# divelab/DIG

Hardware: NVIDIA H100
Metric: molecules/sec SphereNet QM9-shape (higher is better)
Workload: dtype f32

## Files before the change

### dig_b200/_lib.py

```python
import ctypes
import os
from ctypes import POINTER, Structure, c_char_p, c_double, c_int32, c_int64, c_void_p

_HERE = os.path.dirname(os.path.abspath(__file__))
LIB_PATH = os.path.join(_HERE, "libdig3d.so")

P = c_void_p


class InitEWeights(Structure):
    _fields_ = [(n, P) for n in ("emb", "w_rbf0", "b_rbf0", "w_lin", "b_lin", "w_rbf1")]


class UpdateEWeights(Structure):
    _fields_ = ([(n, P) for n in ("w_rbf1", "w_rbf2", "w_sbf2", "w_t2", "w_rbf",
                                  "w_kj", "b_kj", "w_ji", "b_ji", "w_down", "w_up")]
                + [("w_res", P * 6), ("b_res", P * 6), ("w_lin", P), ("b_lin", P)])


class SchnetBlockWeights(Structure):
    _fields_ = [(n, P) for n in ("w_lin", "w_mlp0", "b_mlp0", "w_mlp2", "b_mlp2", "w_v1", "b_v1", "w_v2", "b_v2")]


class ComenetBlockWeights(Structure):
    _fields_ = ([(n, P) for n in ("w_lin", "b_lin", "w_f1a", "w_f1b", "w_f2a", "w_f2b", "w_rel1", "b_rel1",
                                  "w_root1", "w_rel2", "b_rel2", "w_root2", "w_lin1", "b_lin1", "w_lin2",
                                  "b_lin2", "w_cat", "b_cat")]
                + [("w_lins", P * 8), ("b_lins", P * 8)]
                + [(n, P) for n in ("norm_w", "norm_b", "norm_ms", "w_final", "b_final")]
                + [("n_lins", c_int32)])


class ComenetHeadWeights(Structure):
    _fields_ = [("w_lins", P * 8), ("b_lins", P * 8), ("w_out", P), ("b_out", P), ("n_lins", c_int32)]


class TcUpdateE(Structure):
    _fields_ = ([(n, P) for n in ("p_ji", "b_ji", "p_kj", "b_kj", "p_down", "p_up")]
                + [("p_res", P * 6), ("b_res", P * 6)]
                + [(n, P) for n in ("p_lin", "b_lin", "w_rbf1", "w_rbf2", "w_rbf", "w_sbf2", "w_t2")])


class UpdateVWeights(Structure):
    _fields_ = [("w_up", P), ("b_up", P), ("w_lins", P * 8), ("b_lins", P * 8), ("w_out", P),
                ("n_lins", c_int32)]


SIGNATURES = {
    "dig3d_last_error": [],
    "dig3d_abi_version": [],
    "dig3d_graph_ptr": [P, c_int64, c_int64, P, P],
    "dig3d_radius_neighbors": [P, P, P, c_int64, c_int64, c_double, c_int32, P, P, P],
    "dig3d_validate_nodes": [P, P, c_int64, c_int64, c_int32, P, P],
    "dig3d_knn2": [P, P, P, c_int64, c_int64, P, P, P],
    "dig3d_triplet_geometry_knn": [P, P, P, P, P, c_int64, P, P, P, P, P, P, P],
    "dig3d_triplet_count": [P, P, c_int64, c_int32, P, P],
    "dig3d_triplet_count_out": [P, P, c_int64, c_int32, P, P, P],
    "dig3d_scan_counts3": [P, P, P, c_int64, P, P, P, P, P],
    "dig3d_edge_fill_out": [P, P, P, P, P, c_int64, c_int32, c_int64, P, P, P, P, P, P, P, P, P, P, P, P],
    "dig3d_scan_counts": [P, P, c_int64, P, P, P, P],
    "dig3d_edge_fill": [P, P, P, P, P, c_int64, c_int32, c_int64, P, P, P, P, P, P, P],
    "dig3d_edges_to_csr": [P, P, c_int64, c_int64, P, P, P, P, P, P, P, P],
    "dig3d_triplet_geometry": [P, P, P, P, P, c_int64, c_int32, P, P, P, P, P, P, P],
    "dig3d_edge_basis": [P, c_int64, c_double, c_int32, P, c_int32, c_int32, P, P, P],
    "dig3d_edge_basis_set_split": [c_int32],
    "dig3d_triplet_basis_project_set_mode": [c_int32],
    "dig3d_triplet_basis": [P, P, P, P, c_int64, c_int32, P, P, P],
    "dig3d_triplet_basis_project": [P, P, P, P, P, P, P, P, P, c_int64, c_int64, c_int32, c_int32,
                                    c_int32, P, P, P, P, P],
    "dig3d_triplet_basis_project_lists": [P, P, P, P, P, P, P, P, P, c_int64, c_int64, c_int32, c_int32,
                                    c_int32, P, P, P, P, P, P, P, P],
    "dig3d_triplet_basis_project_node": [P, P, P, P, P, P, P, P, c_int64, c_int64, c_int32, c_int32, c_int32, c_int32,
                                         P, P, P, P, P],
    "dig3d_segment_sum": [P, P, c_int64, c_int64, P, P],
    "dig3d_sphere_init_e": [P, P, P, P, c_int64, POINTER(InitEWeights), P, P, P],
    "dig3d_sphere_update_e_a": [P, P, c_int64, POINTER(UpdateEWeights), P, P, P],
    "dig3d_sphere_update_e_b": [P, P, P, P, P, P, c_int32, P, P, P, P, c_int64,
                                POINTER(UpdateEWeights), P, P, P],
    "dig3d_sphere_update_v": [P, c_int64, c_int32, POINTER(UpdateVWeights), P, P],
    "dig3d_sphere_update_v_batched": [P, c_int64, c_int32, c_int32, P, P, P],
    "dig3d_graph_readout": [P, P, c_int64, c_int64, c_int32, c_int32, P, P],
    "dig3d_tc_packed_floats": [c_int32, c_int32],
    "dig3d_tc_pack": [P, P, P, P, c_int32, P],
    "dig3d_tc_timeouts": [],
    "dig3d_sphere_init_e_tc": [P, P, P, P, c_int64, POINTER(InitEWeights), P, P, P, P],
    "dig3d_sphere_update_e_a_tc": [P, P, c_int64, POINTER(TcUpdateE), P, P, P],
    "dig3d_sphere_triplet_gather": [P, P, P, c_int32, P, P, P, P, c_int64, P, P, P, P],
    "dig3d_sphere_triplet_gather_node": [P, P, P, c_int32, P, P, P, P, P, c_int64, c_int32, P, P, P, P],
    "dig3d_sphere_triplet_gather_warp": [P, P, P, c_int32, P, P, P, P, P, c_int64, c_int32, c_int32, P, P, P, P, P,
                                         P, P],
    "dig3d_sphere_triplet_gather_tc": [P, P, P, c_int32, P, P, P, P, P, c_int64, c_int32, P, P, P, P],
    "dig3d_sphere_update_e_b_tc": [P, P, P, P, P, c_int64, POINTER(TcUpdateE), P, P, P],
    "dig3d_tc_set_fast_swish": [c_int32],
    "dig3d_h16_packed_bytes": [c_int32, c_int32],
    "dig3d_h16_pack": [P, P, P, P, c_int32, P],
    "dig3d_sphere_init_e_h16": [P, P, P, P, c_int64, POINTER(InitEWeights), P, P, P, P],
    "dig3d_sphere_init_e_h16_tab": [P, P, P, P, c_int64, POINTER(InitEWeights), P, P, P, P, P, P],
    "dig3d_sphere_update_e_a_h16": [P, P, c_int64, POINTER(TcUpdateE), P, P, P],
    "dig3d_sphere_update_e_b_h16": [P, P, P, P, P, c_int64, POINTER(TcUpdateE), P, P, P],
    "dig3d_sphere_update_e_ba_h16": [P, P, P, P, P, c_int64, POINTER(TcUpdateE), POINTER(TcUpdateE), P, P, P, P, P],
    "dig3d_sphere_update_v_h16_supported": [c_int32, c_int32, c_int32, c_int32],
    "dig3d_sphere_update_v_h16": [P, c_int64, c_int32, c_int32, c_int32, P, P, P, P],
    "dig3d_h16_pack_t": [P, P, P, P, P, c_int32, P],
    "dig3d_linear_h16_supported": [c_int32, c_int32],
    "dig3d_linear_h16": [P, c_int64, c_int32, c_int32, P, P, P, P, P, P],
    "dig3d_h16_overflow": [c_int32],
    "dig3d_h16_timeouts": [],
    "dig3d_h16_trace": [c_int32, P],
    "dig3d_h16_set_fast_swish": [c_int32],
    "dig3d_h16_set_wide_epilogue": [c_int32],
    "dig3d_tc_trace": [c_int32, P],
    "dig3d_schnet_block": [P, c_int64, P, P, P, c_int64, P, c_int32, c_double, c_double, c_int32, c_int32,
                           POINTER(SchnetBlockWeights), P, P, P, P],
    "dig3d_schnet_readout": [P, c_int64, c_int32, P, P, P, P, c_int32, P, P],
    "dig3d_comenet_geometry": [P, P, P, P, P, P, P, c_int64, c_int64, c_double, P, P, P, P, P],
    "dig3d_comenet_embed": [P, P, c_int64, P, P],
    "dig3d_pbc_edge_vectors": [P, P, P, P, P, c_int64, P, P, P],
    "dig3d_comenet_geometry_edges": [P, P, P, P, P, c_int64, c_int64, c_double, P, P, P, P, P, P],
    "dig3d_radius_graph_pbc_count": [P, P, P, c_int64, c_int64, c_double, c_int32, P, P, P, P, P, P, P],
    "dig3d_radius_graph_pbc_fill": [P, P, c_int64, c_int64, c_double, P, P, P, P, c_int64, P, P, P, P],
    "dig3d_comenet_block": [P, P, P, P, P, P, P, c_int64, c_int64, c_int64, POINTER(ComenetBlockWeights),
                            POINTER(ComenetHeadWeights), c_int32, P, P, P, P, P, P, P, P],
    "dig3d_edge_weighted_sum": [P, P, P, P, c_int64, c_int32, P, P],
    "dig3d_comenet_filter_sum": [P, c_int32, P, P, P, P, c_int64, c_int32, P, P],
    "dig3d_linear": [P, c_int64, c_int32, c_int32, P, P, P, P, c_int32, P],
    "dig3d_wgrad": [P, P, c_int64, c_int32, c_int32, P, P, c_int32, P],
    "dig3d_wgrad_tc": [P, P, c_int64, c_int32, c_int32, P, P, c_int32, P],
    "dig3d_wgrad_tc_supported": [c_int64, c_int32, c_int32],
    "dig3d_wgrad_set_mode": [c_int32],
    "dig3d_wgrad_tc_timeouts": [],
    "dig3d_act": [P, c_int64, c_int32, P, P],
    "dig3d_act_bwd": [P, P, c_int64, c_int32, P, P],
    "dig3d_adam_step": [P, P, P, P, c_int64, c_double, c_double, c_double, c_double, c_double, c_int64, P],
    "dig3d_ewise": [P, P, c_int64, c_int32, P, P],
    "dig3d_rowscale": [P, P, c_int64, c_int32, P, P],
    "dig3d_gather_rows": [P, P, c_int32, c_int64, c_int32, P, P],
    "dig3d_scatter_add_rows": [P, P, c_int32, c_int64, c_int32, P, P],
    "dig3d_rbf_freq_grad": [P, c_int64, c_double, c_int32, P, c_int32, P, P, P],
    "dig3d_triplet_basis_project_bwd": [P, P, P, P, P, P, P, P, P, c_int64, c_int64, c_int32, P, P, P, P, P],
    "dig3d_sphere_triplet_gather_bwd": [P, P, P, P, P, P, P, P, c_int64, P, P, P, P, P, P, P, P],
    "dig3d_graphnorm": [P, P, c_int64, c_int32, P, P, P, c_double, P, P, P, P],
    "dig3d_graphnorm_bwd": [P, P, P, c_int64, c_int32, P, P, P, P, P, P, P, P, P],
    "dig3d_edge_dist_bwd": [P, P, P, P, P, c_int64, P, P],
    "dig3d_triplet_angle_bwd": [P, P, P, P, P, P, c_int64, P, P],
    "dig3d_edge_basis_bwd": [P, c_int64, c_double, c_int32, P, c_int32, c_int32, P, P, P, P],
    "dig3d_triplet_basis_project_bwd_geom": [P, P, P, P, P, P, P, P, P, P, c_int64, c_int64, c_int32, P, P, P, P,
                                             c_double, P, P, P, P],
    "dig3d_triplet_torsion_bwd": [P, P, P, P, P, P, c_int64, P, P],
    "dig3d_schnet_edge_features_bwd": [P, c_int64, P, c_int32, c_double, c_double, P, P, P, P],
    "dig3d_rowdot": [P, P, c_int64, c_int32, P, P],
    "dig3d_tc_pack_t": [P, P, P, P, P, c_int32, P],
    "dig3d_linear_tc_supported": [c_int32, c_int32],
    "dig3d_linear_tc": [P, c_int64, c_int32, c_int32, P, P, P, P, P],
    "dig3d_act_bwd2": [P, P, P, c_int64, c_int32, P, P],
    "dig3d_geometry_jvp": [P, P, P, P, P, P, P, c_int64, P, P, P, P],
    "dig3d_edge_basis_tangent": [P, P, c_int64, c_double, c_int32, P, c_int32, c_int32, P, P, P],
    "dig3d_rbf_freq_grad_tangent": [P, P, c_int64, c_double, c_int32, P, c_int32, P, P, P],
    "dig3d_triplet_basis_tangent": [P, P, P, P, P, P, P, c_int64, c_int32, P, P, P],
    "dig3d_edge_dist_bwd2": [P, P, P, P, P, P, c_int64, P, P, P],
    "dig3d_schnet_edge_features_bwd2": [P, c_int64, P, c_int32, c_double, c_double, P, P, P, P, P, P, P],
    "dig3d_pronet_edge_features": [P, P, P, P, P, c_int64, c_int64, c_int32, c_double, c_int32, P, P, P, P, P, P],
    "dig3d_linear_set_config": [c_int32],
    "dig3d_transpose": [P, c_int32, c_int32, P, P],
    "dig3d_schnet_edge_features": [P, c_int64, P, c_int32, c_double, c_double, P, P, P],
}
_RESTYPES = {"dig3d_last_error": c_char_p, "dig3d_h16_packed_bytes": c_int64}

_lib = None


class Dig3dError(RuntimeError):
    rc = None


def load():
    global _lib
    if _lib is not None:
        return _lib
    if not os.path.exists(LIB_PATH):
        raise Dig3dError(
            f"{LIB_PATH} not found: build it with `python -m dig_b200.build` "
            "(nvcc -gencode arch=compute_90a,code=sm_90a). There is no CPU/PyTorch fallback.")
    lib = ctypes.CDLL(LIB_PATH)
    for name, argtypes in SIGNATURES.items():
        try:
            fn = getattr(lib, name)
        except AttributeError as exc:
            raise Dig3dError(f"libdig3d.so does not export {name}") from exc
        fn.argtypes = argtypes
        fn.restype = _RESTYPES.get(name, ctypes.c_int)
    _lib = lib
    return lib


launch_count = 0
_timing = None


def start_timing():
    global _timing
    _timing = {}


def stop_timing():
    global _timing
    import torch
    torch.cuda.synchronize()
    out = {k: [a.elapsed_time(b) for a, b in v] for k, v in (_timing or {}).items()}
    _timing = None
    return out


def call(name, *args):
    global launch_count
    lib = load()
    if _timing is not None:
        import torch
        a, b = torch.cuda.Event(enable_timing=True), torch.cuda.Event(enable_timing=True)
        a.record()
        rc = getattr(lib, name)(*args)
        b.record()
        _timing.setdefault(name, []).append((a, b))
    else:
        rc = getattr(lib, name)(*args)
    launch_count += 1
    if rc != 0:
        msg = lib.dig3d_last_error()
        err = Dig3dError(f"{name} failed (rc={rc}): {msg.decode() if msg else ''}")
        err.rc = rc
        raise err
```

### dig_b200/csrc/spherenet_h16.cu

```cuda
#include <cuda_fp16.h>
#include "common.cuh"
#define TC90_TM_COLS 512
#include "wgmma.cuh"

namespace dig3d {
using namespace tc90;

constexpr int H_M = 128;
constexpr int H_AKU = H_M + 1;
constexpr int H_PLANE = 16 * H_AKU * 16;
constexpr int H_STAGES = 5;
constexpr int H_SLAB_K = 32;
constexpr int H_STAGE_BYTES = 2 * 4 * 128 * 16;
constexpr int H_TILE_WARPS = 8;
constexpr int H_TILE_THREADS = H_TILE_WARPS * 32;
constexpr int H_CTRL_THREADS = 128;
constexpr int H_THREADS = H_CTRL_THREADS + 2 * H_TILE_THREADS;
constexpr int H_CTRL_WARPS = H_CTRL_THREADS / 32;
__device__ __forceinline__ void h_regs_ctrl() { asm volatile("setmaxnreg.dec.sync.aligned.u32 64;"); }
__device__ __forceinline__ void h_regs_epi() { asm volatile("setmaxnreg.inc.sync.aligned.u32 104;"); }
constexpr float H_SA = 8.0f, H_SW = 64.0f;
constexpr float H_INV = 1.0f / (H_SA * H_SW);
constexpr int H_LDS = 129;

struct HSmem {
  unsigned char a[2][2][H_PLANE];
  unsigned char w[H_STAGES][H_STAGE_BYTES];
  float bias[8][128];
  float wr[128 * 8];
  int dst[2][H_M];
  int aux[2][2][H_M];
  uint64_t full[H_STAGES], empty[H_STAGES], a_ready[2], d_ready[2][2], d_free[2][2];
  uint64_t l_done;
  uint32_t tmem_base;
};
static_assert(sizeof(HSmem) <= 227 * 1024, "HSmem exceeds the shared memory of an SM");
static_assert(sizeof(HSmem) > TM_ONE_CTA_PER_SM_SMEM, "one CTA per SM sizes the accumulator-store slot pool");
static_assert(2 * H_PLANE == H_M * H_LDS * 4, "the fp32 staging overlay must cover exactly one tile's planes");

struct HGemm {
  const unsigned char* w;
  const float* bias;
  int K, N;
  int tile_stride;
};

static __device__ unsigned int g_h16_overflow = 0;
static int h16_fast_swish = 1;
static __device__ long long g_h16_trace[128];
static __device__ int g_h16_trace_on = 0;

__device__ __forceinline__ float ex2_ftz(float x) {
  float y;
  asm("ex2.approx.ftz.f32 %0, %1;" : "=f"(y) : "f"(x));
  return y;
}
__device__ __forceinline__ float rcp_ftz(float x) {
  float y;
  asm("rcp.approx.ftz.f32 %0, %1;" : "=f"(y) : "f"(x));
  return y;
}
template <bool FAST>
__device__ __forceinline__ float hswish(float x) {
  return FAST ? x * rcp_ftz(1.0f + ex2_ftz(x * -1.4426950408889634f)) : __fdiv_rn(x, 1.0f + expf(-x));
}
template <bool FAST>
__device__ __forceinline__ float hswish8(float t8) {
  return FAST ? t8 * rcp_ftz(1.0f + ex2_ftz(t8 * (-1.4426950408889634f / H_SA)))
              : __fdiv_rn(t8, 1.0f + expf(-t8 * (1.0f / H_SA)));
}

struct HRing {
  int q, t, c;
};
__device__ __forceinline__ void h_produce(HSmem& s, const HGemm* g, int ng, int ntile, HRing& r, int& it) {
  if (r.q >= ng) return;
  const uint32_t bytes = 2u * 4u * (uint32_t)g[r.q].N * 16u;
  if (threadIdx.x == 0) {
    const int st = it % H_STAGES;
    mbar_arrive_expect_tx(&s.full[st], bytes);
    bulk_g2s(s.w[st], g[r.q].w + (size_t)r.t * g[r.q].tile_stride + (size_t)r.c * bytes, bytes, &s.full[st]);
  }
  ++it;
  if (++r.c == g[r.q].K / H_SLAB_K) { r.c = 0; if (++r.t == ntile) { r.t = 0; ++r.q; } }
}
template <bool SHARED_A>
__device__ __forceinline__ void h_mma_n(HSmem& s, const HGemm* g, int ng, int ntile, uint32_t tmem) {
  const int wt = threadIdx.x;
  HRing ring = {0, 0, 0};
  int pit = 0;
  for (int i = 0; i < H_STAGES; ++i) h_produce(s, g, ng, ntile, ring, pit);
  int it = 0, ch = 0;
  int uses00 = 0, uses01 = 0, uses10 = 0, uses11 = 0;
  int last0 = -1, last1 = -1;
  for (int q = 0; q < ng; ++q) {
    const int nslab = g[q].K / H_SLAB_K, n = g[q].N;
    for (int t = 0; t < ntile; ++t) {
      if (!SHARED_A || t == 0) {
        mbar_wait(&s.a_ready[SHARED_A ? 0 : t], q & 1);
        tc_fence_after();
      }
      const uint32_t a_hi = smem_u32(SHARED_A ? s.a[0][0] : s.a[t][0]), a_lo = smem_u32(SHARED_A ? s.a[1][0] : s.a[t][1]);
      for (int c = 0; c < nslab; c += 2, it += 2) {
        const int ab = ch & 1;
        const int lt = ab ? last1 : last0;
        if (lt >= 0) {
          const int u = lt ? (ab ? uses11 : uses10) : (ab ? uses01 : uses00);
          mbar_wait(&s.d_free[lt][ab], (u - 1) & 1);
        }
        mbar_wait(&s.full[it % H_STAGES], (it / H_STAGES) & 1);
        mbar_wait(&s.full[(it + 1) % H_STAGES], ((it + 1) / H_STAGES) & 1);
        tc_fence_after();
        for (int mh = 0; mh < 2; ++mh)
          for (int nh = 0; nh < n / 64; ++nh) {
            float d[32];
            wg_fence();
#pragma unroll
            for (int sl = 0; sl < 2; ++sl) {
              const uint32_t w_hi = smem_u32(s.w[(it + sl) % H_STAGES]) + (uint32_t)(nh * 64 * 16), w_lo = w_hi + 4u * n * 16u;
              const uint32_t a_m = (uint32_t)(mh * 64 * 16);
#pragma unroll
              for (int ks = 0; ks < 2; ++ks) {
                const uint32_t a_off = a_m + (uint32_t)(((c + sl) * 4 + ks * 2) * H_AKU * 16), b_off = (uint32_t)(ks * 2 * n * 16);
                mma_f16(d, smem_desc(a_lo + a_off, H_AKU * 16, 128), smem_desc(w_hi + b_off, n * 16, 128), (sl | ks) != 0);
                mma_f16(d, smem_desc(a_hi + a_off, H_AKU * 16, 128), smem_desc(w_lo + b_off, n * 16, 128), 1);
              }
#pragma unroll
              for (int ks = 0; ks < 2; ++ks) {
                const uint32_t a_off = a_m + (uint32_t)(((c + sl) * 4 + ks * 2) * H_AKU * 16), b_off = (uint32_t)(ks * 2 * n * 16);
                mma_f16(d, smem_desc(a_hi + a_off, H_AKU * 16, 128), smem_desc(w_hi + b_off, n * 16, 128), 1);
              }
            }
            wg_commit();
            wg_wait0();
            tm_store_frag(d, wt, tmem + ((uint32_t)(64 * mh) << 16) + 128u * ab + 64u * nh);
          }
        tc_fence_before();
        wg_bar();
        h_produce(s, g, ng, ntile, ring, pit);
        h_produce(s, g, ng, ntile, ring, pit);
        if (wt == 0) mbar_arrive(&s.d_ready[t][ab]);
        if (t) { if (ab) ++uses11; else ++uses10; } else { if (ab) ++uses01; else ++uses00; }
        if (ab) last1 = t; else last0 = t;
        ++ch;
      }
      if (SHARED_A && t == ntile - 1 && wt == 0) mbar_arrive(&s.l_done);
    }
  }
}

struct HCtx {
  int t, et, row, half;
  uint32_t tl;
  int ntile, ch;
  int use0, use1;
  bool bad;
  unsigned char *ahi, *alo;
};
__device__ __forceinline__ HCtx h_ctx(HSmem& s, int ntile) {
  const int warp = threadIdx.x >> 5, lane = threadIdx.x & 31;
  const int t = (warp - H_CTRL_WARPS) / H_TILE_WARPS, we = (warp - H_CTRL_WARPS) % H_TILE_WARPS;
  const int quarter = warp & 3;
  return {t, (int)threadIdx.x - H_CTRL_THREADS - t * H_TILE_THREADS, 32 * quarter + lane, we >> 2,
          s.tmem_base + ((uint32_t)(32 * quarter) << 16), ntile, 0, 0, 0, false, s.a[t][0], s.a[t][1]};
}
__device__ __forceinline__ void h_tile_bar(int t) {
  asm volatile("bar.sync %0, %1;" ::"r"(1 + t), "n"(H_TILE_THREADS) : "memory");
}
__device__ __forceinline__ void h_epi_done(HSmem& s, int t) {
  fence_async_smem();
  tc_fence_before();
  __syncwarp();
  if ((threadIdx.x & 31) == 0) mbar_arrive(&s.a_ready[t]);
}
__device__ __forceinline__ void h_store_ku(HSmem& s, const HCtx& c, int row, int ku, const float (&x)[8]) {
  uint32_t h[4], l[4];
#pragma unroll
  for (int i = 0; i < 4; ++i) {
    const __half2 hh = __floats2half2_rn(x[2 * i], x[2 * i + 1]);
    const float2 hf = __half22float2(hh);
    const __half2 ll = __floats2half2_rn(x[2 * i] - hf.x, x[2 * i + 1] - hf.y);
    h[i] = *reinterpret_cast<const uint32_t*>(&hh);
    l[i] = *reinterpret_cast<const uint32_t*>(&ll);
  }
  const int o = (ku * H_AKU + row) * 16;
  *reinterpret_cast<uint4*>(c.ahi + o) = make_uint4(h[0], h[1], h[2], h[3]);
  *reinterpret_cast<uint4*>(c.alo + o) = make_uint4(l[0], l[1], l[2], l[3]);
}
__device__ __forceinline__ void h_store_a16(HSmem& s, const HCtx& c, int col, const float (&v8)[16]) {
  float x[8];
#pragma unroll
  for (int u = 0; u < 2; ++u) {
#pragma unroll
    for (int i = 0; i < 8; ++i) x[i] = v8[8 * u + i];
    h_store_ku(s, c, c.row, (col >> 3) + u, x);
  }
}
__device__ __forceinline__ bool h_finite(float x) { return fabsf(x) <= 3.402823466e38f; }
template <int KU>
__device__ __forceinline__ void h_load_tile(HSmem& s, HCtx& c, const float* __restrict__ g, size_t ld, int rows) {
#pragma unroll
  for (int k = 0; k < H_M * KU / H_TILE_THREADS; ++k) {
    const int f = c.et + k * H_TILE_THREADS, row = f / KU, ku = f % KU;
    float x[8];
    if (row < rows) {
      const float4 p0 = __ldg(reinterpret_cast<const float4*>(g + (size_t)row * ld + ku * 8));
      const float4 p1 = __ldg(reinterpret_cast<const float4*>(g + (size_t)row * ld + ku * 8 + 4));
      x[0] = p0.x * H_SA; x[1] = p0.y * H_SA; x[2] = p0.z * H_SA; x[3] = p0.w * H_SA;
      x[4] = p1.x * H_SA; x[5] = p1.y * H_SA; x[6] = p1.z * H_SA; x[7] = p1.w * H_SA;
    } else {
#pragma unroll
      for (int i = 0; i < 8; ++i) x[i] = 0.f;
    }
    h_store_ku(s, c, row, ku, x);
  }
}
template <int KU>
struct HTileRegs { float4 v[H_M * KU / H_TILE_THREADS][2]; };
template <int KU>
__device__ __forceinline__ void h_tile_fetch(HTileRegs<KU>& r, int et, const float* __restrict__ g, size_t ld, int rows) {
#pragma unroll
  for (int k = 0; k < H_M * KU / H_TILE_THREADS; ++k) {
    const int f = et + k * H_TILE_THREADS, row = f / KU, ku = f % KU;
    if (row < rows) {
      r.v[k][0] = __ldg(reinterpret_cast<const float4*>(g + (size_t)row * ld + ku * 8));
      r.v[k][1] = __ldg(reinterpret_cast<const float4*>(g + (size_t)row * ld + ku * 8 + 4));
    } else {
      r.v[k][0] = r.v[k][1] = make_float4(0.f, 0.f, 0.f, 0.f);
    }
  }
}
template <int KU>
__device__ __forceinline__ void h_tile_commit(HSmem& s, const HCtx& c, const HTileRegs<KU>& r) {
#pragma unroll
  for (int k = 0; k < H_M * KU / H_TILE_THREADS; ++k) {
    const int f = c.et + k * H_TILE_THREADS, row = f / KU, ku = f % KU;
    const float4 p0 = r.v[k][0], p1 = r.v[k][1];
    const float x[8] = {p0.x * H_SA, p0.y * H_SA, p0.z * H_SA, p0.w * H_SA, p1.x * H_SA, p1.y * H_SA, p1.z * H_SA, p1.w * H_SA};
    h_store_ku(s, c, row, ku, x);
  }
}
template <int NP, bool FIRST>
__device__ __forceinline__ void h_drain(HSmem& s, HCtx& c, int col0, int chunks, float (&acc)[NP * 16]) {
  if (c.t == 1) c.ch += chunks;
  for (int k = 0; k < chunks; ++k, ++c.ch) {
    const int ab = c.ch & 1;
    const int use = ab ? c.use1 : c.use0;
    mbar_wait(&s.d_ready[c.t][ab], use & 1);
    if (ab) ++c.use1; else ++c.use0;
    tc_fence_after();
    const uint32_t ta = c.tl + 128u * ab + col0;
    if (FIRST && k == 0) {
#pragma unroll
      for (int p = 0; p < NP; ++p) tmem_ld16f(ta + 16 * p, &acc[p * 16]);
      tmem_ld_wait();
    } else {
#pragma unroll
      for (int p = 0; p < NP; p += 2) {
        uint32_t r[2][16];
        tmem_ld16(ta + 16 * p, r[0]);
        if (p + 1 < NP) tmem_ld16(ta + 16 * p + 16, r[1]);
        tmem_ld_wait();
#pragma unroll
        for (int i = 0; i < 16; ++i) {
          acc[p * 16 + i] = __fadd_rn(acc[p * 16 + i], __uint_as_float(r[0][i]));
          if (p + 1 < NP) acc[p * 16 + 16 + i] = __fadd_rn(acc[p * 16 + 16 + i], __uint_as_float(r[1][i]));
        }
      }
    }
    tc_fence_before();
    __syncwarp();
    if ((threadIdx.x & 31) == 0) mbar_arrive(&s.d_free[c.t][ab]);
  }
  if (c.t == 0 && c.ntile == 2) c.ch += chunks;
}
__device__ __forceinline__ void h_setup(HSmem& s, int a_ready_warps = H_TILE_WARPS, int d_free_warps = H_TILE_WARPS) {
  if (threadIdx.x == 0) {
    for (int i = 0; i < H_STAGES; ++i) { mbar_init(&s.full[i], 1); mbar_init(&s.empty[i], 1); }
    for (int i = 0; i < 2; ++i) {
      mbar_init(&s.a_ready[i], a_ready_warps);
      for (int j = 0; j < 2; ++j) { mbar_init(&s.d_ready[i][j], 1); mbar_init(&s.d_free[i][j], d_free_warps); }
    }
    mbar_init(&s.l_done, 1);
    mbar_fence_init();
  }
  if ((threadIdx.x >> 5) == 0) tmem_alloc(&s.tmem_base, 512);
}
__device__ __forceinline__ void h_finish(HSmem& s, const HCtx* c) {
  if (c && c->bad) atomicOr(&g_h16_overflow, 1u);
  tc_fence_before();
  __syncthreads();
  if ((threadIdx.x >> 5) == 0) tmem_dealloc(s.tmem_base, 512);
}
template <int W>
__device__ __forceinline__ void h_store_tile_coalesced(HSmem& s, const HCtx& c, int col0, const float (&v)[W / 2],
                                                       float* __restrict__ out, int rows) {
  constexpr int LD = W + 1, RPW = 128 / W;
  float* st = reinterpret_cast<float*>(s.a[c.t][0]);
#pragma unroll
  for (int i = 0; i < W / 2; ++i) st[c.row * LD + col0 + i] = v[i];
  h_tile_bar(c.t);
  const int w = c.et >> 5, lane = c.et & 31;
  for (int r0 = w * RPW; r0 < rows; r0 += H_TILE_WARPS * RPW) {
    const int r = r0 + (RPW == 2 ? (lane >> 4) : 0), c4 = 4 * (RPW == 2 ? (lane & 15) : lane);
    if (r < rows) {
      const float* src = st + r * LD + c4;
      *reinterpret_cast<float4*>(out + (size_t)r * W + c4) = make_float4(src[0], src[1], src[2], src[3]);
    }
  }
}

template <int W>
__device__ __forceinline__ void h_store_tile_strided(HSmem& s, const HCtx& c, int col0, const float (&v)[W / 2],
                                                     float* __restrict__ out, int ld, int rows,
                                                     const float* __restrict__ res = nullptr) {
  constexpr int LD = W + 1, RPW = 128 / W;
  float* st = reinterpret_cast<float*>(s.a[c.t][0]);
#pragma unroll
  for (int i = 0; i < W / 2; ++i) st[c.row * LD + col0 + i] = v[i];
  h_tile_bar(c.t);
  const int w = c.et >> 5, lane = c.et & 31;
  for (int r0 = w * RPW; r0 < rows; r0 += H_TILE_WARPS * RPW) {
    const int r = r0 + (RPW == 2 ? (lane >> 4) : 0), c4 = 4 * (RPW == 2 ? (lane & 15) : lane);
    if (r < rows) {
      const float* src = st + r * LD + c4;
      float4 o = make_float4(src[0], src[1], src[2], src[3]);
      if (res) {
        const float4 q = __ldg(reinterpret_cast<const float4*>(res + (size_t)r * ld + c4));
        o.x += q.x; o.y += q.y; o.z += q.z; o.w += q.w;
      }
      *reinterpret_cast<float4*>(out + (size_t)r * ld + c4) = o;
    }
  }
}

__device__ __forceinline__ void h_segment_sums(const HSmem& s, const HCtx& c, int rows, float* __restrict__ v_in) {
  const int col = c.et & 127, r0 = (c.et >> 7) * 64, r1 = min(rows, r0 + 64);
  if (r0 >= r1) return;
  const float* e2t = reinterpret_cast<const float*>(s.a[c.t][0]);
  const int* dst = s.dst[c.t];
  float run = 0.f;
  int cur = dst[r0];
  bool first = true;
  for (int r = r0; r < r1; ++r) {
    const int d = dst[r];
    if (d != cur) {
      if (first) atomicAdd(v_in + (size_t)cur * 128 + col, run);
      else v_in[(size_t)cur * 128 + col] = run;
      first = false; run = 0.f; cur = d;
    }
    run += e2t[r * H_LDS + col];
  }
  atomicAdd(v_in + (size_t)cur * 128 + col, run);
}

struct HPackJob { const float* w; unsigned char* out; int N, K, trans; };
struct HPackJobs { HPackJob job[16]; };
__global__ void h16_pack_kernel(HPackJobs jobs) {
  const HPackJob jb = jobs.job[blockIdx.y];
  const int total = jb.N * jb.K;
  for (int id = blockIdx.x * blockDim.x + threadIdx.x; id < total; id += gridDim.x * blockDim.x) {
    const int n = id / jb.K, k = id % jb.K;
    const float x = __ldg(jb.w + (jb.trans ? (size_t)k * jb.trans + n : (size_t)id)) * H_SW;
    const __half h = __float2half_rn(x);
    const __half l = __float2half_rn(x - __half2float(h));
    const int c = k >> 5, ku = (k & 31) >> 3, kk = k & 7;
    const size_t slab = (size_t)c * (2 * 4 * jb.N * 16);
    const size_t o = ((size_t)ku * jb.N + n) * 16 + kk * 2;
    *reinterpret_cast<__half*>(jb.out + slab + o) = h;
    *reinterpret_cast<__half*>(jb.out + slab + (size_t)4 * jb.N * 16 + o) = l;
  }
}

constexpr int R_UNIT = 64;
constexpr int R_STAGES = 8;
constexpr int R_LDS = 136;
constexpr int R_WG = 128;
constexpr int R_THREADS = 3 * R_WG;
__device__ __forceinline__ void r_regs_producer() { asm volatile("setmaxnreg.dec.sync.aligned.u32 40;"); }
__device__ __forceinline__ void r_regs_consumer() { asm volatile("setmaxnreg.inc.sync.aligned.u32 232;"); }

struct RSmem {
  unsigned char w[R_STAGES][H_STAGE_BYTES];
  float tile[2][R_UNIT * R_LDS];
  float rbf[2][R_UNIT * 6];
  float bias[8][128];
  float bias_a[2][128];
  float wr[128 * 8];
  float wr1[64];
  float wr2[128 * 8];
  int dst[2][R_UNIT];
  uint64_t full[R_STAGES], empty[R_STAGES];
};
static_assert(sizeof(RSmem) <= 227 * 1024, "RSmem exceeds the shared memory of an SM");

enum { RE_B = 0, RE_BA = 1, RE_A = 2 };
struct REParams {
  HGemm g[11];
  const float* w_rbf;
  const float *w_rbf1, *w_rbf2;
  float *x_ji, *x_down;
};

__device__ __forceinline__ void r_bar(int cw) { asm volatile("bar.sync %0, %1;" ::"r"(1 + cw), "n"(R_WG) : "memory"); }
__device__ __forceinline__ void cp_async4(void* sm, const void* g, bool valid) {
  asm volatile("cp.async.ca.shared.global [%0], [%1], 4, %2;" ::"r"(smem_u32(sm)), "l"(g), "r"(valid ? 4 : 0) : "memory");
}
__device__ __forceinline__ void cp_async8(void* sm, const void* g, bool valid) {
  asm volatile("cp.async.ca.shared.global [%0], [%1], 8, %2;" ::"r"(smem_u32(sm)), "l"(g), "r"(valid ? 8 : 0) : "memory");
}
__device__ __forceinline__ void cp_async_commit() { asm volatile("cp.async.commit_group;" ::: "memory"); }
__device__ __forceinline__ void cp_async_wait_all() { asm volatile("cp.async.wait_group 0;" ::: "memory"); }

__device__ __forceinline__ void r_split(float x0, float x1, uint32_t& hi, uint32_t& lo) {
  const __half2 hh = __floats2half2_rn(x0, x1);
  const float2 hf = __half22float2(hh);
  const __half2 ll = __floats2half2_rn(x0 - hf.x, x1 - hf.y);
  hi = *reinterpret_cast<const uint32_t*>(&hh);
  lo = *reinterpret_cast<const uint32_t*>(&ll);
}
struct RA { uint32_t hi[8][4], lo[8][4]; };
__device__ __forceinline__ void r_acc_to_a(const float (&v)[64], RA& a, float scale = 1.0f) {
#pragma unroll
  for (int s = 0; s < 8; ++s)
#pragma unroll
    for (int r = 0; r < 4; ++r) r_split(v[frag_a_src(s, r)] * scale, v[frag_a_src(s, r) + 1] * scale, a.hi[s][r], a.lo[s][r]);
}
template <int KS>
__device__ __forceinline__ void r_load_a(RA& a, const float* __restrict__ g, int ld, int rows, int wt) {
#pragma unroll
  for (int s = 0; s < KS; ++s)
#pragma unroll
    for (int r = 0; r < 4; ++r) {
      const int row = frag_a_row(wt, r), col = frag_a_col(wt, s, r);
      const float2 x = row < rows ? __ldg(reinterpret_cast<const float2*>(g + (size_t)row * ld + col)) : make_float2(0.f, 0.f);
      r_split(x.x * H_SA, x.y * H_SA, a.hi[s][r], a.lo[s][r]);
    }
}
__device__ __forceinline__ void r_fetch_rows(float* tile, const float* __restrict__ src, int rows, int fr, int fc) {
#pragma unroll
  for (int j = 0; j < 16; ++j)
#pragma unroll
    for (int h = 0; h < 2; ++h) {
      const int row = fr + 8 * h, col = 8 * j + fc;
      cp_async8(tile + row * R_LDS + col, src + (size_t)(row < rows ? row : 0) * 128 + col, row < rows);
    }
  cp_async_commit();
}

__device__ __forceinline__ void r_release(RSmem& s, int it, int n) {
  __syncwarp();
  if ((threadIdx.x & 31) == 0)
    for (int i = 0; i < n; ++i) mbar_arrive(&s.empty[(it + i) % R_STAGES]);
}
template <int CH, int N>
__device__ __forceinline__ void r_chunk(RSmem& s, const RA& a, float (&t)[N / 2], int it) {
#pragma unroll
  for (int sl = 0; sl < 2; ++sl) {
    const uint32_t w_hi = smem_u32(s.w[(it + 2 * CH + sl) % R_STAGES]), w_lo = w_hi + 4u * N * 16u;
#pragma unroll
    for (int ks = 0; ks < 2; ++ks) {
      const int k = 4 * CH + 2 * sl + ks;
      const uint32_t b_off = (uint32_t)(ks * 2 * N * 16);
      mma_f16_rs(t, a.lo[k], smem_desc(w_hi + b_off, N * 16, 128), (sl | ks) != 0);
      mma_f16_rs(t, a.hi[k], smem_desc(w_lo + b_off, N * 16, 128), 1);
    }
#pragma unroll
    for (int ks = 0; ks < 2; ++ks)
      mma_f16_rs(t, a.hi[4 * CH + 2 * sl + ks], smem_desc(w_hi + (uint32_t)(ks * 2 * N * 16), N * 16, 128), 1);
  }
}
template <int NCH, int N>
__device__ __forceinline__ void r_issue(RSmem& s, const RA& a, float (&acc)[N / 2], float (&d)[N / 2], int it) {
#pragma unroll
  for (int i = 0; i < 2 * NCH; ++i) mbar_wait(&s.full[(it + i) % R_STAGES], ((it + i) / R_STAGES) & 1);
  wg_fence();
  r_chunk<0, N>(s, a, acc, it);
  if (NCH == 2) r_chunk<1, N>(s, a, d, it);
  wg_commit();
}
template <int NCH, int N>
__device__ __forceinline__ void r_complete(RSmem& s, float (&acc)[N / 2], const float (&d)[N / 2], int& it) {
  wg_wait0();
  r_release(s, it, 2 * NCH);
  it += 2 * NCH;
  if (NCH == 2) {
#pragma unroll
    for (int i = 0; i < N / 2; ++i) acc[i] = __fadd_rn(acc[i], d[i]);
  }
}
__device__ __forceinline__ void r_skip(RSmem& s, int& it, int n) {
  for (int i = 0; i < n; ++i, ++it) {
    mbar_wait(&s.full[it % R_STAGES], (it / R_STAGES) & 1);
    r_release(s, it, 1);
  }
}

__device__ __forceinline__ void r_segment_sums(const float* tile, const int* dst, int rows, int col,
                                               float* __restrict__ v_in) {
  float run = 0.f;
  int cur = dst[0];
  bool first = true;
  for (int r = 0; r < rows; ++r) {
    const int d = dst[r];
    if (d != cur) {
      if (first) atomicAdd(v_in + (size_t)cur * 128 + col, run);
      else v_in[(size_t)cur * 128 + col] = run;
      first = false; run = 0.f; cur = d;
    }
    run += tile[r * R_LDS + col];
  }
  atomicAdd(v_in + (size_t)cur * 128 + col, run);
}

template <bool FAST, int MODE>
__global__ void __launch_bounds__(R_THREADS, 1)
sphere_update_e_h16_kernel(const float* __restrict__ m, const float* __restrict__ x_ji,
                           const float* __restrict__ e1_in, const float* __restrict__ rbf0,
                           const int32_t* __restrict__ dst, int n_edges, REParams P, float* __restrict__ e1_out,
                           float* __restrict__ v_in) {
  constexpr int NG = MODE == RE_B ? 8 : MODE == RE_BA ? 11 : 3;
  extern __shared__ __align__(1024) unsigned char h_raw[];
  RSmem& s = *reinterpret_cast<RSmem*>(h_raw);
  const int tid = threadIdx.x, wg = tid / R_WG;
  auto n_units = [&]() { return (n_edges + R_UNIT - 1) / R_UNIT; };
  auto rounds = [&]() {
    return (n_units() - (int)blockIdx.x + 2 * (int)gridDim.x - 1) / (2 * (int)gridDim.x);
  };
  const bool trace = g_h16_trace_on && blockIdx.x == 0;
  if (tid == 0 && trace) { g_h16_trace[100] = clock64(); g_h16_trace[101] = (long long)global_ns(); }
  if (tid == 0) {
    for (int i = 0; i < R_STAGES; ++i) { mbar_init(&s.full[i], 1); mbar_init(&s.empty[i], 8); }
    mbar_fence_init();
  }
  if (MODE != RE_A) {
    for (int i = tid; i < 8 * 128; i += R_THREADS) {
      const float* b = P.g[i / 128].bias;
      s.bias[i / 128][i % 128] = b ? H_SA * __ldg(b + i % 128) : 0.f;
    }
    for (int i = tid; i < 128 * 8; i += R_THREADS) s.wr[i] = (i % 8 < 6) ? __ldg(P.w_rbf + (i / 8) * 6 + i % 8) : 0.f;
  }
  if (MODE != RE_B) {
    constexpr int GA = MODE == RE_A ? 0 : 8;
    for (int i = tid; i < 2 * 128; i += R_THREADS)
      s.bias_a[i / 128][i % 128] = (i / 128 ? H_SA : 1.0f) * __ldg(P.g[GA + i / 128].bias + i % 128);
    for (int i = tid; i < 128 * 8; i += R_THREADS) s.wr2[i] = __ldg(P.w_rbf2 + i);
    for (int i = tid; i < 64; i += R_THREADS) s.wr1[i] = (i % 8 < 6) ? __ldg(P.w_rbf1 + (i / 8) * 6 + i % 8) : 0.f;
  }
  __syncthreads();
  if (tid == 0 && trace) g_h16_trace[104] = clock64();

  if (wg == 0) {
    r_regs_producer();
    if (tid == 0) {
      int it = 0;
      const int nr = rounds();
      for (int k = 0; k < nr; ++k)
        for (int q = 0; q < NG; ++q) {
          const uint32_t bytes = 2u * 4u * (uint32_t)P.g[q].N * 16u;
          for (int c = 0; c < P.g[q].K / H_SLAB_K; ++c, ++it) {
            const int st = it % R_STAGES;
            if (it >= R_STAGES) mbar_wait(&s.empty[st], ((it / R_STAGES) + 1) & 1);
            mbar_arrive_expect_tx(&s.full[st], bytes);
            bulk_g2s(s.w[st], P.g[q].w + (size_t)c * bytes, bytes, &s.full[st]);
          }
        }
    }
    return;
  }

  r_regs_consumer();
  const int cw = threadIdx.x / R_WG - 1, wt = threadIdx.x & (R_WG - 1);
  const int nu = n_units(), nr = rounds();
  const int fr = frag_row(wt), fc = frag_col(wt);
  float* tile = s.tile[cw];
  const float* rbf = s.rbf[cw];
  int slabs = 0;
  for (int q = 0; q < NG; ++q) slabs += P.g[q].K / H_SLAB_K;
  const bool probe = g_h16_trace_on && blockIdx.x == 0 && wt == 0;
  int lq = 0;
  auto tp = [&](bool on, int point) { if (on) g_h16_trace[cw * 48 + lq * 4 + point] = clock64(); };
  bool staggered = cw == 1, bad = false;
  auto stagger = [&]() {
    if (!staggered) { asm volatile("bar.arrive 3, %0;" ::"n"(2 * R_WG) : "memory"); staggered = true; }
  };
  if (cw == 1) asm volatile("bar.sync 3, %0;" ::"n"(2 * R_WG) : "memory");
  int it = 0;
#pragma unroll 1
  for (int k = 0; k < nr; ++k) {
    const int unit = blockIdx.x + (2 * k + cw) * gridDim.x;
    if (unit >= nu) { r_skip(s, it, slabs); continue; }
    const int e0 = unit * R_UNIT, rows = min(R_UNIT, n_edges - e0);
    const bool tr = probe && k == 0;
    lq = 0;
    r_bar(cw);
    for (int i = wt; i < R_UNIT * 6; i += R_WG)
      cp_async4(&s.rbf[cw][i], rbf0 + (size_t)e0 * 6 + (i < rows * 6 ? i : 0), i < rows * 6);
    RA a;
    float acc[64], d[64];
    if (MODE != RE_A) {
      if (wt < R_UNIT) cp_async4(&s.dst[cw][wt], dst + e0 + (wt < rows ? wt : 0), wt < rows);
      r_fetch_rows(tile, x_ji + (size_t)e0 * 128, rows, fr, fc);
      r_load_a<4>(a, m + (size_t)e0 * 64, 64, rows, wt);
#pragma unroll 1
      for (int q = 0; q < 7; ++q, ++lq) {
        tp(tr, 0);
        if (q == 0) {
          r_issue<1, 128>(s, a, acc, d, it);
          stagger();
          tp(tr, 1);
          r_complete<1, 128>(s, acc, d, it);
        } else {
          r_issue<2, 128>(s, a, acc, d, it);
          tp(tr, 1);
          r_complete<2, 128>(s, acc, d, it);
        }
        tp(tr, 2);
        const bool add_tile = q == 0 || q == 2 || q == 3 || q == 5;
        const bool to_tile = q == 0 || q == 3 || q == 5;
        const float tile_scale = (q == 0 || q == 3) ? H_SA : 1.0f;
        if (q == 0 || q == 3) cp_async_wait_all();
#pragma unroll
        for (int j = 0; j < 16; ++j)
#pragma unroll
          for (int h = 0; h < 2; ++h) {
            const int row = fr + 8 * h, col = 8 * j + fc, i = 4 * j + 2 * h;
            const float2 b = *reinterpret_cast<const float2*>(&s.bias[q][col]);
            float v0 = hswish8<FAST>(fmaf(acc[i], H_SA * H_INV, b.x));
            float v1 = hswish8<FAST>(fmaf(acc[i + 1], H_SA * H_INV, b.y));
            float2* tp2 = reinterpret_cast<float2*>(tile + row * R_LDS + col);
            if (add_tile) {
              const float2 r = *tp2;
              v0 += r.x * tile_scale;
              v1 += r.y * tile_scale;
            }
            if (to_tile) *tp2 = make_float2(v0, v1);
            acc[i] = v0;
            acc[i + 1] = v1;
          }
        r_acc_to_a(acc, a);
        if (q == 0) r_bar(cw);
        if (q == 2) r_fetch_rows(tile, e1_in + (size_t)e0 * 128, rows, fr, fc);
        tp(tr, 3);
      }
      tp(tr, 0);
      r_issue<2, 128>(s, a, acc, d, it);
      tp(tr, 1);
      r_complete<2, 128>(s, acc, d, it);
      tp(tr, 2);
      {
        float rb[2][6];
#pragma unroll
        for (int h = 0; h < 2; ++h)
#pragma unroll
          for (int n = 0; n < 6; ++n) rb[h][n] = rbf[(fr + 8 * h) * 6 + n];
#pragma unroll
        for (int j = 0; j < 16; ++j)
#pragma unroll
          for (int h = 0; h < 2; ++h) {
            const int row = fr + 8 * h, col = 8 * j + fc, i = 4 * j + 2 * h;
            const float2 b = *reinterpret_cast<const float2*>(&s.bias[7][col]);
            float2* tp2 = reinterpret_cast<float2*>(tile + row * R_LDS + col);
            const float2 r = *tp2;
            float e2[2];
#pragma unroll
            for (int u = 0; u < 2; ++u) {
              const float v = hswish8<FAST>(fmaf(acc[i + u], H_SA * H_INV, u ? b.y : b.x)) + (u ? r.y : r.x);
              const float o = v * (1.0f / H_SA);
              bad |= !h_finite(o);
              const float4 w0 = *reinterpret_cast<const float4*>(s.wr + (col + u) * 8);
              const float2 w1 = *reinterpret_cast<const float2*>(s.wr + (col + u) * 8 + 4);
              const float gsum = fmaf(w1.y, rb[h][5], fmaf(w1.x, rb[h][4], fmaf(w0.w, rb[h][3], fmaf(w0.z, rb[h][2],
                                 fmaf(w0.y, rb[h][1], w0.x * rb[h][0])))));
              e2[u] = gsum * o;
              acc[i + u] = o;
            }
            *tp2 = make_float2(e2[0], e2[1]);
          }
      }
      tp(tr, 3);
      ++lq;
      r_bar(cw);
      r_segment_sums(tile, s.dst[cw], rows, wt, v_in);
#pragma unroll
      for (int j = 0; j < 16; ++j)
#pragma unroll
        for (int h = 0; h < 2; ++h) {
          const int row = fr + 8 * h, i = 4 * j + 2 * h;
          if (row < rows)
            *reinterpret_cast<float2*>(e1_out + (size_t)(e0 + row) * 128 + 8 * j + fc) = make_float2(acc[i], acc[i + 1]);
        }
      if (tr) g_h16_trace[96 + cw] = clock64();
      if (MODE == RE_BA) r_acc_to_a(acc, a, H_SA);
    } else {
      cp_async_commit();
      r_load_a<8>(a, e1_in + (size_t)e0 * 128, 128, rows, wt);
    }
    if (MODE != RE_B) {
      tp(tr, 0);
      r_issue<2, 128>(s, a, acc, d, it);
      stagger();
      tp(tr, 1);
      r_complete<2, 128>(s, acc, d, it);
      tp(tr, 2);
#pragma unroll
      for (int j = 0; j < 16; ++j)
#pragma unroll
        for (int h = 0; h < 2; ++h) {
          const int row = fr + 8 * h, col = 8 * j + fc, i = 4 * j + 2 * h;
          const float2 b = *reinterpret_cast<const float2*>(&s.bias_a[0][col]);
          if (row < rows) {
            const float2 o = make_float2(hswish<FAST>(fmaf(acc[i], H_INV, b.x)), hswish<FAST>(fmaf(acc[i + 1], H_INV, b.y)));
            bad |= !(h_finite(o.x) && h_finite(o.y));
            *reinterpret_cast<float2*>(P.x_ji + (size_t)(e0 + row) * 128 + col) = o;
          }
        }
      if (MODE == RE_A) { cp_async_wait_all(); r_bar(cw); }
      tp(tr, 3);
      ++lq;
      tp(tr, 0);
      r_issue<2, 128>(s, a, acc, d, it);
      tp(tr, 1);
      r_complete<2, 128>(s, acc, d, it);
      tp(tr, 2);
      {
        float r8[2][8];
#pragma unroll
        for (int h = 0; h < 2; ++h)
#pragma unroll
          for (int mm = 0; mm < 8; ++mm) {
            float x = 0.f;
#pragma unroll
            for (int n = 0; n < 6; ++n) x = fmaf(s.wr1[mm * 8 + n], rbf[(fr + 8 * h) * 6 + n], x);
            r8[h][mm] = x;
          }
#pragma unroll
        for (int j = 0; j < 16; ++j)
#pragma unroll
          for (int h = 0; h < 2; ++h)
#pragma unroll
            for (int u = 0; u < 2; ++u) {
              const int col = 8 * j + fc + u, i = 4 * j + 2 * h + u;
              const float4 w0 = *reinterpret_cast<const float4*>(s.wr2 + col * 8);
              const float4 w1 = *reinterpret_cast<const float4*>(s.wr2 + col * 8 + 4);
              const float* g = r8[h];
              const float gate = fmaf(w1.w, g[7], fmaf(w1.z, g[6], fmaf(w1.y, g[5], fmaf(w1.x, g[4],
                                 fmaf(w0.w, g[3], fmaf(w0.z, g[2], fmaf(w0.y, g[1], w0.x * g[0])))))));
              acc[i] = hswish8<FAST>(fmaf(acc[i], H_SA * H_INV, s.bias_a[1][col])) * gate;
            }
      }
      r_acc_to_a(acc, a);
      tp(tr, 3);
      ++lq;
      {
        float a64[32], d64[32];
        tp(tr, 0);
        r_issue<2, 64>(s, a, a64, d64, it);
        tp(tr, 1);
        r_complete<2, 64>(s, a64, d64, it);
        tp(tr, 2);
#pragma unroll
        for (int j = 0; j < 8; ++j)
#pragma unroll
          for (int h = 0; h < 2; ++h) {
            const int row = fr + 8 * h, i = 4 * j + 2 * h;
            if (row < rows) {
              const float2 o = make_float2(hswish<FAST>(a64[i] * H_INV), hswish<FAST>(a64[i + 1] * H_INV));
              bad |= !(h_finite(o.x) && h_finite(o.y));
              *reinterpret_cast<float2*>(P.x_down + (size_t)(e0 + row) * 64 + 8 * j + fc) = o;
            }
          }
        tp(tr, 3);
      }
    }
  }
  stagger();
  if (bad) atomicOr(&g_h16_overflow, 1u);
  if (probe && cw == 0) { g_h16_trace[102] = clock64(); g_h16_trace[103] = (long long)global_ns(); }
}

template <int MODE>
static int launch_update_e_h16(const float* m, const float* x_ji, const float* e1_in, const float* rbf0,
                               const int32_t* dst, int64_t n_edges, const REParams& P, float* e1_out, float* v_in,
                               cudaStream_t st) {
  auto kfn = h16_fast_swish ? sphere_update_e_h16_kernel<true, MODE> : sphere_update_e_h16_kernel<false, MODE>;
  cudaError_t e = cudaFuncSetAttribute(kfn, cudaFuncAttributeMaxDynamicSharedMemorySize, (int)sizeof(RSmem));
  if (e != cudaSuccess) {
    set_error("cudaFuncSetAttribute(%zu): %s", sizeof(RSmem), cudaGetErrorString(e));
    return DIG3D_ECUDA;
  }
  int dev = 0, n_sm = 132;
  cudaGetDevice(&dev);
  cudaDeviceGetAttribute(&n_sm, cudaDevAttrMultiProcessorCount, dev);
  const int units = (int)ceil_div(n_edges, R_UNIT);
  const int grid = min(n_sm, (units + 1) / 2);
  kfn<<<grid, R_THREADS, sizeof(RSmem), st>>>(m, x_ji, e1_in, rbf0, dst, (int)n_edges, P, e1_out, v_in);
  DIG3D_LAUNCH_CHECK();
  return DIG3D_OK;
}

struct HInitParams {
  HGemm g[3];
  const float *emb, *w_rbf0, *b_rbf0, *b_lin, *w_rbf1;
  const float *tab_i, *tab_j;
};

template <bool FAST, bool TABLE>
__global__ void __launch_bounds__(H_THREADS, 1)
sphere_init_e_h16_kernel(const int64_t* __restrict__ z, const int32_t* __restrict__ src,
                         const int32_t* __restrict__ dst, const float* __restrict__ rbf0, int n_edges, HInitParams P,
                         float* __restrict__ e1, float* __restrict__ v_in) {
  extern __shared__ __align__(1024) unsigned char h_raw[];
  HSmem& s = *reinterpret_cast<HSmem*>(h_raw);
  const int tid = threadIdx.x, warp = tid >> 5;
  const int n_tiles = (n_edges + H_M - 1) / H_M, tile0 = blockIdx.x * 2, ntile = min(2, n_tiles - tile0);
  float* w0 = &s.bias[2][0];
  h_setup(s);
  for (int i = tid; i < 128; i += H_THREADS) { s.bias[0][i] = __ldg(P.b_lin + i); s.bias[1][i] = __ldg(P.b_rbf0 + i); }
  for (int i = tid; i < 128 * 6; i += H_THREADS) w0[i] = __ldg(P.w_rbf0 + i);
  for (int i = tid; i < 128 * 8; i += H_THREADS) s.wr[i] = (i % 8 < 6) ? __ldg(P.w_rbf1 + (i / 8) * 6 + i % 8) : 0.f;
  for (int i = tid; i < 2 * H_M; i += H_THREADS) {
    const int t = i / H_M, r = i % H_M, e = (tile0 + t) * H_M + r;
    const int d = (e < n_edges) ? dst[e] : -1, sj = (e < n_edges) ? src[e] : -1;
    s.dst[t][r] = d;
    s.aux[t][0][r] = d >= 0 ? (int)z[d] : 0;
    s.aux[t][1][r] = sj >= 0 ? (int)z[sj] : 0;
  }
  tc_fence_before();
  __syncthreads();
  tc_fence_after();
  HCtx c;
  bool epi = false;
  if (warp < H_CTRL_WARPS) {
    h_regs_ctrl();
    h_mma_n<false>(s, P.g, TABLE ? 1 : 3, ntile, s.tmem_base);
  } else if (h_regs_epi(), (c = h_ctx(s, ntile)).t < ntile) {
    epi = true;
    const int e0 = (tile0 + c.t) * H_M, rows = min(H_M, n_edges - e0);
    const bool valid = c.row < rows;
    const size_t ge = (size_t)(e0 + c.row);
    const int col0 = c.half * 64;
    const uint32_t stash = c.tl + 256u + 128u * c.t + col0;
    float rb[6];
#pragma unroll
    for (int n = 0; n < 6; ++n) rb[n] = valid ? __ldg(rbf0 + ge * 6 + n) : 0.f;
    auto fill_embedding = [&](const int* zrow) {
#pragma unroll
      for (int k = 0; k < H_M * 16 / H_TILE_THREADS; ++k) {
        const int f = c.et + k * H_TILE_THREADS, row = f >> 4, ku = f & 15;
        float x[8];
        if (row < rows) {
          const float* er = P.emb + (size_t)zrow[row] * 128 + ku * 8;
          const float4 p0 = __ldg(reinterpret_cast<const float4*>(er));
          const float4 p1 = __ldg(reinterpret_cast<const float4*>(er + 4));
          x[0] = p0.x * H_SA; x[1] = p0.y * H_SA; x[2] = p0.z * H_SA; x[3] = p0.w * H_SA;
          x[4] = p1.x * H_SA; x[5] = p1.y * H_SA; x[6] = p1.z * H_SA; x[7] = p1.w * H_SA;
        } else {
#pragma unroll
          for (int i = 0; i < 8; ++i) x[i] = 0.f;
        }
        h_store_ku(s, c, row, ku, x);
      }
    };
    float acc[64];
    if (!TABLE) {
      fill_embedding(s.aux[c.t][0]);
      h_epi_done(s, c.t);
      h_drain<4, true>(s, c, col0, 2, acc);
      fill_embedding(s.aux[c.t][1]);
      h_epi_done(s, c.t);
      h_drain<4, false>(s, c, col0, 2, acc);
    }
#pragma unroll
    for (int p = 0; p < 4; ++p) {
      float v[16];
#pragma unroll
      for (int i = 0; i < 16; ++i) {
        const int col = col0 + 16 * p + i;
        float a = 0.f;
#pragma unroll
        for (int n = 0; n < 6; ++n) a = fmaf(w0[col * 6 + n], rb[n], a);
        v[i] = valid ? H_SA * hswish<FAST>(a + s.bias[1][col]) : 0.f;
      }
      h_store_a16(s, c, col0 + 16 * p, v);
    }
    h_epi_done(s, c.t);
    if (TABLE) {
      const float* ti = P.tab_i + (size_t)s.aux[c.t][0][c.row] * 128 + col0;
      const float* tj = P.tab_j + (size_t)s.aux[c.t][1][c.row] * 128 + col0;
#pragma unroll
      for (int p = 0; p < 4; ++p) {
        uint32_t r[16];
#pragma unroll
        for (int i = 0; i < 16; i += 4) {
          const float4 a = __ldg(reinterpret_cast<const float4*>(ti + 16 * p + i));
          const float4 b = __ldg(reinterpret_cast<const float4*>(tj + 16 * p + i));
          r[i] = __float_as_uint(a.x + b.x); r[i + 1] = __float_as_uint(a.y + b.y);
          r[i + 2] = __float_as_uint(a.z + b.z); r[i + 3] = __float_as_uint(a.w + b.w);
        }
        tmem_st16(stash + 16 * p, r);
      }
      tmem_st_wait();
      h_drain<4, true>(s, c, col0, 2, acc);
#pragma unroll
      for (int p = 0; p < 4; ++p) {
        uint32_t r[16];
        tmem_ld16(stash + 16 * p, r);
        tmem_ld_wait();
#pragma unroll
        for (int i = 0; i < 16; ++i) acc[16 * p + i] = fmaf(acc[16 * p + i], H_INV, __uint_as_float(r[i])) * (H_SA * H_SW);
      }
    } else {
      h_drain<4, false>(s, c, col0, 2, acc);
    }
    float* e2t = reinterpret_cast<float*>(s.a[c.t][0]);
#pragma unroll
    for (int i = 0; i < 64; ++i) {
      const int col = col0 + i;
      const float o = hswish<FAST>(fmaf(acc[i], H_INV, s.bias[0][col]));
      c.bad |= !h_finite(o);
      const float4 w0 = *reinterpret_cast<const float4*>(s.wr + col * 8);
      const float2 w1 = *reinterpret_cast<const float2*>(s.wr + col * 8 + 4);
      const float gsum = fmaf(w1.y, rb[5], fmaf(w1.x, rb[4], fmaf(w0.w, rb[3], fmaf(w0.z, rb[2],
                         fmaf(w0.y, rb[1], w0.x * rb[0])))));
      e2t[c.row * H_LDS + col] = gsum * o;
      acc[i] = o;
    }
    h_tile_bar(c.t);
    h_segment_sums(s, c, rows, v_in);
    h_tile_bar(c.t);
    h_store_tile_coalesced<128>(s, c, col0, acc, e1 + (size_t)e0 * 128, rows);
  }
  h_finish(s, epi ? &c : nullptr);
}

struct HVBlock {
  const unsigned char* p[9];
  const float* b[9];
  const float* w_out;
};
struct HVParams { HVBlock blk[8]; int n_lins, out_channels; };

template <bool FAST>
__global__ void __launch_bounds__(H_THREADS, 1)
sphere_update_v_h16_kernel(const float* __restrict__ v_in_all, int n_nodes, HVParams P, float* __restrict__ v_out_all) {
  extern __shared__ __align__(1024) unsigned char h_raw[];
  HSmem& s = *reinterpret_cast<HSmem*>(h_raw);
  const int tid = threadIdx.x, warp = tid >> 5;
  const HVBlock& B = P.blk[blockIdx.y];
  const int r0 = blockIdx.x * H_M, rows = min(H_M, n_nodes - r0);
  const int ng = P.n_lins + 1, C = P.out_channels;
  __shared__ HGemm g[9];
  h_setup(s, 2 * H_TILE_WARPS);
  if (tid < ng) g[tid] = {B.p[tid], nullptr, tid == 0 ? 128 : 256, 128, (tid == 0 ? 128 : 256) * 128 * 4};
  for (int i = tid; i < min(ng, 4) * 256; i += H_THREADS) (&s.bias[0][0])[i] = H_SA * __ldg(B.b[i / 256] + i % 256);
  for (int i = tid; i < C * 256; i += H_THREADS) s.wr[i] = __ldg(B.w_out + i);
  tc_fence_before();
  __syncthreads();
  tc_fence_after();
  if (warp < H_CTRL_WARPS) {
    h_regs_ctrl();
    h_mma_n<true>(s, g, ng, 2, s.tmem_base);
  } else {
    h_regs_epi();
    HCtx c = h_ctx(s, 2);
    c.ahi = s.a[0][0];
    c.alo = s.a[1][0];
    const int et2 = tid - H_CTRL_THREADS;
    const int col0 = c.half * 64;
    const int gcol0 = 128 * c.t + col0;
    const float* vin = v_in_all + ((size_t)blockIdx.y * n_nodes + r0) * 128;
#pragma unroll
    for (int k = 0; k < H_M * 16 / (2 * H_TILE_THREADS); ++k) {
      const int f = et2 + k * 2 * H_TILE_THREADS, row = f >> 4, ku = f & 15;
      float x[8];
      if (row < rows) {
        const float4 p0 = __ldg(reinterpret_cast<const float4*>(vin + (size_t)row * 128 + ku * 8));
        const float4 p1 = __ldg(reinterpret_cast<const float4*>(vin + (size_t)row * 128 + ku * 8 + 4));
        x[0] = p0.x * H_SA; x[1] = p0.y * H_SA; x[2] = p0.z * H_SA; x[3] = p0.w * H_SA;
        x[4] = p1.x * H_SA; x[5] = p1.y * H_SA; x[6] = p1.z * H_SA; x[7] = p1.w * H_SA;
      } else {
#pragma unroll
        for (int i = 0; i < 8; ++i) x[i] = 0.f;
      }
      h_store_ku(s, c, row, ku, x);
    }
    fence_async_smem();
    tc_fence_before();
    __syncwarp();
    if ((tid & 31) == 0) mbar_arrive(&s.a_ready[0]);
    float acc[64];
#pragma unroll 1
    for (int q = 0; q < ng; ++q) {
      h_drain<4, true>(s, c, col0, q == 0 ? 2 : 4, acc);
#pragma unroll
      for (int i = 0; i < 64; i += 4) {
        float4 b;
        if (q < 4) b = *reinterpret_cast<const float4*>(&(&s.bias[0][0])[q * 256 + gcol0 + i]);
        else {
          b = __ldg(reinterpret_cast<const float4*>(B.b[q] + gcol0 + i));
          b.x *= H_SA; b.y *= H_SA; b.z *= H_SA; b.w *= H_SA;
        }
        acc[i] = fmaf(acc[i], H_SA * H_INV, b.x); acc[i + 1] = fmaf(acc[i + 1], H_SA * H_INV, b.y);
        acc[i + 2] = fmaf(acc[i + 2], H_SA * H_INV, b.z); acc[i + 3] = fmaf(acc[i + 3], H_SA * H_INV, b.w);
        if (q > 0) {
          acc[i] = hswish8<FAST>(acc[i]); acc[i + 1] = hswish8<FAST>(acc[i + 1]);
          acc[i + 2] = hswish8<FAST>(acc[i + 2]); acc[i + 3] = hswish8<FAST>(acc[i + 3]);
        }
      }
      mbar_wait(&s.l_done, q & 1);
      tc_fence_after();
      if (q + 1 < ng) {
#pragma unroll
        for (int p = 0; p < 4; ++p) {
          float v16[16];
#pragma unroll
          for (int i = 0; i < 16; ++i) v16[i] = acc[16 * p + i];
          h_store_a16(s, c, gcol0 + 16 * p, v16);
        }
        fence_async_smem();
        tc_fence_before();
        __syncwarp();
        if ((tid & 31) == 0) mbar_arrive(&s.a_ready[0]);
      }
    }
    float* red = reinterpret_cast<float*>(s.a[0][0]);
    const int slot = 2 * c.t + c.half;
    for (int o = 0; o < C; ++o) {
      float part = 0.f;
#pragma unroll
      for (int i = 0; i < 64; ++i) part = fmaf(acc[i], s.wr[o * 256 + gcol0 + i], part);
      red[(c.row * 4 + slot) * C + o] = part * (1.0f / H_SA);
      c.bad |= !h_finite(part);
    }
    asm volatile("bar.sync 3, %0;" ::"n"(2 * H_TILE_THREADS) : "memory");
    if (slot == 0 && c.row < rows) {
      float* out = v_out_all + ((size_t)blockIdx.y * n_nodes + r0 + c.row) * C;
      for (int o = 0; o < C; ++o) {
        const float* rr = red + (c.row * 4) * C + o;
        out[o] = ((rr[0] + rr[C]) + rr[2 * C]) + rr[3 * C];
      }
    }
    h_finish(s, &c);
    return;
  }
  h_finish(s, nullptr);
}

struct HLinParams { HGemm g[3]; };

template <int NPANEL, int KU, int N>
__global__ void __launch_bounds__(H_THREADS, 1)
linear_h16_kernel(const float* __restrict__ x, int n_rows, int ldx, HLinParams P, const float* __restrict__ bias,
                  float* __restrict__ y, float* __restrict__ act_out, const float* __restrict__ residual, int ldy,
                  int tiles_per_cta, int slice_bytes) {
  extern __shared__ __align__(1024) unsigned char h_raw[];
  HSmem& s = *reinterpret_cast<HSmem*>(h_raw);
  constexpr int NC = N / 2;
  const int tid = threadIdx.x, warp = tid >> 5;
  {
    const int slice = blockIdx.y;
#pragma unroll
    for (int p = 0; p < NPANEL; ++p) P.g[p].w += (size_t)slice * slice_bytes;
    if (bias) bias += slice * N;
    if (y) y += slice * N;
    if (act_out) act_out += slice * N;
    if (residual) residual += slice * N;
  }
  const int n_tiles = (n_rows + H_M - 1) / H_M, tile0 = blockIdx.x * tiles_per_cta;
  const int ntile = min(tiles_per_cta, n_tiles - tile0);
  h_setup(s);
  for (int i = tid; i < N; i += H_THREADS) s.bias[0][i] = bias ? __ldg(bias + i) : 0.f;
  tc_fence_before();
  __syncthreads();
  tc_fence_after();
  HCtx c;
  bool epi = false;
  if (warp < H_CTRL_WARPS) {
    h_regs_ctrl();
    h_mma_n<false>(s, P.g, NPANEL, ntile, s.tmem_base);
  } else if (h_regs_epi(), (c = h_ctx(s, ntile)).t < ntile) {
    epi = true;
    const int r0 = (tile0 + c.t) * H_M, rows = min(H_M, n_rows - r0);
    const int col0 = c.half * NC;
    float acc[NC];
#pragma unroll
    for (int p = 0; p < NPANEL; ++p) {
      h_load_tile<KU>(s, c, x + (size_t)r0 * ldx + p * (KU * 8), ldx, rows);
      h_epi_done(s, c.t);
      if (p == 0) h_drain<NC / 16, true>(s, c, col0, KU / 8, acc);
      else h_drain<NC / 16, false>(s, c, col0, KU / 8, acc);
    }
#pragma unroll
    for (int i = 0; i < NC; ++i) {
      acc[i] = fmaf(acc[i], H_INV, s.bias[0][col0 + i]);
      c.bad |= !h_finite(acc[i]);
    }
    const float* res = residual ? residual + (size_t)r0 * ldy : nullptr;
    if (y) h_store_tile_strided<N>(s, c, col0, acc, y + (size_t)r0 * ldy, ldy, rows, act_out ? nullptr : res);
    if (act_out) {
#pragma unroll
      for (int i = 0; i < NC; ++i) acc[i] = hswish<false>(acc[i]);
      if (y) h_tile_bar(c.t);
      h_store_tile_strided<N>(s, c, col0, acc, act_out + (size_t)r0 * ldy, ldy, rows, res);
    }
  }
  h_finish(s, epi ? &c : nullptr);
}

constexpr int GT_ROWS = 128;
constexpr int GT_XLD = 68;
constexpr int GT_YLD = 65;
constexpr int GT_MAXIN = 64, GT_MAXOUT = 256, GT_MAXSEG = 128;
constexpr float GT_SS = 8.0f, GT_SW = 64.0f;

struct GTSmem {
  unsigned char s_hi[2 * GT_ROWS * 16], s_lo[2 * GT_ROWS * 16];
  unsigned char t_hi[2 * GT_ROWS * 16], t_lo[2 * GT_ROWS * 16];
  unsigned char ws_hi[2 * 64 * 16], ws_lo[2 * 64 * 16], wt_hi[2 * 64 * 16], wt_lo[2 * 64 * 16];
  float x[GT_MAXIN * GT_XLD];
  float y[GT_ROWS * GT_YLD];
  int in_src[GT_MAXIN];
  int out_e[GT_MAXOUT], out_pos[GT_MAXOUT];
  int seg_row[GT_MAXSEG + 1], seg_out[GT_MAXSEG];
  int row_seg[GT_ROWS];
  int row_src[GT_ROWS];
  int n_out, n_seg, next_u;
};

template <bool TORSION>
__global__ void __launch_bounds__(GT_ROWS)
sphere_triplet_gather_tc_kernel(const float* __restrict__ x_down, const float* __restrict__ sbf_p,
                                const float* __restrict__ t_p, const int32_t* __restrict__ src,
                                const int32_t* __restrict__ row_ptr, const int32_t* __restrict__ trip_ptr,
                                const int32_t* __restrict__ graph_ptr, const int64_t* __restrict__ batch,
                                int n_nodes, const float* __restrict__ w_sbf2, const float* __restrict__ w_t2,
                                float* __restrict__ m) {
  extern __shared__ __align__(1024) unsigned char gt_raw[];
  GTSmem& s = *reinterpret_cast<GTSmem*>(gt_raw);
  const int tid = threadIdx.x, lane = tid & 31, w = tid >> 5;
  for (int i = tid; i < (int)(4 * 2 * GT_ROWS * 16 / 16); i += GT_ROWS) reinterpret_cast<uint4*>(s.s_hi)[i] = make_uint4(0, 0, 0, 0);
  for (int i = tid; i < 64 * 8; i += GT_ROWS) {
    const int n = i >> 3, k = i & 7;
    {
      const float v = __ldg(w_sbf2 + i) * GT_SW;
      const __half h = __float2half_rn(v);
      reinterpret_cast<__half*>(s.ws_hi)[n * 8 + k] = h;
      reinterpret_cast<__half*>(s.ws_lo)[n * 8 + k] = __float2half_rn(v - __half2float(h));
    }
    if (TORSION) {
      const float v = __ldg(w_t2 + i) * GT_SW;
      const __half h = __float2half_rn(v);
      reinterpret_cast<__half*>(s.wt_hi)[n * 8 + k] = h;
      reinterpret_cast<__half*>(s.wt_lo)[n * 8 + k] = __float2half_rn(v - __half2float(h));
    }
  }
  for (int i = tid; i < 64 * 8; i += GT_ROWS) {
    reinterpret_cast<__half*>(s.ws_hi)[64 * 8 + i] = __float2half_rn(0.f);
    reinterpret_cast<__half*>(s.ws_lo)[64 * 8 + i] = __float2half_rn(0.f);
    reinterpret_cast<__half*>(s.wt_hi)[64 * 8 + i] = __float2half_rn(0.f);
    reinterpret_cast<__half*>(s.wt_lo)[64 * 8 + i] = __float2half_rn(0.f);
  }
  __syncthreads();
  for (int j = blockIdx.x; j < n_nodes; j += gridDim.x) {
    const int base = row_ptr[j], d = row_ptr[j + 1] - base;
    const int g = (int)batch[j], lo = graph_ptr[g], hi = graph_ptr[g + 1];
    __syncthreads();
    for (int k = tid; k < d; k += GT_ROWS) s.in_src[k] = src[base + k];
    for (int i = tid; i < d * 16; i += GT_ROWS) {
      const int r = i >> 4, c4 = i & 15;
      *reinterpret_cast<float4*>(&s.x[r * GT_XLD + 4 * c4]) =
          __ldg(reinterpret_cast<const float4*>(x_down + (size_t)(base + r) * 64) + c4);
    }
    for (int c0 = lo; c0 < hi; c0 += GT_MAXOUT) {
      if (tid == 0) s.n_out = 0;
      __syncthreads();
      for (int i = c0 + tid; i < min(hi, c0 + GT_MAXOUT); i += GT_ROWS) {
        if (i == j) continue;
        const int ib = row_ptr[i], di = row_ptr[i + 1] - ib;
        int a = 0, b = di;
        while (a < b) { const int mid = (a + b) >> 1; if (src[ib + mid] < j) a = mid + 1; else b = mid; }
        if (a < di && src[ib + a] == j) {
          int pa = 0, pb = d;
          while (pa < pb) { const int mid = (pa + pb) >> 1; if (s.in_src[mid] < i) pa = mid + 1; else pb = mid; }
          const int slot = atomicAdd(&s.n_out, 1);
          s.out_e[slot] = ib + a;
          s.out_pos[slot] = (pa < d && s.in_src[pa] == i) ? pa : d;
        }
      }
      __syncthreads();
      const int no = s.n_out;
      int u0 = 0;
      while (u0 < no) {
        if (tid == 0) {
          int rows = 0, u = u0, ns = 0;
          while (u < no && ns < GT_MAXSEG) {
            const int nt = d - (s.out_pos[u] < d ? 1 : 0);
            if (rows + nt > GT_ROWS) break;
            s.seg_row[ns] = rows; s.seg_out[ns] = u;
            rows += nt; ++ns; ++u;
          }
          s.seg_row[ns] = rows;
          s.n_seg = ns;
          s.next_u = u;
        }
        __syncthreads();
        const int ns = s.n_seg, rows = s.seg_row[ns];
        for (int sg = w; sg < ns; sg += GT_ROWS / 32)
          for (int r = s.seg_row[sg] + lane; r < s.seg_row[sg + 1]; r += 32) s.row_seg[r] = sg;
        __syncthreads();
        int srow = 0;
        {
          const int p = tid;
          float sv[8], tv[8];
#pragma unroll
          for (int i = 0; i < 8; ++i) sv[i] = tv[i] = 0.f;
          if (p < rows) {
            const int sg = s.row_seg[p], u = s.seg_out[sg], r = p - s.seg_row[sg];
            const int pos_i = s.out_pos[u];
            srow = r + (r >= pos_i ? 1 : 0);
            const size_t t = (size_t)trip_ptr[s.out_e[u]] + r;
            const float4 a0 = __ldg(reinterpret_cast<const float4*>(sbf_p + t * 8));
            const float4 a1 = __ldg(reinterpret_cast<const float4*>(sbf_p + t * 8) + 1);
            sv[0] = a0.x; sv[1] = a0.y; sv[2] = a0.z; sv[3] = a0.w; sv[4] = a1.x; sv[5] = a1.y; sv[6] = a1.z; sv[7] = a1.w;
            if (TORSION) {
              const float4 b0 = __ldg(reinterpret_cast<const float4*>(t_p + t * 8));
              const float4 b1 = __ldg(reinterpret_cast<const float4*>(t_p + t * 8) + 1);
              tv[0] = b0.x; tv[1] = b0.y; tv[2] = b0.z; tv[3] = b0.w; tv[4] = b1.x; tv[5] = b1.y; tv[6] = b1.z; tv[7] = b1.w;
            }
          }
          uint32_t h[4], l[4];
#pragma unroll
          for (int i = 0; i < 4; ++i) {
// ... 23 lines not shown
        __syncthreads();
        {
          const float scale = TORSION ? 1.0f / (GT_SS * GT_SW * GT_SS * GT_SW) : 1.0f / (GT_SS * GT_SW);
          const uint64_t dwh = smem_desc(smem_u32(s.ws_hi), 64 * 16, 128), dwl = smem_desc(smem_u32(s.ws_lo), 64 * 16, 128);
          const uint64_t dvh = smem_desc(smem_u32(s.wt_hi), 64 * 16, 128), dvl = smem_desc(smem_u32(s.wt_lo), 64 * 16, 128);
#pragma unroll 1
          for (int mh = 0; mh < 2; ++mh) {
            const uint32_t mo = (uint32_t)(mh * 64 * 16);
            float gs[32], gt[32];
            wg_fence();
            const uint64_t dsh = smem_desc(smem_u32(s.s_hi) + mo, GT_ROWS * 16, 128), dsl = smem_desc(smem_u32(s.s_lo) + mo, GT_ROWS * 16, 128);
            mma_f16(gs, dsl, dwh, 0);
            mma_f16(gs, dsh, dwl, 1);
            mma_f16(gs, dsh, dwh, 1);
            if (TORSION) {
              const uint64_t dth = smem_desc(smem_u32(s.t_hi) + mo, GT_ROWS * 16, 128), dtl = smem_desc(smem_u32(s.t_lo) + mo, GT_ROWS * 16, 128);
              mma_f16(gt, dtl, dvh, 0);
              mma_f16(gt, dth, dvl, 1);
              mma_f16(gt, dth, dvh, 1);
            }
            wg_commit();
            wg_wait0();
#pragma unroll
            for (int h = 0; h < 2; ++h) {
              const int r = 64 * mh + frag_row(tid) + 8 * h;
              const float* xr = &s.x[s.row_src[r] * GT_XLD];
#pragma unroll
              for (int j = 0; j < 8; ++j)
#pragma unroll
                for (int e = 0; e < 2; ++e) {
                  const int cc = 8 * j + frag_col(tid) + e, i = 4 * j + 2 * h + e;
                  float y = (xr[cc] * scale) * gs[i];
                  if (TORSION) y *= gt[i];
                  s.y[r * GT_YLD + cc] = y;
                }
            }
          }
        }
        __syncthreads();
        for (int sg = w; sg < ns; sg += GT_ROWS / 32) {
          const int r0 = s.seg_row[sg], r1 = s.seg_row[sg + 1];
          float a0 = 0.f, a1 = 0.f;
          for (int r = r0; r < r1; ++r) { a0 += s.y[r * GT_YLD + lane]; a1 += s.y[r * GT_YLD + lane + 32]; }
          const size_t e = (size_t)s.out_e[s.seg_out[sg]];
          m[e * 64 + lane] = a0;
          m[e * 64 + lane + 32] = a1;
        }
        u0 = s.next_u;
        __syncthreads();
      }
    }
  }
}

static int h_smem_attr(const void* fn);
template <int NPANEL, int KU, int N>
static int launch_linear_h16(const float* x, int64_t rows, int ldx, const unsigned char* packed, const float* bias,
                             float* y, float* act_out, const float* residual, int ldy, int slices, cudaStream_t st) {
  HLinParams P;
  const size_t panel = (size_t)(KU / 4) * 2 * 4 * N * 16;
  for (int p = 0; p < NPANEL; ++p) P.g[p] = {packed + p * panel, nullptr, KU * 8, N};
  auto kfn = linear_h16_kernel<NPANEL, KU, N>;
  int rc = h_smem_attr((const void*)kfn);
  if (rc) return rc;
  int dev = 0, n_sm = 132;
  cudaGetDevice(&dev);
  cudaDeviceGetAttribute(&n_sm, cudaDevAttrMultiProcessorCount, dev);
  const int tiles = ceil_div(rows, H_M);
  const int tpc = (ceil_div(tiles, 2) * slices < n_sm) ? 1 : 2;
  dim3 grid(ceil_div(tiles, tpc), slices);
  kfn<<<grid, H_THREADS, sizeof(HSmem), st>>>(x, (int)rows, ldx, P, bias, y, act_out, residual, ldy, tpc,
                                              4 * N * (NPANEL * KU * 8));
  return DIG3D_OK;
}

static int h_smem_attr(const void* fn) {
  cudaError_t e = cudaFuncSetAttribute(fn, cudaFuncAttributeMaxDynamicSharedMemorySize, (int)sizeof(HSmem));
  if (e != cudaSuccess) {
    set_error("cudaFuncSetAttribute(%zu): %s", sizeof(HSmem), cudaGetErrorString(e));
    return DIG3D_ECUDA;
  }
  return DIG3D_OK;
}

}

using namespace dig3d;

extern "C" {

int64_t dig3d_h16_packed_bytes(int32_t n, int32_t k) { return (int64_t)4 * n * k; }

static int h16_pack_impl(const float* const* weights, const int32_t* n, const int32_t* k, const int32_t* trans,
                         void* const* outs, int32_t count, void* stream) {
  DIG3D_REQUIRE(weights && n && k && outs && count >= 1 && count <= 16, "h16_pack: bad arguments");
  HPackJobs jobs;
  int max_total = 0;
  for (int i = 0; i < count; ++i) {
    DIG3D_REQUIRE(weights[i] && outs[i] && k[i] % 64 == 0 && n[i] % 8 == 0 && n[i] <= 128,
                  "h16_pack: matrix %d has N=%d K=%d (need K %% 64 == 0, N %% 8 == 0, N <= 128)", i, n[i], k[i]);
    jobs.job[i] = {weights[i], (unsigned char*)outs[i], n[i], k[i], trans ? trans[i] : 0};
    max_total = max_total > n[i] * k[i] ? max_total : n[i] * k[i];
  }
  dim3 grid(ceil_div(max_total, 256), count);
  h16_pack_kernel<<<grid, 256, 0, (cudaStream_t)stream>>>(jobs);
  DIG3D_LAUNCH_CHECK();
  return DIG3D_OK;
}

int dig3d_h16_pack(const float* const* weights, const int32_t* n, const int32_t* k, void* const* outs, int32_t count,
                   void* stream) {
  return h16_pack_impl(weights, n, k, nullptr, outs, count, stream);
}

int dig3d_h16_pack_t(const float* const* weights, const int32_t* n, const int32_t* k, const int32_t* trans,
                     void* const* outs, int32_t count, void* stream) {
  DIG3D_REQUIRE(trans, "h16_pack_t: null pointer");
  return h16_pack_impl(weights, n, k, trans, outs, count, stream);
}

int dig3d_h16_set_fast_swish(int32_t on) {
  h16_fast_swish = on ? 1 : 0;
  return DIG3D_OK;
}

int dig3d_h16_set_wide_epilogue(int32_t on) {
  (void)on;
  return DIG3D_OK;
}

int dig3d_h16_overflow(int32_t clear) {
  unsigned int v = 0;
  cudaMemcpyFromSymbol(&v, g_h16_overflow, sizeof(v));
  if (clear && v) {
    unsigned int zero = 0;
    cudaMemcpyToSymbol(g_h16_overflow, &zero, sizeof(zero));
  }
  return (int)v;
}

int dig3d_h16_trace(int32_t on, long long* out128 ) {
  if (out128) cudaMemcpyFromSymbol(out128, g_h16_trace, sizeof(long long) * 128);
  int v = on ? 1 : 0;
  cudaMemcpyToSymbol(g_h16_trace_on, &v, sizeof(v));
  return DIG3D_OK;
}

int dig3d_h16_timeouts(void) {
  unsigned int v = 0;
  cudaMemcpyFromSymbol(&v, tc90::g_mbar_timeout, sizeof(v));
  return (int)v;
}

int dig3d_sphere_init_e_h16(const int64_t* z, const int32_t* src, const int32_t* dst, const float* rbf0,
                            int64_t n_edges, const dig3d_init_e_weights* w, const void* packed_lin, float* e1,
                            float* v_in, void* stream) {
  DIG3D_REQUIRE(z && src && dst && rbf0 && w && packed_lin && e1 && v_in, "sphere_init_e_h16: null pointer");
  DIG3D_REQUIRE(w->emb && w->w_rbf0 && w->b_rbf0 && w->b_lin && w->w_rbf1, "sphere_init_e_h16: null weight");
  if (n_edges == 0) return DIG3D_OK;
  HInitParams P;
  const size_t panel = (size_t)4 * 2 * 4 * 128 * 16;
  for (int p = 0; p < 3; ++p) P.g[p] = {(const unsigned char*)packed_lin + p * panel, nullptr, 128, 128};
  P.emb = w->emb; P.w_rbf0 = w->w_rbf0; P.b_rbf0 = w->b_rbf0; P.b_lin = w->b_lin; P.w_rbf1 = w->w_rbf1;
  P.tab_i = P.tab_j = nullptr;
  auto kfn = h16_fast_swish ? sphere_init_e_h16_kernel<true, false> : sphere_init_e_h16_kernel<false, false>;
  int rc = h_smem_attr((const void*)kfn);
  if (rc) return rc;
  const int pairs = ceil_div(ceil_div(n_edges, H_M), 2);
  kfn<<<pairs, H_THREADS, sizeof(HSmem), (cudaStream_t)stream>>>(z, src, dst, rbf0, (int)n_edges, P, e1, v_in);
  DIG3D_LAUNCH_CHECK();
  return DIG3D_OK;
}

int dig3d_sphere_init_e_h16_tab(const int64_t* z, const int32_t* src, const int32_t* dst, const float* rbf0,
                                int64_t n_edges, const dig3d_init_e_weights* w, const void* packed_rbf_panel,
                                const float* tab_i, const float* tab_j, float* e1, float* v_in, void* stream) {
  DIG3D_REQUIRE(z && src && dst && rbf0 && w && packed_rbf_panel && tab_i && tab_j && e1 && v_in,
                "sphere_init_e_h16_tab: null pointer");
  DIG3D_REQUIRE(w->w_rbf0 && w->b_rbf0 && w->b_lin && w->w_rbf1, "sphere_init_e_h16_tab: null weight");
  DIG3D_REQUIRE((((uintptr_t)tab_i | (uintptr_t)tab_j) & 15) == 0, "sphere_init_e_h16_tab: tables must be 16-byte aligned");
  if (n_edges == 0) return DIG3D_OK;
  HInitParams P;
  P.g[0] = {(const unsigned char*)packed_rbf_panel, nullptr, 128, 128};
  P.g[1] = P.g[2] = P.g[0];
  P.emb = w->emb; P.w_rbf0 = w->w_rbf0; P.b_rbf0 = w->b_rbf0; P.b_lin = w->b_lin; P.w_rbf1 = w->w_rbf1;
  P.tab_i = tab_i; P.tab_j = tab_j;
  auto kfn = h16_fast_swish ? sphere_init_e_h16_kernel<true, true> : sphere_init_e_h16_kernel<false, true>;
  int rc = h_smem_attr((const void*)kfn);
  if (rc) return rc;
  const int pairs = ceil_div(ceil_div(n_edges, H_M), 2);
  kfn<<<pairs, H_THREADS, sizeof(HSmem), (cudaStream_t)stream>>>(z, src, dst, rbf0, (int)n_edges, P, e1, v_in);
  DIG3D_LAUNCH_CHECK();
  return DIG3D_OK;
}

int dig3d_sphere_update_e_a_h16(const float* e1, const float* rbf0, int64_t n_edges, const dig3d_tc_update_e* w,
                                float* x_ji, float* x_down, void* stream) {
  DIG3D_REQUIRE(e1 && rbf0 && w && x_ji && x_down, "sphere_update_e_a_h16: null pointer");
  if (n_edges == 0) return DIG3D_OK;
  REParams P = {};
  P.g[0] = {(const unsigned char*)w->p_ji, w->b_ji, 128, 128};
  P.g[1] = {(const unsigned char*)w->p_kj, w->b_kj, 128, 128};
  P.g[2] = {(const unsigned char*)w->p_down, nullptr, 128, 64};
  P.w_rbf1 = w->w_rbf1; P.w_rbf2 = w->w_rbf2;
  P.x_ji = x_ji; P.x_down = x_down;
  return launch_update_e_h16<RE_A>(nullptr, nullptr, e1, rbf0, nullptr, n_edges, P, nullptr, nullptr,
                                   (cudaStream_t)stream);
}

static void update_e_b_params(REParams& P, const dig3d_tc_update_e* w) {
  P.g[0] = {(const unsigned char*)w->p_up, nullptr, 64, 128};
  for (int i = 0; i < 2; ++i) P.g[1 + i] = {(const unsigned char*)w->p_res[i], w->b_res[i], 128, 128};
  P.g[3] = {(const unsigned char*)w->p_lin, w->b_lin, 128, 128};
  for (int i = 2; i < 6; ++i) P.g[2 + i] = {(const unsigned char*)w->p_res[i], w->b_res[i], 128, 128};
  P.w_rbf = w->w_rbf;
}

int dig3d_sphere_update_e_b_h16(const float* m, const float* e1_in, const float* x_ji, const float* rbf0,
                                const int32_t* dst, int64_t n_edges, const dig3d_tc_update_e* w, float* e1_out,
                                float* v_in, void* stream) {
  DIG3D_REQUIRE(m && e1_in && x_ji && rbf0 && dst && w && e1_out && v_in, "sphere_update_e_b_h16: null pointer");
  if (n_edges == 0) return DIG3D_OK;
  REParams P = {};
  update_e_b_params(P, w);
  return launch_update_e_h16<RE_B>(m, x_ji, e1_in, rbf0, dst, n_edges, P, e1_out, v_in, (cudaStream_t)stream);
}

int dig3d_sphere_update_e_ba_h16(const float* m, const float* e1_in, const float* x_ji, const float* rbf0,
                                 const int32_t* dst, int64_t n_edges, const dig3d_tc_update_e* w,
                                 const dig3d_tc_update_e* w_next, float* e1_out, float* v_in, float* x_ji_next,
                                 float* x_down_next, void* stream) {
  DIG3D_REQUIRE(m && e1_in && x_ji && rbf0 && dst && w && w_next && e1_out && v_in && x_ji_next && x_down_next,
                "sphere_update_e_ba_h16: null pointer");
  DIG3D_REQUIRE(x_ji_next != x_ji, "sphere_update_e_ba_h16: x_ji_next must not alias x_ji (other units still read it)");
  if (n_edges == 0) return DIG3D_OK;
  REParams P = {};
  update_e_b_params(P, w);
  P.g[8] = {(const unsigned char*)w_next->p_ji, w_next->b_ji, 128, 128};
  P.g[9] = {(const unsigned char*)w_next->p_kj, w_next->b_kj, 128, 128};
  P.g[10] = {(const unsigned char*)w_next->p_down, nullptr, 128, 64};
  P.w_rbf1 = w_next->w_rbf1; P.w_rbf2 = w_next->w_rbf2;
  P.x_ji = x_ji_next; P.x_down = x_down_next;
  return launch_update_e_h16<RE_BA>(m, x_ji, e1_in, rbf0, dst, n_edges, P, e1_out, v_in, (cudaStream_t)stream);
}

int dig3d_sphere_triplet_gather_tc(const float* x_down, const float* sbf_p, const float* t_p, int32_t ld_p,
                                   const int32_t* src, const int32_t* row_ptr, const int32_t* trip_ptr,
                                   const int32_t* graph_ptr, const int64_t* batch, int64_t n_nodes, int32_t cap,
                                   const float* w_sbf2, const float* w_t2, float* m, void* stream) {
  DIG3D_REQUIRE(x_down && sbf_p && src && row_ptr && trip_ptr && graph_ptr && batch && w_sbf2 && m,
                "sphere_triplet_gather_tc: null pointer");
  DIG3D_REQUIRE((t_p != nullptr) == (w_t2 != nullptr), "sphere_triplet_gather_tc: t_p and w_t2 must agree");
  DIG3D_REQUIRE(ld_p == 8, "sphere_triplet_gather_tc: expects the layer-major [T, 8] slices (ld_p == 8), got %d", ld_p);
  DIG3D_REQUIRE(cap >= 1 && cap <= GT_MAXIN, "sphere_triplet_gather_tc: cap=%d outside [1,%d]", cap, GT_MAXIN);
  DIG3D_REQUIRE((((uintptr_t)x_down | (uintptr_t)sbf_p | (uintptr_t)t_p) & 15) == 0, "sphere_triplet_gather_tc: 16-byte alignment");
  if (n_nodes == 0) return DIG3D_OK;
  cudaStream_t st = (cudaStream_t)stream;
  int dev = 0, n_sm = 132;
  cudaGetDevice(&dev);
  cudaDeviceGetAttribute(&n_sm, cudaDevAttrMultiProcessorCount, dev);
  const int grid = (int)(n_nodes < 2 * n_sm ? n_nodes : 2 * n_sm);
  cudaError_t e;
  if (t_p) {
    e = cudaFuncSetAttribute(sphere_triplet_gather_tc_kernel<true>, cudaFuncAttributeMaxDynamicSharedMemorySize, (int)sizeof(GTSmem));
    if (e == cudaSuccess)
      sphere_triplet_gather_tc_kernel<true><<<grid, GT_ROWS, sizeof(GTSmem), st>>>(
          x_down, sbf_p, t_p, src, row_ptr, trip_ptr, graph_ptr, batch, (int)n_nodes, w_sbf2, w_t2, m);
  } else {
    e = cudaFuncSetAttribute(sphere_triplet_gather_tc_kernel<false>, cudaFuncAttributeMaxDynamicSharedMemorySize, (int)sizeof(GTSmem));
    if (e == cudaSuccess)
      sphere_triplet_gather_tc_kernel<false><<<grid, GT_ROWS, sizeof(GTSmem), st>>>(
          x_down, sbf_p, t_p, src, row_ptr, trip_ptr, graph_ptr, batch, (int)n_nodes, w_sbf2, w_t2, m);
  }
  if (e != cudaSuccess) { set_error("sphere_triplet_gather_tc: %s", cudaGetErrorString(e)); return DIG3D_ECUDA; }
  DIG3D_LAUNCH_CHECK();
  return DIG3D_OK;
}

int dig3d_linear_h16_supported(int32_t k, int32_t nout) {
  return ((k == 64 || k == 128 || k == 256 || k == 384) && nout >= 64 && nout % 64 == 0 && nout <= 512) ? 1 : 0;
}

int dig3d_linear_h16(const float* x, int64_t rows, int32_t k, int32_t nout, const void* packed, const float* bias,
                     float* y, float* act_out, const float* residual, void* stream) {
  DIG3D_REQUIRE(x && packed && (y || act_out), "linear_h16: null pointer");
  DIG3D_REQUIRE(dig3d_linear_h16_supported(k, nout), "linear_h16: shape %d -> %d is not compiled", k, nout);
  DIG3D_REQUIRE((((uintptr_t)x | (uintptr_t)y | (uintptr_t)act_out | (uintptr_t)residual) & 15) == 0,
                "linear_h16: 16-byte alignment");
  if (rows == 0) return DIG3D_OK;
  cudaStream_t st = (cudaStream_t)stream;
  const unsigned char* pw = (const unsigned char*)packed;
  for (int c0 = 0; c0 < nout;) {
    const int n = nout - c0 >= 128 ? 128 : 64;
    const int slices = n == 128 ? (nout - c0) / 128 : 1;
    const float* b = bias ? bias + c0 : nullptr;
    float* yo = y ? y + c0 : nullptr;
    float* ao = act_out ? act_out + c0 : nullptr;
    const float* ro = residual ? residual + c0 : nullptr;
    int rc;
#define DIG3D_LIN(NP, KU)                                                                                             \
    (n == 128 ? launch_linear_h16<NP, KU, 128>(x, rows, k, pw, b, yo, ao, ro, nout, slices, st)                        \
              : launch_linear_h16<NP, KU, 64>(x, rows, k, pw, b, yo, ao, ro, nout, slices, st))
    if (k == 64) rc = DIG3D_LIN(1, 8);
    else if (k == 128) rc = DIG3D_LIN(1, 16);
    else if (k == 256) rc = DIG3D_LIN(2, 16);
    else rc = DIG3D_LIN(3, 16);
#undef DIG3D_LIN
    if (rc) return rc;
    pw += (size_t)4 * n * k * slices;
    c0 += n * slices;
  }
  DIG3D_LAUNCH_CHECK();
  return DIG3D_OK;
}

int dig3d_sphere_update_v_h16_supported(int32_t hidden, int32_t out_emb, int32_t out_channels, int32_t n_lins) {
  return (hidden == 128 && out_emb == 256 && out_channels >= 1 && out_channels <= 4 && n_lins >= 0 && n_lins <= 8) ? 1 : 0;
}

int dig3d_sphere_update_v_h16(const float* v_in_all, int64_t n_nodes, int32_t n_blocks, int32_t out_channels,
                              int32_t n_lins, const void* const* packed ,
                              const dig3d_update_v_weights* w, float* v_out_all, void* stream) {
  DIG3D_REQUIRE(v_in_all && packed && w && v_out_all, "sphere_update_v_h16: null pointer");
  DIG3D_REQUIRE(n_blocks >= 1 && n_blocks <= 8, "sphere_update_v_h16: n_blocks=%d outside [1,8]", n_blocks);
  DIG3D_REQUIRE(dig3d_sphere_update_v_h16_supported(128, 256, out_channels, n_lins),
                "sphere_update_v_h16: out_channels=%d / n_lins=%d not compiled", out_channels, n_lins);
  if (n_nodes == 0) return DIG3D_OK;
  HVParams P;
  P.n_lins = n_lins; P.out_channels = out_channels;
  for (int b = 0; b < n_blocks; ++b) {
    DIG3D_REQUIRE(w[b].n_lins == n_lins && w[b].w_out && w[b].b_up, "sphere_update_v_h16: block %d weights", b);
    for (int l = 0; l <= n_lins; ++l) {
      P.blk[b].p[l] = (const unsigned char*)packed[b * (n_lins + 1) + l];
      P.blk[b].b[l] = l == 0 ? w[b].b_up : w[b].b_lins[l - 1];
      DIG3D_REQUIRE(P.blk[b].p[l] && P.blk[b].b[l], "sphere_update_v_h16: block %d layer %d null", b, l);
    }
    P.blk[b].w_out = w[b].w_out;
  }
  auto kfn = h16_fast_swish ? sphere_update_v_h16_kernel<true> : sphere_update_v_h16_kernel<false>;
  int rc = h_smem_attr((const void*)kfn);
  if (rc) return rc;
  dim3 grid(ceil_div(n_nodes, H_M), n_blocks);
  kfn<<<grid, H_THREADS, sizeof(HSmem), (cudaStream_t)stream>>>(v_in_all, (int)n_nodes, P, v_out_all);
  DIG3D_LAUNCH_CHECK();
  return DIG3D_OK;
}

}
```

### dig_b200/csrc/wgmma.cuh

```cuda
#pragma once
#include <cuda_runtime.h>
#include <stdint.h>

namespace tc90 {

__device__ __forceinline__ uint32_t smem_u32(const void* p) { return (uint32_t)__cvta_generic_to_shared(p); }

__device__ __forceinline__ void mbar_init(uint64_t* bar, uint32_t count) {
  asm volatile("mbarrier.init.shared::cta.b64 [%0], %1;" ::"r"(smem_u32(bar)), "r"(count));
}
__device__ __forceinline__ void mbar_fence_init() { asm volatile("fence.mbarrier_init.release.cluster;" ::: "memory"); }
__device__ __forceinline__ void mbar_arrive(uint64_t* bar) {
  asm volatile("mbarrier.arrive.shared::cta.b64 _, [%0];" ::"r"(smem_u32(bar)) : "memory");
}
__device__ __forceinline__ void mbar_arrive_expect_tx(uint64_t* bar, uint32_t bytes) {
  asm volatile("mbarrier.arrive.expect_tx.shared::cta.b64 _, [%0], %1;" ::"r"(smem_u32(bar)), "r"(bytes) : "memory");
}
static __device__ unsigned int g_mbar_timeout = 0;
__device__ __forceinline__ uint64_t global_ns() {
  uint64_t t;
  asm volatile("mov.u64 %0, %%globaltimer;" : "=l"(t));
  return t;
}
__device__ __forceinline__ bool mbar_try(uint32_t addr, uint32_t parity) {
  uint32_t ok;
  asm volatile(
      "{\n\t.reg .pred p;\n\t"
      "mbarrier.try_wait.parity.shared::cta.b64 p, [%1], %2;\n\t"
      "selp.u32 %0, 1, 0, p;\n\t}"
      : "=r"(ok)
      : "r"(addr), "r"(parity)
      : "memory");
  return ok != 0;
}
static __device__ __noinline__ void mbar_timeout_trap() {
  atomicAdd(&g_mbar_timeout, 1u);
  __threadfence_system();
  __trap();
}
__device__ __forceinline__ bool mbar_wait(uint64_t* bar, uint32_t parity) {
  const uint32_t addr = smem_u32(bar);
  if (mbar_try(addr, parity)) return true;
  const uint64_t t0 = global_ns();
  for (;;) {
#pragma unroll 1
    for (int spin = 0; spin < 4096; ++spin)
      if (mbar_try(addr, parity)) return true;
    if (global_ns() - t0 > 2000000000ull) break;
  }
  mbar_timeout_trap();
  return false;
}

__device__ __forceinline__ void fence_async_smem() { asm volatile("fence.proxy.async.shared::cta;" ::: "memory"); }
__device__ __forceinline__ void tc_fence_before() { asm volatile("fence.acq_rel.cta;" ::: "memory"); }
__device__ __forceinline__ void tc_fence_after() { asm volatile("fence.acq_rel.cta;" ::: "memory"); }

__device__ __forceinline__ void bulk_g2s(void* smem_dst, const void* gmem_src, uint32_t bytes, uint64_t* bar) {
  asm volatile("cp.async.bulk.shared::cluster.global.mbarrier::complete_tx::bytes [%0], [%1], %2, [%3];" ::"r"(
                   smem_u32(smem_dst)),
               "l"(gmem_src), "r"(bytes), "r"(smem_u32(bar))
               : "memory");
}

__device__ __forceinline__ void wg_bar(int id = 15) { asm volatile("bar.sync %0, 128;" ::"r"(id) : "memory"); }

__device__ __forceinline__ uint64_t smem_desc(uint32_t saddr, uint32_t lbo_bytes, uint32_t sbo_bytes) {
  uint64_t d = 0;
  d |= (uint64_t)((saddr & 0x3FFFF) >> 4);
  d |= (uint64_t)((lbo_bytes >> 4) & 0x3FFF) << 16;
  d |= (uint64_t)((sbo_bytes >> 4) & 0x3FFF) << 32;
  return d;
}
__device__ __forceinline__ void wg_fence() { asm volatile("wgmma.fence.sync.aligned;" ::: "memory"); }
__device__ __forceinline__ void wg_commit() { asm volatile("wgmma.commit_group.sync.aligned;" ::: "memory"); }
__device__ __forceinline__ void wg_wait0() { asm volatile("wgmma.wait_group.sync.aligned 0;" ::: "memory"); }

#define TC90_D32 "{%0,%1,%2,%3,%4,%5,%6,%7,%8,%9,%10,%11,%12,%13,%14,%15," \
                 "%16,%17,%18,%19,%20,%21,%22,%23,%24,%25,%26,%27,%28,%29,%30,%31}"
#define TC90_D32_OPS(d)                                                                                          \
  "+f"(d[0]), "+f"(d[1]), "+f"(d[2]), "+f"(d[3]), "+f"(d[4]), "+f"(d[5]), "+f"(d[6]), "+f"(d[7]), "+f"(d[8]),   \
      "+f"(d[9]), "+f"(d[10]), "+f"(d[11]), "+f"(d[12]), "+f"(d[13]), "+f"(d[14]), "+f"(d[15]), "+f"(d[16]),    \
      "+f"(d[17]), "+f"(d[18]), "+f"(d[19]), "+f"(d[20]), "+f"(d[21]), "+f"(d[22]), "+f"(d[23]), "+f"(d[24]),   \
      "+f"(d[25]), "+f"(d[26]), "+f"(d[27]), "+f"(d[28]), "+f"(d[29]), "+f"(d[30]), "+f"(d[31])

__device__ __forceinline__ void mma_f16(float (&d)[32], uint64_t a_desc, uint64_t b_desc, uint32_t accumulate) {
  asm volatile(
      "{\n\t.reg .pred p;\n\t"
      "setp.ne.b32 p, %34, 0;\n\t"
      "wgmma.mma_async.sync.aligned.m64n64k16.f32.f16.f16 " TC90_D32 ", %32, %33, p, 1, 1, 0, 0;\n\t}"
      : TC90_D32_OPS(d)
      : "l"(a_desc), "l"(b_desc), "r"(accumulate)
      : "memory");
}
__device__ __forceinline__ void mma_tf32(float (&d)[32], uint64_t a_desc, uint64_t b_desc, uint32_t accumulate) {
  asm volatile(
      "{\n\t.reg .pred p;\n\t"
      "setp.ne.b32 p, %34, 0;\n\t"
      "wgmma.mma_async.sync.aligned.m64n64k8.f32.tf32.tf32 " TC90_D32 ", %32, %33, p, 1, 1;\n\t}"
      : TC90_D32_OPS(d)
      : "l"(a_desc), "l"(b_desc), "r"(accumulate)
      : "memory");
}
__device__ __forceinline__ int frag_row(int wt) { return 16 * (wt >> 5) + ((wt & 31) >> 2); }
__device__ __forceinline__ int frag_col(int wt) { return 2 * (wt & 3); }

__device__ __forceinline__ constexpr int frag_a_src(int s, int r) { return 8 * s + 2 * r; }
__device__ __forceinline__ int frag_a_row(int wt, int r) { return frag_row(wt) + 8 * (r & 1); }
__device__ __forceinline__ int frag_a_col(int wt, int s, int r) { return 16 * s + 8 * (r >> 1) + frag_col(wt); }

#define TC90_D64 "{%0,%1,%2,%3,%4,%5,%6,%7,%8,%9,%10,%11,%12,%13,%14,%15,"                                          \
                 "%16,%17,%18,%19,%20,%21,%22,%23,%24,%25,%26,%27,%28,%29,%30,%31,"                                  \
                 "%32,%33,%34,%35,%36,%37,%38,%39,%40,%41,%42,%43,%44,%45,%46,%47,"                                  \
                 "%48,%49,%50,%51,%52,%53,%54,%55,%56,%57,%58,%59,%60,%61,%62,%63}"
#define TC90_D64_OPS(d)                                                                                          \
  TC90_D32_OPS(d), "+f"(d[32]), "+f"(d[33]), "+f"(d[34]), "+f"(d[35]), "+f"(d[36]), "+f"(d[37]), "+f"(d[38]),    \
      "+f"(d[39]), "+f"(d[40]), "+f"(d[41]), "+f"(d[42]), "+f"(d[43]), "+f"(d[44]), "+f"(d[45]), "+f"(d[46]),    \
      "+f"(d[47]), "+f"(d[48]), "+f"(d[49]), "+f"(d[50]), "+f"(d[51]), "+f"(d[52]), "+f"(d[53]), "+f"(d[54]),    \
      "+f"(d[55]), "+f"(d[56]), "+f"(d[57]), "+f"(d[58]), "+f"(d[59]), "+f"(d[60]), "+f"(d[61]), "+f"(d[62]),    \
      "+f"(d[63])

__device__ __forceinline__ void mma_f16_rs(float (&d)[32], const uint32_t (&a)[4], uint64_t b_desc, uint32_t accumulate) {
  asm volatile(
      "{\n\t.reg .pred p;\n\t"
      "setp.ne.b32 p, %37, 0;\n\t"
      "wgmma.mma_async.sync.aligned.m64n64k16.f32.f16.f16 " TC90_D32 ", {%32,%33,%34,%35}, %36, p, 1, 1, 0;\n\t}"
      : TC90_D32_OPS(d)
      : "r"(a[0]), "r"(a[1]), "r"(a[2]), "r"(a[3]), "l"(b_desc), "r"(accumulate)
      : "memory");
}
__device__ __forceinline__ void mma_f16_rs(float (&d)[64], const uint32_t (&a)[4], uint64_t b_desc, uint32_t accumulate) {
  asm volatile(
      "{\n\t.reg .pred p;\n\t"
      "setp.ne.b32 p, %69, 0;\n\t"
      "wgmma.mma_async.sync.aligned.m64n128k16.f32.f16.f16 " TC90_D64 ", {%64,%65,%66,%67}, %68, p, 1, 1, 0;\n\t}"
      : TC90_D64_OPS(d)
      : "r"(a[0]), "r"(a[1]), "r"(a[2]), "r"(a[3]), "l"(b_desc), "r"(accumulate)
      : "memory");
}

#ifdef TC90_TM_COLS
constexpr int TM_COLS = TC90_TM_COLS;
constexpr int TM_SLOTS = 144;
constexpr int TM_SLOT_SHIFT = 23;
static __device__ float g_tm_store[(size_t)TM_SLOTS * 128 * TM_COLS];
static __device__ unsigned int g_tm_owner[TM_SLOTS];
constexpr size_t TM_ONE_CTA_PER_SM_SMEM = 114 * 1024;

__device__ __forceinline__ float* tm_ptr(uint32_t taddr, int lane_add) {
  const uint32_t slot = taddr >> TM_SLOT_SHIFT, row = ((taddr >> 16) & 127u) + (uint32_t)lane_add;
  return g_tm_store + ((size_t)slot * 128 + row) * TM_COLS + (taddr & 0xFFFFu);
}
__device__ __forceinline__ void tmem_alloc(uint32_t* smem_holder, uint32_t) {
  if ((threadIdx.x & 31) == 0) {
    uint32_t sm;
    asm volatile("mov.u32 %0, %%smid;" : "=r"(sm));
    const uint64_t t0 = global_ns();
    for (uint32_t i = sm;; ++i) {
      const uint32_t slot = i % TM_SLOTS;
      if (atomicCAS(&g_tm_owner[slot], 0u, 1u) == 0u) {
        __threadfence();
        *smem_holder = slot << TM_SLOT_SHIFT;
        break;
      }
      if ((i & 1023) == 1023 && global_ns() - t0 > 2000000000ull) mbar_timeout_trap();
    }
  }
  __syncwarp();
}
__device__ __forceinline__ void tmem_dealloc(uint32_t taddr, uint32_t) {
  if ((threadIdx.x & 31) == 0) {
    __threadfence();
    atomicExch(&g_tm_owner[taddr >> TM_SLOT_SHIFT], 0u);
  }
  __syncwarp();
}
__device__ __forceinline__ void tmem_ld16(uint32_t taddr, uint32_t (&r)[16]) {
  const float4* p = reinterpret_cast<const float4*>(tm_ptr(taddr, threadIdx.x & 31));
#pragma unroll
  for (int i = 0; i < 4; ++i) {
    const float4 v = __ldcg(p + i);
    r[4 * i] = __float_as_uint(v.x); r[4 * i + 1] = __float_as_uint(v.y);
    r[4 * i + 2] = __float_as_uint(v.z); r[4 * i + 3] = __float_as_uint(v.w);
  }
}
__device__ __forceinline__ void tmem_ld16f(uint32_t taddr, float* r) {
  const float4* p = reinterpret_cast<const float4*>(tm_ptr(taddr, threadIdx.x & 31));
#pragma unroll
  for (int i = 0; i < 4; ++i) {
    const float4 v = __ldcg(p + i);
    r[4 * i] = v.x; r[4 * i + 1] = v.y; r[4 * i + 2] = v.z; r[4 * i + 3] = v.w;
  }
}
__device__ __forceinline__ void tmem_ld_wait() {}
__device__ __forceinline__ void tmem_st16(uint32_t taddr, const uint32_t (&r)[16]) {
  float4* p = reinterpret_cast<float4*>(tm_ptr(taddr, threadIdx.x & 31));
#pragma unroll
  for (int i = 0; i < 4; ++i)
    __stcg(p + i, make_float4(__uint_as_float(r[4 * i]), __uint_as_float(r[4 * i + 1]), __uint_as_float(r[4 * i + 2]),
                              __uint_as_float(r[4 * i + 3])));
}
__device__ __forceinline__ void tmem_st_wait() {}

__device__ __forceinline__ void tm_store_frag(const float (&d)[32], int wt, uint32_t taddr) {
  float* base = tm_ptr(taddr, frag_row(wt)) + frag_col(wt);
#pragma unroll
  for (int j = 0; j < 8; ++j) {
    __stcg(reinterpret_cast<float2*>(base + 8 * j), make_float2(d[4 * j], d[4 * j + 1]));
    __stcg(reinterpret_cast<float2*>(base + 8 * TM_COLS + 8 * j), make_float2(d[4 * j + 2], d[4 * j + 3]));
  }
}
#endif

__device__ __forceinline__ float tf32_rna(float x) {
  uint32_t u;
  asm("cvt.rna.tf32.f32 %0, %1;" : "=r"(u) : "f"(x));
  return __uint_as_float(u);
}
__device__ __forceinline__ void split_tf32(float x, float& hi, float& lo) {
  hi = tf32_rna(x);
  lo = tf32_rna(x - hi);
}

}
```

### dig_b200/threedgraph/method/dimenet_family.py

```python
import os
from math import sqrt

import torch
from torch import nn

from ... import autograd as ag
from ... import autograd_jvp as jv
from ... import ops
from ...basis import envelope_coefficients
from ._common import ResidualLayer, glorot_orthogonal, require_cuda, swish, wants_grad

_SUPPORTED = dict(hidden_channels=128, int_emb_size=64, out_emb_channels=256, num_radial=6,
                  num_before_skip=1, num_after_skip=2)


class dist_emb(nn.Module):

    def __init__(self, num_radial, cutoff=5.0, envelope_exponent=5):
        super().__init__()
        self.cutoff = cutoff
        self.envelope_exponent = envelope_exponent
        self.freq = nn.Parameter(torch.Tensor(num_radial))
        self.reset_parameters()

# ... 182 lines not shown
        out = super().load_state_dict(*args, **kw)
        self.invalidate_packed()
        return out

    def train(self, mode=True):
        self.invalidate_packed()
        return super().train(mode)

    def _projection_rows(self, first, count):
        def rows(name):
            ws = [getattr(self.update_es[l], name).weight.detach() for l in range(first, first + count)]
            w = torch.cat(ws, 0)
            if w.size(0) < 32:
                w = torch.cat([w, w.new_zeros(32 - w.size(0), w.size(1))], 0)
            return w.contiguous()
        return rows("lin_sbf1"), (rows("lin_t1") if self._torsion else None)

    def forward(self, batch_data):
        z, pos, batch = batch_data.z, batch_data.pos, batch_data.batch
        require_cuda(pos, type(self).__name__ + ".forward")
        if self.energy_and_force:
            pos.requires_grad_()
        ns, nr = self.num_spherical, self.num_radial
        with_emb = self.init_e.use_node_features
        g = ops.build_graph(pos, batch, self.cutoff, num_graphs=getattr(batch_data, "num_graphs", None),
                            z=z if with_emb else None, z_rows=self.init_e.emb.num_embeddings if with_emb else 0)
        if wants_grad(self) or self._generic:
            nf = getattr(batch_data, "node_feature", None)
            if (self.training and torch.is_grad_enabled() and pos.requires_grad
                    and any(p.requires_grad for p in self.parameters())):
                return jv.energy_with_force(lambda p: self._exact(self._forward_train, z, p, g, nf),
                                            lambda p, c: self._exact(self._forward_dual, z, p, c, g, nf),
                                            pos, tuple(self.parameters()))
            return self._exact(self._forward_train, z, pos, g, nf, exact=bool(pos.requires_grad))
        ops.h16_wide_from_env()
        if (os.environ.get("DIG3D_DENSE", "h16") == "h16" and g.n_edges and self.num_layers <= 4
                and os.environ.get("DIG3D_LEAN", "1") != "0"):
            plan = self._inference_plan()
            if plan is not None:
                return self._forward_lean(plan, z, pos, g)
        ops.triplet_geometry(g, pos, use_torsion=self._torsion, want_idx=False)
        rbf0, bess = ops.edge_basis(g.dist, self.cutoff, self.envelope_exponent, self.emb.dist_emb.freq,
                                    self._basis_id, envelope_on_bessel=not self._torsion, num_radial=nr,
                                    n_bessel=ns * nr)
        L = self.num_layers
        proj = []
        for first in range(0, L, 4):
            w_s, w_t = self._projection_rows(first, min(4, L - first))
            proj.append(ops.triplet_basis_project(g, bess, self._basis_id, w_s, w_t))

        dev = pos.device
        v_in_all = torch.zeros(L + 1, g.n_nodes, self.hidden_channels, dtype=torch.float32, device=dev)
        v_all = torch.empty(L + 1, g.n_nodes, self.out_channels, dtype=torch.float32, device=dev)
        dense = os.environ.get("DIG3D_DENSE", "h16")
        if dense not in ("h16", "tc", "simt"):
            raise ValueError(f"DIG3D_DENSE={dense!r}: expected h16, tc or simt")
        tc_cache = self.__dict__.setdefault("_tc_cache", {})
        if dense == "h16":
            packed = ops.tc_pack_matrix(self.init_e.lin.weight, tc_cache, "init_e.lin", kind="h16")
            tables = (ops.init_e_tables(self.init_e, tc_cache)
                      if os.environ.get("DIG3D_INIT_TABLES", "1") != "0" and self.hidden_channels == 128 else None)
            e1, _ = ops.sphere_init_e_h16(z, g, rbf0, ops.pack_init_e(self.init_e), packed, self.hidden_channels,
                                          v_in=v_in_all[0], tables=tables)
        elif dense == "tc":
            packed = ops.tc_pack_matrix(self.init_e.lin.weight, tc_cache, "init_e.lin")
            e1, _ = ops.sphere_init_e_tc(z, g, rbf0, ops.pack_init_e(self.init_e), packed, self.hidden_channels,
                                         v_in=v_in_all[0])
        else:
            e1, _ = ops.sphere_init_e(z, g, rbf0, ops.pack_init_e(self.init_e), self.hidden_channels,
                                      v_in=v_in_all[0])
        for l in range(L):
            sbf_p, t_p = proj[l // 4]
            if dense == "h16":
                wt = ops.tc_pack_update_e(self.update_es[l], self._torsion, tc_cache, kind="h16")
                e1, _, _, _ = ops.sphere_update_e_h16(e1, g, rbf0, sbf_p, t_p, 8 * (l % 4), wt,
                                                      self.hidden_channels, self.int_emb_size, v_in=v_in_all[l + 1])
            elif dense == "tc":
                wt = ops.tc_pack_update_e(self.update_es[l], self._torsion, tc_cache)
                e1, _, _, _ = ops.sphere_update_e_tc(e1, g, rbf0, sbf_p, t_p, 8 * (l % 4), wt,
                                                     self.hidden_channels, self.int_emb_size, v_in=v_in_all[l + 1])
            else:
                e1, _ = ops.sphere_update_e(e1, g, rbf0, sbf_p, t_p, 8 * (l % 4),
                                            ops.pack_update_e(self.update_es[l], self._torsion),
                                            self.hidden_channels, self.int_emb_size, v_in=v_in_all[l + 1])
        holders = [self.init_v] + list(self.update_vs)
        if dense == "h16" and ops.update_v_h16_supported(self.init_v, self.out_channels):
            ops.sphere_update_v_h16(v_in_all, holders, self.out_channels, v_all, tc_cache)
        else:
            ops.sphere_update_v_batched(v_in_all, holders, self.out_channels, v_all)
        return ops.graph_readout(v_all, g.graph_ptr, g.n_graphs, g.n_nodes)


    def _inference_plan(self):
        tables = os.environ.get("DIG3D_INIT_TABLES", "1")
        key = ops.plan_key(self, tables)
        plan = self.__dict__.get("_plan")
        if plan is not None and plan["key"] == key:
            return plan
        key = ops.plan_key_refresh(self, tables)
        holders = [self.init_v] + list(self.update_vs)
        if not ops.update_v_h16_supported(self.init_v, self.out_channels):
            return None
        tc_cache = self.__dict__.setdefault("_tc_cache", {})
        L = self.num_layers
        w_s, w_t = self._projection_rows(0, L)
        parr, varr, n_lins = ops.pack_update_v_h16(holders, tc_cache)
        plan = {
            "key": key,
            "init_w": ops.pack_init_e(self.init_e),
            "init_packed": ops.tc_pack_matrix(self.init_e.lin.weight, tc_cache, "init_e.lin", kind="h16"),
            "init_tables": (ops.init_e_tables(self.init_e, tc_cache)
                            if os.environ.get("DIG3D_INIT_TABLES", "1") != "0" and self.hidden_channels == 128 else None),
            "layers": [ops.tc_pack_update_e(self.update_es[l], self._torsion, tc_cache, kind="h16") for l in range(L)],
            "w_s": w_s, "w_t": w_t, "parr": parr, "varr": varr, "n_lins": n_lins,
            "freq": self.emb.dist_emb.freq.detach(),
            "emb_rows": self.init_e.emb.num_embeddings if self.init_e.use_node_features else 0,
        }
        self.__dict__["_plan"] = plan
        return plan

    def _forward_lean(self, plan, z, pos, g):
        import ctypes
        call, byref = ops.call, ctypes.byref
        tors = self._torsion
        E, T, N, L = g.n_edges, g.n_triplets, g.n_nodes, self.num_layers
        H, I, O = self.hidden_channels, self.int_emb_size, self.out_channels
        nb_s = self.num_spherical * self.num_radial
        dev = pos.device
        sizes = (("angle", T), ("torsion", T if tors else 0), ("rbf0", E * self.num_radial), ("bess", E * nb_s),
                 ("sbf_p", 32 * T), ("t_p", 32 * T if tors else 0), ("e1a", E * H), ("e1b", E * H), ("x_ji", E * H),
                 ("x_ji2", E * H), ("x_down", E * I), ("m", E * I), ("v_all", (L + 1) * N * O))
        off, total = {}, 0
        for name, n in sizes:
            off[name] = total
            total += (n + 63) & ~63
        ws = torch.empty(total + 64, dtype=torch.float32, device=dev)
        base = (ws.data_ptr() + 255) & ~255
        a = {name: base + 4 * o for name, o in off.items()}
        v_in_all = torch.zeros(L + 1, N, H, dtype=torch.float32, device=dev)
        v_in = v_in_all.data_ptr()
        st = ops._stream()
        src, dst, row_ptr, trip_ptr = g.src.data_ptr(), g.dst.data_ptr(), g.row_ptr.data_ptr(), g.trip_ptr.data_ptr()
        graph_ptr, batch = g.graph_ptr.data_ptr(), ops._p(g.batch, torch.int64, "batch")
        pos_p = ops._p(pos.detach(), torch.float32, "pos")
        if T:
            call("dig3d_triplet_geometry", pos_p, src, dst, row_ptr, trip_ptr, E, int(tors), a["angle"],
                 a["torsion"] if tors else None, None, None, None, None, st)
        call("dig3d_edge_basis", g.dist.data_ptr(), E, float(self.cutoff), int(self.envelope_exponent),
             ops._p(plan["freq"], torch.float32, "freq"), int(self._basis_id), int(not tors), a["rbf0"], a["bess"], st)
        if T:
            call("dig3d_triplet_basis_project_lists", a["bess"], a["angle"], a["torsion"] if tors else None, src, dst,
                 row_ptr, trip_ptr, graph_ptr, batch, E, T, int(self._basis_id), 4, 8, plan["w_s"].data_ptr(),
                 plan["w_t"].data_ptr() if tors else None, a["sbf_p"], a["t_p"] if tors else None, *ops._out_lists(g), st)
        if plan["init_tables"] is not None:
            tab_i, tab_j, packed_rbf = plan["init_tables"]
            call("dig3d_sphere_init_e_h16_tab", ops._p(z, torch.int64, "z"), src, dst, a["rbf0"], E, byref(plan["init_w"]),
                 packed_rbf.data_ptr(), tab_i.data_ptr(), tab_j.data_ptr(), a["e1a"], v_in, st)
        else:
            call("dig3d_sphere_init_e_h16", ops._p(z, torch.int64, "z"), src, dst, a["rbf0"], E, byref(plan["init_w"]),
                 plan["init_packed"].data_ptr(), a["e1a"], v_in, st)
        fuse = os.environ.get("DIG3D_FUSE_BA", "1") != "0"
        e1, e1_next = a["e1a"], a["e1b"]
        x_ji, x_ji_next = a["x_ji"], a["x_ji2"]
        for l in range(L):
            w = plan["layers"][l]
            if l == 0 or not fuse:
                call("dig3d_sphere_update_e_a_h16", e1, a["rbf0"], E, byref(w), x_ji, a["x_down"], st)
            sp = ctypes.c_void_p(a["sbf_p"] + 4 * 8 * T * l)
            tp = ctypes.c_void_p(a["t_p"] + 4 * 8 * T * l) if tors else None
            ops.triplet_gather(a["x_down"], sp, tp, g, w.w_sbf2, w.w_t2, a["m"], st)
            if fuse and l + 1 < L:
                call("dig3d_sphere_update_e_ba_h16", a["m"], e1, x_ji, a["rbf0"], dst, E, byref(w),
                     byref(plan["layers"][l + 1]), e1_next, v_in + 4 * (l + 1) * N * H, x_ji_next, a["x_down"], st)
                x_ji, x_ji_next = x_ji_next, x_ji
            else:
                call("dig3d_sphere_update_e_b_h16", a["m"], e1, x_ji, a["rbf0"], dst, E, byref(w), e1_next,
                     v_in + 4 * (l + 1) * N * H, st)
            e1, e1_next = e1_next, e1
        call("dig3d_sphere_update_v_h16", v_in, N, L + 1, int(O), plan["n_lins"], plan["parr"], plan["varr"], a["v_all"], st)
        u = torch.empty(g.n_graphs, O, dtype=torch.float32, device=dev)
        if g.n_graphs:
            call("dig3d_graph_readout", a["v_all"], graph_ptr, g.n_graphs, N, L + 1, O, u.data_ptr(), st)
        return u

    @staticmethod
    def _exact(fn, *args, exact=True):
        ag.EXACT_BACKWARD[0] = exact
        try:
            return fn(*args)
        finally:
            ag.EXACT_BACKWARD[0] = False

    def _update_v_train(self, mods, e2_list, g):
        v = torch.stack([ag.segment_sum(e2, g.row_ptr, g.dst) for e2 in e2_list])
        v = ag.grouped_lin([m.lin_up for m in mods], v)
        for j in range(len(mods[0].lins)):
            v = ag.grouped_lin([m.lins[j] for m in mods], v, act=True)
        return ag.grouped_lin([m.lin for m in mods], v)

    def _forward_train(self, z, pos, g, node_feature=None):
        ns, nr = self.num_spherical, self.num_radial
        ops.triplet_geometry(g, pos, use_torsion=self._torsion, want_idx=False)
        tors_angle = None
        if pos.requires_grad:
            if self._torsion:
                dist, angle, tors_angle = ag.geometry(pos, g, 3)
            else:
                dist, angle = ag.geometry(pos, g, 2)
        else:
            dist, angle = g.dist, g.angle
        geo_cfg = (self.cutoff, self.envelope_exponent, not self._torsion, dist)
        rbf0, bess = ag.edge_basis(self.emb.dist_emb.freq, dist, self.cutoff, self.envelope_exponent,
                                   self._basis_id, not self._torsion, nr, ns * nr)
        L = self.num_layers
        sbf_ps, t_ps = [], []
        sbf = tbf = None
        if self._triplet_generic:
            if pos.requires_grad:
                raise NotImplementedError(
                    f"{type(self).__name__}: forces with non-default int_emb_size / basis_emb_size_angle / _torsion are not "
                    "built (the materialised-basis path carries no geometry gradient)")
            ops.triplet_geometry(g, pos, use_torsion=self._torsion, want_idx=True)
            sbf, tbf = ops.triplet_basis(bess, g.angle, g.torsion, g.idx_kj, self._basis_id, ns, nr, self._torsion)
        else:
            for first in range(0, L, 4):
                es = self.update_es[first:first + 4]
                s_l, t_l = ag.basis_project(g, bess, dist, angle, tors_angle, geo_cfg, self._basis_id, ns, nr,
                                            [m.lin_sbf1.weight for m in es],
                                            [m.lin_t1.weight for m in es] if self._torsion else None)
                sbf_ps += s_l
                t_ps += t_l if t_l is not None else [None] * len(s_l)
        swish_, lin = ag.swish, ag.lin
        ie = self.init_e
        if ie.use_node_features:
            x = ag.gather_rows(ie.emb.weight, z)
        else:
            x = ag.gather_rows(ie.node_embedding.view(1, -1), torch.zeros_like(z))
        if self.use_extra_node_feature and node_feature is not None:
            x = torch.cat([x, lin(self.extra_emb, node_feature.to(torch.float32).contiguous())], dim=1)
        r0 = ag.lin_swish(ie.lin_rbf_0, rbf0)
        cat = torch.cat([ag.gather_rows(x, g.dst, g.row_ptr), ag.gather_rows(x, g.src), r0], dim=-1)
        e1 = ag.lin_swish(ie.lin, cat)
        e2 = ag.mul(lin(ie.lin_rbf_1, rbf0), e1)
        e2_list = [e2]
        for l, (ue, uv) in enumerate(zip(self.update_es, self.update_vs)):
            x_ji = ag.lin_swish(ue.lin_ji, e1)
            x_kj = ag.lin_swish(ue.lin_kj, e1)
            x_kj = ag.mul(x_kj, lin(ue.lin_rbf2, lin(ue.lin_rbf1, rbf0)))
            x_kj = ag.lin_swish(ue.lin_down, x_kj)
            if self._triplet_generic:
                prod = ag.mul(ag.gather_rows(x_kj, g.idx_kj), lin(ue.lin_sbf2, lin(ue.lin_sbf1, sbf)))
                if self._torsion:
                    prod = ag.mul(prod, lin(ue.lin_t2, lin(ue.lin_t1, tbf)))
                x_kj = ag.segment_sum(prod, g.trip_ptr, g.idx_ji)
            else:
                x_kj = ag.triplet_gather(x_kj, sbf_ps[l], t_ps[l], ue.lin_sbf2.weight,
                                         ue.lin_t2.weight if self._torsion else None, g)
            x_kj = ag.lin_swish(ue.lin_up, x_kj)
            h = ag.add(x_ji, x_kj)
            for layer in ue.layers_before_skip:
                h = ag.add(h, ag.lin_swish(layer.lin2, ag.lin_swish(layer.lin1, h)))
            h = ag.add(ag.lin_swish(ue.lin, h), e1)
            for layer in ue.layers_after_skip:
                h = ag.add(h, ag.lin_swish(layer.lin2, ag.lin_swish(layer.lin1, h)))
            e1 = h
            e2_list.append(ag.mul(lin(ue.lin_rbf, rbf0), e1))
        v = self._update_v_train([self.init_v] + list(self.update_vs), e2_list, g)
        u = ag.segment_sum(v[0], g.graph_ptr, g.batch)
        for l in range(1, v.size(0)):
            u = ag.add(u, ag.segment_sum(v[l], g.graph_ptr, g.batch))
        return u


    def _forward_dual(self, z, pos, cvec, g, node_feature=None):
        ns, nr = self.num_spherical, self.num_radial
        tors = self._torsion
        pos = pos.detach()
        ops.triplet_geometry(g, pos, use_torsion=tors, want_idx=True)
        d_dot, a_dot, t_dot = ops.geometry_jvp(pos, cvec, g, want_angle=True, want_torsion=tors)
        dist, angle, tors_angle = g.dist.view(-1), g.angle.view(-1), (g.torsion.view(-1) if tors else None)
        freq = self.emb.dist_emb.freq
        cfg = (self.cutoff, self.envelope_exponent, self._basis_id, not tors, nr, ns * nr)
        rbf0, bess = ag.edge_basis(freq, dist, *cfg)
        rbf0_d = jv.edge_basis_tangent(freq, dist, d_dot, *cfg)
        _, bess_d = ops.edge_basis_tangent(dist, d_dot, self.cutoff, self.envelope_exponent, None, self._basis_id,
                                           not tors, nr, ns * nr, want_rbf0=False, want_bess=True)
        sbf_d, tbf_d = ops.triplet_basis_tangent(bess, bess_d, angle, a_dot, tors_angle, t_dot, g.idx_kj,
                                                 self._basis_id, ns, nr, want_tbf=tors)
        geo_cfg = (self.cutoff, self.envelope_exponent, not tors, dist)
        L = self.num_layers
        sbf_ps, t_ps = [], []
        for first in range(0, L, 4):
            es = self.update_es[first:first + 4]
            s_l, t_l = ag.basis_project(g, bess, dist, angle, tors_angle, geo_cfg, self._basis_id, ns, nr,
                                        [m.lin_sbf1.weight for m in es],
                                        [m.lin_t1.weight for m in es] if tors else None)
            sbf_ps += s_l
            t_ps += t_l if t_l is not None else [None] * len(s_l)
        lin, lsd, muld, addd = ag.lin, jv.lin_swish_dual, jv.mul_dual, jv.add_dual
        ie = self.init_e
        if ie.use_node_features:
            x = ag.gather_rows(ie.emb.weight, z)
        else:
            x = ag.gather_rows(ie.node_embedding.view(1, -1), torch.zeros_like(z))
        if self.use_extra_node_feature and node_feature is not None:
            x = torch.cat([x, lin(self.extra_emb, node_feature.to(torch.float32).contiguous())], dim=1)
        r0, r0_d = lsd(ie.lin_rbf_0, rbf0, rbf0_d)
        xi, xj = ag.gather_rows(x, g.dst, g.row_ptr), ag.gather_rows(x, g.src)
        cat = torch.cat([xi, xj, r0], dim=-1)
        cat_d = torch.cat([torch.zeros_like(xi), torch.zeros_like(xj), r0_d], dim=-1)
        e1, e1_d = lsd(ie.lin, cat, cat_d)
        e2, e2_d = muld(*jv.lin_dual(ie.lin_rbf_1, rbf0, rbf0_d), e1, e1_d)
        e2s = [(e2, e2_d)]
        for l, ue in enumerate(self.update_es):
            x_ji, x_ji_d = lsd(ue.lin_ji, e1, e1_d)
            x_kj, x_kj_d = lsd(ue.lin_kj, e1, e1_d)
            rb, rb_d = jv.lin_dual(ue.lin_rbf2, *jv.lin_dual(ue.lin_rbf1, rbf0, rbf0_d))
            x_kj, x_kj_d = muld(x_kj, x_kj_d, rb, rb_d)
            x_kj, x_kj_d = lsd(ue.lin_down, x_kj, x_kj_d)
# ... 54 lines not shown
```

### include/dig3d.h

```cpp
#ifndef DIG3D_H
#define DIG3D_H
#include <stdint.h>
#ifdef __cplusplus
extern "C" {
#endif

#define DIG3D_OK 0
#define DIG3D_EINVAL (-1)
#define DIG3D_ECUDA (-2)
#define DIG3D_EUNSUPPORTED (-3)

const char* dig3d_last_error(void);
int dig3d_abi_version(void);


int dig3d_knn2(const float* pos, const int64_t* batch, const int32_t* graph_ptr, int64_t n_nodes, int64_t n_graphs,
               int32_t* nn1, int32_t* nn2, void* stream);
int dig3d_triplet_geometry_knn(const float* pos, const int32_t* src, const int32_t* dst, const int32_t* row_ptr,
                               const int32_t* trip_ptr, int64_t n_edges, const int32_t* nn1, const int32_t* nn2,
                               float* angle, float* torsion, int64_t* idx_kj64, int64_t* idx_ji64, void* stream);

int dig3d_graph_ptr(const int64_t* batch, int64_t n_nodes, int64_t n_graphs, int32_t* ptr, void* stream);

int dig3d_radius_neighbors(const float* pos, const int64_t* batch, const int32_t* ptr, int64_t n_nodes,
// ... 20 lines not shown
                    int32_t* trip_ptr, void* stream);

int dig3d_edge_fill_out(const float* pos, const int32_t* nbr, const int32_t* deg, const int32_t* row_ptr,
                        const int32_t* node_trip_ptr, int64_t n_nodes, int32_t cap, int64_t n_edges,
                        int64_t* edge_index, int32_t* src, int32_t* dst, float* dist, float* vec,
                        int32_t* trip_ptr, const int32_t* graph_ptr, const int64_t* batch, const int32_t* out_ptr,
                        int32_t* out_list, int32_t* pos_in, void* stream);

int dig3d_edges_to_csr(const float* pos, const int64_t* edge_index, int64_t n_edges, int64_t n_nodes, int32_t* src,
                       int32_t* dst, int32_t* row_ptr, int32_t* cnt_ws, int32_t* trip_ptr, float* dist,
                       int32_t* flags, void* stream);

int dig3d_triplet_geometry(const float* pos, const int32_t* src, const int32_t* dst, const int32_t* row_ptr,
                           const int32_t* trip_ptr, int64_t n_edges, int32_t use_torsion, float* angle,
                           float* torsion, int32_t* idx_kj, int32_t* idx_ji, int64_t* idx_kj64,
                           int64_t* idx_ji64, void* stream);

int dig3d_edge_basis(const float* dist, int64_t n_edges, double cutoff, int32_t envelope_exponent,
                     const float* freq, int32_t basis_id, int32_t envelope_on_bessel, float* rbf0,
                     float* bess, void* stream);
int dig3d_edge_basis_set_split(int32_t on);

int dig3d_triplet_basis(const float* bess, const float* angle, const float* torsion, const int32_t* idx_kj,
                        int64_t n_triplets, int32_t basis_id, float* sbf, float* tbf, void* stream);

int dig3d_triplet_basis_project(const float* bess, const float* angle, const float* torsion,
                                const int32_t* src, const int32_t* dst, const int32_t* row_ptr,
                                const int32_t* trip_ptr, const int32_t* graph_ptr, const int64_t* batch,
                                int64_t n_edges, int64_t n_triplets, int32_t basis_id, int32_t n_layers,
                                int32_t basis_emb, const float* w_sbf1, const float* w_t1, float* sbf_p,
                                float* t_p, void* stream);
int dig3d_triplet_basis_project_lists(const float* bess, const float* angle, const float* torsion,
                                      const int32_t* src, const int32_t* dst, const int32_t* row_ptr,
                                      const int32_t* trip_ptr, const int32_t* graph_ptr, const int64_t* batch,
                                      int64_t n_edges, int64_t n_triplets, int32_t basis_id, int32_t n_layers,
                                      int32_t basis_emb, const float* w_sbf1, const float* w_t1, float* sbf_p,
                                      float* t_p, const int32_t* out_ptr, const int32_t* out_list,
                                      const int32_t* pos_in, void* stream);
int dig3d_triplet_basis_project_set_mode(int32_t mode);
int dig3d_triplet_basis_project_node(const float* bess, const float* angle, const float* torsion, const int32_t* src,
                                     const int32_t* row_ptr, const int32_t* trip_ptr, const int32_t* graph_ptr,
                                     const int64_t* batch, int64_t n_nodes, int64_t n_triplets, int32_t cap,
                                     int32_t basis_id, int32_t n_layers, int32_t basis_emb, const float* w_sbf1,
                                     const float* w_t1, float* sbf_p, float* t_p, void* stream);

int dig3d_segment_sum(const float* x, const int32_t* ptr, int64_t n_segments, int64_t width, float* out,
                      void* stream);

typedef struct {
  const float* emb;
  const float* w_rbf0;
  const float* b_rbf0;
  const float* w_lin;
  const float* b_lin;
  const float* w_rbf1;
} dig3d_init_e_weights;

typedef struct {
  const float *w_rbf1, *w_rbf2;
  const float *w_sbf2, *w_t2;
  const float *w_rbf;
  const float *w_kj, *b_kj, *w_ji, *b_ji;
  const float *w_down, *w_up;
  const float *w_res[6], *b_res[6];
  const float *w_lin, *b_lin;
} dig3d_update_e_weights;

typedef struct {
  const float *w_up, *b_up;
  const float *w_lins[8], *b_lins[8];
  const float *w_out;
  int32_t n_lins;
} dig3d_update_v_weights;

int dig3d_sphere_init_e(const int64_t* z, const int32_t* src, const int32_t* dst, const float* rbf0,
                        int64_t n_edges, const dig3d_init_e_weights* w, float* e1, float* v_in,
                        void* stream);

int dig3d_sphere_update_e_a(const float* e1, const float* rbf0, int64_t n_edges,
                            const dig3d_update_e_weights* w, float* x_ji, float* x_down, void* stream);

int dig3d_sphere_update_e_b(const float* e1_in, const float* x_ji, const float* x_down, const float* rbf0,
                            const float* sbf_p, const float* t_p, int32_t ld_p, const int32_t* src,
                            const int32_t* dst, const int32_t* row_ptr, const int32_t* trip_ptr,
                            int64_t n_edges, const dig3d_update_e_weights* w, float* e1_out, float* v_in,
                            void* stream);

int dig3d_sphere_update_v(const float* v_in, int64_t n_nodes, int32_t out_channels,
                          const dig3d_update_v_weights* w, float* v_out, void* stream);

int dig3d_sphere_update_v_batched(const float* v_in_all, int64_t n_nodes, int32_t n_blocks, int32_t out_channels,
                                  const dig3d_update_v_weights* w, float* v_out_all, void* stream);

int dig3d_graph_readout(const float* v, const int32_t* graph_ptr, int64_t n_graphs, int64_t n_nodes,
                        int32_t n_blocks, int32_t channels, float* u, void* stream);

int dig3d_tc_packed_floats(int32_t n, int32_t k);
int dig3d_tc_pack(const float* const* weights, const int32_t* n, const int32_t* k, float* const* outs,
                  int32_t count, void* stream);
int dig3d_tc_timeouts(void);

typedef struct {
  const float *p_ji, *b_ji, *p_kj, *b_kj;
  const float *p_down, *p_up;
  const float *p_res[6], *b_res[6];
  const float *p_lin, *b_lin;
  const float *w_rbf1, *w_rbf2, *w_rbf;
  const float *w_sbf2, *w_t2;
} dig3d_tc_update_e;

int dig3d_sphere_init_e_tc(const int64_t* z, const int32_t* src, const int32_t* dst, const float* rbf0,
                           int64_t n_edges, const dig3d_init_e_weights* w, const float* packed_lin, float* e1,
                           float* v_in, void* stream);
int dig3d_sphere_update_e_a_tc(const float* e1, const float* rbf0, int64_t n_edges, const dig3d_tc_update_e* w,
                               float* x_ji, float* x_down, void* stream);
int dig3d_sphere_triplet_gather(const float* x_down, const float* sbf_p, const float* t_p, int32_t ld_p,
                                const int32_t* src, const int32_t* dst, const int32_t* row_ptr,
                                const int32_t* trip_ptr, int64_t n_edges, const float* w_sbf2, const float* w_t2,
                                float* m, void* stream);
int dig3d_sphere_triplet_gather_node(const float* x_down, const float* sbf_p, const float* t_p, int32_t ld_p,
                                     const int32_t* src, const int32_t* row_ptr, const int32_t* trip_ptr,
                                     const int32_t* graph_ptr, const int64_t* batch, int64_t n_nodes, int32_t cap,
                                     const float* w_sbf2, const float* w_t2, float* m, void* stream);
int dig3d_sphere_triplet_gather_warp(const float* x_down, const float* sbf_p, const float* t_p, int32_t ld_p,
                                     const int32_t* src, const int32_t* row_ptr, const int32_t* trip_ptr,
                                     const int32_t* graph_ptr, const int64_t* batch, int64_t n_nodes, int32_t cap,
                                     int32_t split, const float* w_sbf2, const float* w_t2, float* m,
                                     const int32_t* out_ptr, const int32_t* out_list, const int32_t* pos_in,
                                     void* stream);
int dig3d_sphere_update_e_b_tc(const float* m, const float* e1_in, const float* x_ji, const float* rbf0,
                               const int32_t* dst, int64_t n_edges, const dig3d_tc_update_e* w, float* e1_out,
                               float* v_in, void* stream);
int dig3d_tc_trace(int32_t on, long long* out64);
int dig3d_tc_set_fast_swish(int32_t on);

int64_t dig3d_h16_packed_bytes(int32_t n, int32_t k);
int dig3d_h16_pack(const float* const* weights, const int32_t* n, const int32_t* k, void* const* outs, int32_t count,
                   void* stream);
int dig3d_sphere_init_e_h16(const int64_t* z, const int32_t* src, const int32_t* dst, const float* rbf0,
                            int64_t n_edges, const dig3d_init_e_weights* w, const void* packed_lin, float* e1,
                            float* v_in, void* stream);
int dig3d_sphere_init_e_h16_tab(const int64_t* z, const int32_t* src, const int32_t* dst, const float* rbf0,
                                int64_t n_edges, const dig3d_init_e_weights* w, const void* packed_rbf_panel,
                                const float* tab_i, const float* tab_j, float* e1, float* v_in, void* stream);
int dig3d_sphere_update_e_a_h16(const float* e1, const float* rbf0, int64_t n_edges, const dig3d_tc_update_e* w,
                                float* x_ji, float* x_down, void* stream);
int dig3d_sphere_update_e_b_h16(const float* m, const float* e1_in, const float* x_ji, const float* rbf0,
                                const int32_t* dst, int64_t n_edges, const dig3d_tc_update_e* w, float* e1_out,
                                float* v_in, void* stream);
int dig3d_sphere_update_e_ba_h16(const float* m, const float* e1_in, const float* x_ji, const float* rbf0,
                                 const int32_t* dst, int64_t n_edges, const dig3d_tc_update_e* w,
                                 const dig3d_tc_update_e* w_next, float* e1_out, float* v_in, float* x_ji_next,
                                 float* x_down_next, void* stream);
int dig3d_sphere_update_v_h16_supported(int32_t hidden, int32_t out_emb, int32_t out_channels, int32_t n_lins);
int dig3d_sphere_update_v_h16(const float* v_in_all, int64_t n_nodes, int32_t n_blocks, int32_t out_channels,
                              int32_t n_lins, const void* const* packed, const dig3d_update_v_weights* w,
                              float* v_out_all, void* stream);
int dig3d_sphere_triplet_gather_tc(const float* x_down, const float* sbf_p, const float* t_p, int32_t ld_p,
                                   const int32_t* src, const int32_t* row_ptr, const int32_t* trip_ptr,
                                   const int32_t* graph_ptr, const int64_t* batch, int64_t n_nodes, int32_t cap,
                                   const float* w_sbf2, const float* w_t2, float* m, void* stream);
int dig3d_h16_pack_t(const float* const* weights, const int32_t* n, const int32_t* k, const int32_t* trans,
                     void* const* outs, int32_t count, void* stream);
int dig3d_linear_h16_supported(int32_t k, int32_t nout);
int dig3d_linear_h16(const float* x, int64_t rows, int32_t k, int32_t nout, const void* packed, const float* bias,
                     float* y, float* act_out, const float* residual, void* stream);
int dig3d_h16_overflow(int32_t clear);
int dig3d_h16_timeouts(void);
int dig3d_h16_trace(int32_t on, long long* out128);
int dig3d_h16_set_fast_swish(int32_t on);
int dig3d_h16_set_wide_epilogue(int32_t on);

typedef struct {
  const float *w_lin;
  const float *w_mlp0, *b_mlp0;
  const float *w_mlp2, *b_mlp2;
  const float *w_v1, *b_v1;
  const float *w_v2, *b_v2;
} dig3d_schnet_block_weights;

int dig3d_schnet_block(const float* v, int64_t n_nodes, const float* dist, const int32_t* src,
                       const int32_t* dst, int64_t n_edges, const float* offset, int32_t n_gauss, double coeff,
                       double cutoff, int32_t hidden, int32_t filters, const dig3d_schnet_block_weights* w,
                       float* vlin, float* agg, float* v_out, void* stream);

int dig3d_schnet_readout(const float* v, int64_t n_nodes, int32_t hidden, const float* w1, const float* b1,
                         const float* w2, const float* b2, int32_t out_channels, float* node_out, void* stream);

int dig3d_comenet_geometry(const float* pos, const float* dist, const int32_t* src, const int32_t* dst,
                           const int32_t* row_ptr, const int32_t* graph_ptr, const int64_t* batch,
                           int64_t n_nodes, int64_t n_edges, double cutoff, int32_t* refs, float* feature1,
                           float* feature2, float* angles, void* stream);

int dig3d_pbc_edge_vectors(const float* pos, const int64_t* edge_index, const float* cell, const float* cell_offsets,
                           const int32_t* edge_graph, int64_t n_edges, float* vec, float* dist, void* stream);
int dig3d_comenet_geometry_edges(const float* vec, const float* dist, const int64_t* edge_index, const int32_t* src,
                                 const int32_t* dst, int64_t n_nodes, int64_t n_edges, double cutoff, int32_t* refs,
                                 unsigned long long* keys, float* feature1, float* feature2, float* angles,
                                 void* stream);

int dig3d_radius_graph_pbc_count(const float* pos, const float* cell, const int64_t* natoms, int64_t n_atoms,
                                 int64_t n_graphs, double radius, int32_t max_num_neighbors, int32_t* graph_ptr,
                                 int32_t* counts, uint32_t* select, int32_t* row_ptr, int64_t* info,
                                 int64_t* n_edges_host, void* stream);
int dig3d_radius_graph_pbc_fill(const float* pos, const float* cell, int64_t n_atoms, int64_t n_graphs, double radius,
                                const int32_t* graph_ptr, const uint32_t* select, const int32_t* row_ptr,
                                const int64_t* info, int64_t n_edges, int64_t* edge_index, float* cell_offsets,
                                int64_t* neighbors, void* stream);

int dig3d_comenet_embed(const int64_t* z, const float* emb, int64_t n_nodes, float* x, void* stream);

typedef struct {
  const float *w_lin, *b_lin;
  const float *w_f1a, *w_f1b;
  const float *w_f2a, *w_f2b;
  const float *w_rel1, *b_rel1, *w_root1;
  const float *w_rel2, *b_rel2, *w_root2;
  const float *w_lin1, *b_lin1, *w_lin2, *b_lin2;
  const float *w_cat, *b_cat;
  const float *w_lins[8], *b_lins[8];
  const float *norm_w, *norm_b, *norm_ms;
  const float *w_final, *b_final;
  int32_t n_lins;
} dig3d_comenet_block_weights;

typedef struct {
  const float *w_lins[8], *b_lins[8];
  const float *w_out, *b_out;
  int32_t n_lins;
} dig3d_comenet_head_weights;

int dig3d_comenet_block(const float* x_in, const float* feature1, const float* feature2, const int32_t* src,
                        const int32_t* dst, const int32_t* graph_ptr, const int64_t* batch, int64_t n_nodes,
                        int64_t n_edges, int64_t n_graphs, const dig3d_comenet_block_weights* w,
                        const dig3d_comenet_head_weights* head, int32_t out_channels, float* xs, float* agg1,
                        float* agg2, float* h, float* stats, float* x_out, float* node_out, void* stream);
int dig3d_edge_weighted_sum(const float* w, const float* x, const int32_t* src, const int32_t* row_ptr, int64_t n_nodes,
                            int32_t width, float* out, void* stream);
int dig3d_comenet_filter_sum(const float* feat, int32_t q, const float* weff_t, const float* x, const int32_t* src,
                             const int32_t* row_ptr, int64_t n_nodes, int32_t width, float* out, void* stream);

int dig3d_linear(const float* x, int64_t rows, int32_t k, int32_t nout, const float* w, const float* bias, float* y,
                 float* act_out , int32_t groups, void* stream);
int dig3d_wgrad(const float* dy, const float* x, int64_t rows, int32_t nout, int32_t k, float* dw, float* db,
                int32_t groups, void* stream);
int dig3d_wgrad_tc(const float* dy, const float* x, int64_t rows, int32_t nout, int32_t k, float* dw, float* db,
                   int32_t groups, void* stream);
int dig3d_wgrad_tc_supported(int64_t rows, int32_t nout, int32_t k);
int dig3d_wgrad_set_mode(int32_t mode);
int dig3d_wgrad_tc_timeouts(void);
int dig3d_linear_set_config(int32_t cfg);
int dig3d_act(const float* x, int64_t n, int32_t mode, float* y, void* stream);
int dig3d_act_bwd(const float* x, const float* dy, int64_t n, int32_t mode, float* dx, void* stream);
int dig3d_adam_step(float* param, const float* grad, float* exp_avg, float* exp_avg_sq, int64_t n, double lr,
                    double beta1, double beta2, double eps, double weight_decay, int64_t step, void* stream);
int dig3d_ewise(const float* a, const float* b, int64_t n, int32_t op, float* y, void* stream);
int dig3d_rowscale(const float* a, const float* s, int64_t rows, int32_t width, float* y, void* stream);
int dig3d_gather_rows(const float* x, const void* idx, int32_t idx_is_64, int64_t rows, int32_t width, float* y,
                      void* stream);
int dig3d_scatter_add_rows(const float* y, const void* idx, int32_t idx_is_64, int64_t rows, int32_t width,
                           float* out, void* stream);
int dig3d_rbf_freq_grad(const float* dist, int64_t n_edges, double cutoff, int32_t envelope_exponent,
                        const float* freq, int32_t num_radial, const float* drbf0, float* dfreq, void* stream);
int dig3d_triplet_basis_project_bwd(const float* bess, const float* angle, const float* torsion, const int32_t* src,
                                    const int32_t* dst, const int32_t* row_ptr, const int32_t* trip_ptr,
                                    const int32_t* graph_ptr, const int64_t* batch, int64_t n_edges, int64_t n_triplets,
                                    int32_t basis_id, const float* const* d_sbf_p, const float* const* d_t_p,
                                    float* dw_sbf1, float* dw_t1, void* stream);
int dig3d_sphere_triplet_gather_bwd(const float* dm, const float* x_down, const float* sbf_p, const float* t_p,
                                    const int32_t* src, const int32_t* dst, const int32_t* row_ptr,
                                    const int32_t* trip_ptr, int64_t n_edges, const float* w_sbf2, const float* w_t2,
                                    float* dx_down, float* d_sbf_p, float* d_t_p, float* dw_sbf2, float* dw_t2,
                                    void* stream);
int dig3d_graphnorm(const float* h, const int32_t* graph_ptr, int64_t n_graphs, int32_t width, const float* weight,
                    const float* bias, const float* mean_scale, double eps, float* y, float* shift, float* stdv,
                    void* stream);
int dig3d_graphnorm_bwd(const float* h, const float* dy, const int32_t* graph_ptr, int64_t n_graphs, int32_t width,
                        const float* weight, const float* mean_scale, const float* shift, const float* stdv, float* dx,
                        float* dweight, float* dbias, float* dmean_scale, void* stream);
int dig3d_edge_dist_bwd(const float* pos, const int32_t* src, const int32_t* dst, const float* dist, const float* ddist,
                        int64_t n_edges, float* dpos, void* stream);
int dig3d_triplet_angle_bwd(const float* pos, const int32_t* src, const int32_t* dst, const int32_t* row_ptr,
                            const int32_t* trip_ptr, const float* dangle, int64_t n_edges, float* dpos, void* stream);
int dig3d_edge_basis_bwd(const float* dist, int64_t n_edges, double cutoff, int32_t envelope_exponent, const float* freq,
                         int32_t basis_id, int32_t envelope_on_bessel, const float* drbf0, float* ddist, float* bess_dx,
                         void* stream);
int dig3d_triplet_basis_project_bwd_geom(const float* bess, const float* bess_dx, const float* angle,
                                         const float* torsion, const int32_t* src, const int32_t* dst,
                                         const int32_t* row_ptr, const int32_t* trip_ptr, const int32_t* graph_ptr,
                                         const int64_t* batch, int64_t n_edges, int64_t n_triplets, int32_t basis_id,
                                         const float* const* d_sbf_p, const float* const* d_t_p, const float* w_sbf1,
                                         const float* w_t1, double cutoff, float* ddist, float* dangle, float* dtorsion,
                                         void* stream);
int dig3d_triplet_torsion_bwd(const float* pos, const int32_t* src, const int32_t* dst, const int32_t* row_ptr,
                              const int32_t* trip_ptr, const float* dtorsion, int64_t n_edges, float* dpos, void* stream);
int dig3d_geometry_jvp(const float* pos, const float* cvec, const int32_t* src, const int32_t* dst,
                       const int32_t* row_ptr, const int32_t* trip_ptr, const float* dist, int64_t n_edges,
                       float* dist_dot, float* angle_dot, float* torsion_dot, void* stream);
int dig3d_edge_basis_tangent(const float* dist, const float* dist_dot, int64_t n_edges, double cutoff,
                             int32_t envelope_exponent, const float* freq, int32_t basis_id, int32_t envelope_on_bessel,
                             float* rbf0_dot, float* bess_dot, void* stream);
int dig3d_rbf_freq_grad_tangent(const float* dist, const float* dist_dot, int64_t n_edges, double cutoff,
                                int32_t envelope_exponent, const float* freq, int32_t nr, const float* g_dot,
                                float* dfreq, void* stream);
int dig3d_triplet_basis_tangent(const float* bess, const float* bess_dot, const float* angle, const float* angle_dot,
                                const float* torsion, const float* torsion_dot, const int32_t* idx_kj,
// ... 29 lines not shown
```

Baseline: 94110.

## Fuse SphereNet init edge embedding with first update-e stage A kernel

Moves the init_e computation into the persistent wgmma update-e kernel as new RE_I/RE_IA modes. With fusion enabled, init and the first layer's stage A (x_ji, x_down) run in one kernel, so e1 no longer needs a separate kernel to read it back. The old tcgen05-style init kernel is dropped, and update_v is relaunched on the persistent R-kernel layout. This saves one launch and one pass over E x 128 floats, at the cost of more code paths and register pressure in the shared kernel.

```diff
diff --git a/dig_b200/_lib.py b/dig_b200/_lib.py
--- a/dig_b200/_lib.py
+++ b/dig_b200/_lib.py
@@ -99,6 +99,8 @@
     "dig3d_sphere_update_e_a_h16": [P, P, c_int64, POINTER(TcUpdateE), P, P, P],
     "dig3d_sphere_update_e_b_h16": [P, P, P, P, P, c_int64, POINTER(TcUpdateE), P, P, P],
     "dig3d_sphere_update_e_ba_h16": [P, P, P, P, P, c_int64, POINTER(TcUpdateE), POINTER(TcUpdateE), P, P, P, P, P],
+    "dig3d_sphere_init_update_e_a_h16": [P, P, P, P, c_int64, POINTER(InitEWeights), P, P, P, POINTER(TcUpdateE), P, P,
+                                         P, P, P],
     "dig3d_sphere_update_v_h16_supported": [c_int32, c_int32, c_int32, c_int32],
     "dig3d_sphere_update_v_h16": [P, c_int64, c_int32, c_int32, c_int32, P, P, P, P],
     "dig3d_h16_pack_t": [P, P, P, P, P, c_int32, P],
diff --git a/dig_b200/csrc/spherenet_h16.cu b/dig_b200/csrc/spherenet_h16.cu
--- a/dig_b200/csrc/spherenet_h16.cu
+++ b/dig_b200/csrc/spherenet_h16.cu
@@ -29,9 +29,7 @@
   float bias[8][128];
   float wr[128 * 8];
   int dst[2][H_M];
-  int aux[2][2][H_M];
   uint64_t full[H_STAGES], empty[H_STAGES], a_ready[2], d_ready[2][2], d_free[2][2];
-  uint64_t l_done;
   uint32_t tmem_base;
 };
 static_assert(sizeof(HSmem) <= 227 * 1024, "HSmem exceeds the shared memory of an SM");
@@ -84,7 +82,6 @@
   ++it;
   if (++r.c == g[r.q].K / H_SLAB_K) { r.c = 0; if (++r.t == ntile) { r.t = 0; ++r.q; } }
 }
-template <bool SHARED_A>
 __device__ __forceinline__ void h_mma_n(HSmem& s, const HGemm* g, int ng, int ntile, uint32_t tmem) {
   const int wt = threadIdx.x;
   HRing ring = {0, 0, 0};
@@ -96,11 +93,9 @@
   for (int q = 0; q < ng; ++q) {
     const int nslab = g[q].K / H_SLAB_K, n = g[q].N;
     for (int t = 0; t < ntile; ++t) {
-      if (!SHARED_A || t == 0) {
-        mbar_wait(&s.a_ready[SHARED_A ? 0 : t], q & 1);
-        tc_fence_after();
-      }
-      const uint32_t a_hi = smem_u32(SHARED_A ? s.a[0][0] : s.a[t][0]), a_lo = smem_u32(SHARED_A ? s.a[1][0] : s.a[t][1]);
+      mbar_wait(&s.a_ready[t], q & 1);
+      tc_fence_after();
+      const uint32_t a_hi = smem_u32(s.a[t][0]), a_lo = smem_u32(s.a[t][1]);
       for (int c = 0; c < nslab; c += 2, it += 2) {
         const int ab = ch & 1;
         const int lt = ab ? last1 : last0;
@@ -144,7 +139,6 @@
         if (ab) last1 = t; else last0 = t;
         ++ch;
       }
-      if (SHARED_A && t == ntile - 1 && wt == 0) mbar_arrive(&s.l_done);
     }
   }
 }
@@ -187,15 +181,6 @@
   *reinterpret_cast<uint4*>(c.ahi + o) = make_uint4(h[0], h[1], h[2], h[3]);
   *reinterpret_cast<uint4*>(c.alo + o) = make_uint4(l[0], l[1], l[2], l[3]);
 }
-__device__ __forceinline__ void h_store_a16(HSmem& s, const HCtx& c, int col, const float (&v8)[16]) {
-  float x[8];
-#pragma unroll
-  for (int u = 0; u < 2; ++u) {
-#pragma unroll
-    for (int i = 0; i < 8; ++i) x[i] = v8[8 * u + i];
-    h_store_ku(s, c, c.row, (col >> 3) + u, x);
-  }
-}
 __device__ __forceinline__ bool h_finite(float x) { return fabsf(x) <= 3.402823466e38f; }
 template <int KU>
 __device__ __forceinline__ void h_load_tile(HSmem& s, HCtx& c, const float* __restrict__ g, size_t ld, int rows) {
@@ -281,7 +266,6 @@
       mbar_init(&s.a_ready[i], a_ready_warps);
       for (int j = 0; j < 2; ++j) { mbar_init(&s.d_ready[i][j], 1); mbar_init(&s.d_free[i][j], d_free_warps); }
     }
-    mbar_init(&s.l_done, 1);
     mbar_fence_init();
   }
   if ((threadIdx.x >> 5) == 0) tmem_alloc(&s.tmem_base, 512);
@@ -292,24 +276,6 @@
   __syncthreads();
   if ((threadIdx.x >> 5) == 0) tmem_dealloc(s.tmem_base, 512);
 }
-template <int W>
-__device__ __forceinline__ void h_store_tile_coalesced(HSmem& s, const HCtx& c, int col0, const float (&v)[W / 2],
-                                                       float* __restrict__ out, int rows) {
-  constexpr int LD = W + 1, RPW = 128 / W;
-  float* st = reinterpret_cast<float*>(s.a[c.t][0]);
-#pragma unroll
-  for (int i = 0; i < W / 2; ++i) st[c.row * LD + col0 + i] = v[i];
-  h_tile_bar(c.t);
-  const int w = c.et >> 5, lane = c.et & 31;
-  for (int r0 = w * RPW; r0 < rows; r0 += H_TILE_WARPS * RPW) {
-    const int r = r0 + (RPW == 2 ? (lane >> 4) : 0), c4 = 4 * (RPW == 2 ? (lane & 15) : lane);
-    if (r < rows) {
-      const float* src = st + r * LD + c4;
-      *reinterpret_cast<float4*>(out + (size_t)r * W + c4) = make_float4(src[0], src[1], src[2], src[3]);
-    }
-  }
-}
-
 template <int W>
 __device__ __forceinline__ void h_store_tile_strided(HSmem& s, const HCtx& c, int col0, const float (&v)[W / 2],
                                                      float* __restrict__ out, int ld, int rows,
@@ -332,26 +298,6 @@
       *reinterpret_cast<float4*>(out + (size_t)r * ld + c4) = o;
     }
   }
-}
-
-__device__ __forceinline__ void h_segment_sums(const HSmem& s, const HCtx& c, int rows, float* __restrict__ v_in) {
-  const int col = c.et & 127, r0 = (c.et >> 7) * 64, r1 = min(rows, r0 + 64);
-  if (r0 >= r1) return;
-  const float* e2t = reinterpret_cast<const float*>(s.a[c.t][0]);
-  const int* dst = s.dst[c.t];
-  float run = 0.f;
-  int cur = dst[r0];
-  bool first = true;
-  for (int r = r0; r < r1; ++r) {
-    const int d = dst[r];
-    if (d != cur) {
-      if (first) atomicAdd(v_in + (size_t)cur * 128 + col, run);
-      else v_in[(size_t)cur * 128 + col] = run;
-      first = false; run = 0.f; cur = d;
-    }
-    run += e2t[r * H_LDS + col];
-  }
-  atomicAdd(v_in + (size_t)cur * 128 + col, run);
 }
 
 struct HPackJob { const float* w; unsigned char* out; int N, K, trans; };
@@ -394,12 +340,16 @@
 };
 static_assert(sizeof(RSmem) <= 227 * 1024, "RSmem exceeds the shared memory of an SM");
 
-enum { RE_B = 0, RE_BA = 1, RE_A = 2 };
+enum { RE_B = 0, RE_BA = 1, RE_A = 2, RE_I = 3, RE_IA = 4 };
 struct REParams {
   HGemm g[11];
   const float* w_rbf;
   const float *w_rbf1, *w_rbf2;
   float *x_ji, *x_down;
+  const int64_t* z;
+  const int32_t* src;
+  const float *emb, *w_rbf0, *b_rbf0, *b_lin;
+  const float *tab_i, *tab_j;
 };
 
 __device__ __forceinline__ void r_bar(int cw) { asm volatile("bar.sync %0, %1;" ::"r"(1 + cw), "n"(R_WG) : "memory"); }
@@ -488,6 +438,28 @@
 #pragma unroll
     for (int i = 0; i < N / 2; ++i) acc[i] = __fadd_rn(acc[i], d[i]);
   }
+}
+__device__ __forceinline__ void r_complete_onto(RSmem& s, float (&acc)[64], const float (&d)[64], const float* tile,
+                                                int fr, int fc, int& it) {
+  wg_wait0();
+  r_release(s, it, 4);
+  it += 4;
+#pragma unroll
+  for (int j = 0; j < 16; ++j)
+#pragma unroll
+    for (int h = 0; h < 2; ++h) {
+      const int i = 4 * j + 2 * h;
+      const float2 t = *reinterpret_cast<const float2*>(tile + (fr + 8 * h) * R_LDS + 8 * j + fc);
+      acc[i] = __fadd_rn(__fadd_rn(t.x, acc[i]), d[i]);
+      acc[i + 1] = __fadd_rn(__fadd_rn(t.y, acc[i + 1]), d[i + 1]);
+    }
+}
+__device__ __forceinline__ void r_park(const float (&acc)[64], float* tile, int fr, int fc) {
+#pragma unroll
+  for (int j = 0; j < 16; ++j)
+#pragma unroll
+    for (int h = 0; h < 2; ++h)
+      *reinterpret_cast<float2*>(tile + (fr + 8 * h) * R_LDS + 8 * j + fc) = make_float2(acc[4 * j + 2 * h], acc[4 * j + 2 * h + 1]);
 }
 __device__ __forceinline__ void r_skip(RSmem& s, int& it, int n) {
   for (int i = 0; i < n; ++i, ++it) {
@@ -513,13 +485,14 @@
   atomicAdd(v_in + (size_t)cur * 128 + col, run);
 }
 
-template <bool FAST, int MODE>
+template <bool FAST, int MODE, bool TABLE = false>
 __global__ void __launch_bounds__(R_THREADS, 1)
 sphere_update_e_h16_kernel(const float* __restrict__ m, const float* __restrict__ x_ji,
                            const float* __restrict__ e1_in, const float* __restrict__ rbf0,
                            const int32_t* __restrict__ dst, int n_edges, REParams P, float* __restrict__ e1_out,
                            float* __restrict__ v_in) {
-  constexpr int NG = MODE == RE_B ? 8 : MODE == RE_BA ? 11 : 3;
+  constexpr bool INIT = MODE == RE_I || MODE == RE_IA;
+  constexpr int NG = MODE == RE_B ? 8 : MODE == RE_BA ? 11 : MODE == RE_I ? 1 : MODE == RE_IA ? 4 : 3;
   extern __shared__ __align__(1024) unsigned char h_raw[];
   RSmem& s = *reinterpret_cast<RSmem*>(h_raw);
   const int tid = threadIdx.x, wg = tid / R_WG;
@@ -533,15 +506,19 @@
     for (int i = 0; i < R_STAGES; ++i) { mbar_init(&s.full[i], 1); mbar_init(&s.empty[i], 8); }
     mbar_fence_init();
   }
-  if (MODE != RE_A) {
+  if (INIT) {
+    for (int i = tid; i < 128; i += R_THREADS) { s.bias[0][i] = __ldg(P.b_lin + i); s.bias[1][i] = __ldg(P.b_rbf0 + i); }
+    for (int i = tid; i < 128 * 6; i += R_THREADS) (&s.bias[2][0])[i] = __ldg(P.w_rbf0 + i);
+  } else if (MODE != RE_A) {
     for (int i = tid; i < 8 * 128; i += R_THREADS) {
       const float* b = P.g[i / 128].bias;
       s.bias[i / 128][i % 128] = b ? H_SA * __ldg(b + i % 128) : 0.f;
     }
+  }
+  if (MODE != RE_A)
     for (int i = tid; i < 128 * 8; i += R_THREADS) s.wr[i] = (i % 8 < 6) ? __ldg(P.w_rbf + (i / 8) * 6 + i % 8) : 0.f;
-  }
-  if (MODE != RE_B) {
-    constexpr int GA = MODE == RE_A ? 0 : 8;
+  if (MODE != RE_B && MODE != RE_I) {
+    constexpr int GA = MODE == RE_A ? 0 : MODE == RE_IA ? 1 : 8;
     for (int i = tid; i < 2 * 128; i += R_THREADS)
       s.bias_a[i / 128][i % 128] = (i / 128 ? H_SA : 1.0f) * __ldg(P.g[GA + i / 128].bias + i % 128);
     for (int i = tid; i < 128 * 8; i += R_THREADS) s.wr2[i] = __ldg(P.w_rbf2 + i);
@@ -598,7 +575,123 @@
       cp_async4(&s.rbf[cw][i], rbf0 + (size_t)e0 * 6 + (i < rows * 6 ? i : 0), i < rows * 6);
     RA a;
     float acc[64], d[64];
-    if (MODE != RE_A) {
+    if (INIT) {
+      if (wt < R_UNIT) cp_async4(&s.dst[cw][wt], dst + e0 + (wt < rows ? wt : 0), wt < rows);
+      cp_async_commit();
+      int zi[2], zj[2];
+#pragma unroll
+      for (int h = 0; h < 2; ++h) {
+        const int e = e0 + fr + 8 * h;
+        const bool ok = fr + 8 * h < rows;
+        zi[h] = ok ? (int)__ldg(P.z + __ldg(dst + e)) : 0;
+        zj[h] = ok ? (int)__ldg(P.z + __ldg(P.src + e)) : 0;
+      }
+      auto embedding_a = [&](const int (&zr)[2]) {
+#pragma unroll
+        for (int k = 0; k < 8; ++k)
+#pragma unroll
+          for (int r = 0; r < 4; ++r) {
+            const int h = r & 1, row = fr + 8 * h, col = frag_a_col(wt, k, r);
+            const float2 x = row < rows ? __ldg(reinterpret_cast<const float2*>(P.emb + (size_t)zr[h] * 128 + col))
+                                        : make_float2(0.f, 0.f);
+            r_split(x.x * H_SA, x.y * H_SA, a.hi[k][r], a.lo[k][r]);
+          }
+      };
+      auto rbf_a = [&]() {
+        const float* w0 = &s.bias[2][0];
+#pragma unroll
+        for (int k = 0; k < 8; ++k)
+#pragma unroll
+          for (int r = 0; r < 4; ++r) {
+            const int h = r & 1, row = fr + 8 * h, col = frag_a_col(wt, k, r);
+            float x[2];
+#pragma unroll
+            for (int u = 0; u < 2; ++u) {
+              float t = 0.f;
+#pragma unroll
+              for (int n = 0; n < 6; ++n) t = fmaf(w0[(col + u) * 6 + n], rbf[row * 6 + n], t);
+              x[u] = row < rows ? H_SA * hswish<FAST>(t + s.bias[1][col + u]) : 0.f;
+            }
+            r_split(x[0], x[1], a.hi[k][r], a.lo[k][r]);
+          }
+      };
+      if (TABLE) {
+#pragma unroll
+        for (int j = 0; j < 16; ++j)
+#pragma unroll
+          for (int h = 0; h < 2; ++h) {
+            const int row = fr + 8 * h, col = 8 * j + fc;
+            const float2 ti = __ldg(reinterpret_cast<const float2*>(P.tab_i + (size_t)zi[h] * 128 + col));
+            const float2 tj = __ldg(reinterpret_cast<const float2*>(P.tab_j + (size_t)zj[h] * 128 + col));
+            *reinterpret_cast<float2*>(tile + row * R_LDS + col) = make_float2(ti.x + tj.x, ti.y + tj.y);
+          }
+        cp_async_wait_all();
+        r_bar(cw);
+        rbf_a();
+        r_issue<2, 128>(s, a, acc, d, it);
+        stagger();
+        r_complete<2, 128>(s, acc, d, it);
+#pragma unroll
+        for (int j = 0; j < 16; ++j)
+#pragma unroll
+          for (int h = 0; h < 2; ++h) {
+            const int row = fr + 8 * h, col = 8 * j + fc, i = 4 * j + 2 * h;
+            const float2 t = *reinterpret_cast<const float2*>(tile + row * R_LDS + col);
+            acc[i] = fmaf(acc[i], H_INV, t.x) * (H_SA * H_SW);
+            acc[i + 1] = fmaf(acc[i + 1], H_INV, t.y) * (H_SA * H_SW);
+          }
+      } else {
+        embedding_a(zi);
+        r_issue<2, 128>(s, a, acc, d, it);
+        stagger();
+        r_complete<2, 128>(s, acc, d, it);
+        r_park(acc, tile, fr, fc);
+        embedding_a(zj);
+        r_issue<2, 128>(s, a, acc, d, it);
+        r_complete_onto(s, acc, d, tile, fr, fc, it);
+        r_park(acc, tile, fr, fc);
+        cp_async_wait_all();
+        r_bar(cw);
+        rbf_a();
+        r_issue<2, 128>(s, a, acc, d, it);
+        r_complete_onto(s, acc, d, tile, fr, fc, it);
+      }
+#pragma unroll
+      for (int h = 0; h < 2; ++h) {
+        const int row = fr + 8 * h;
+        float rb[6];
+#pragma unroll
+        for (int n = 0; n < 6; ++n) rb[n] = rbf[row * 6 + n];
+#pragma unroll
+        for (int j = 0; j < 16; ++j) {
+          const int col = 8 * j + fc, i = 4 * j + 2 * h;
+          float e2[2];
+#pragma unroll
+          for (int u = 0; u < 2; ++u) {
+            const float o = hswish<FAST>(fmaf(acc[i + u], H_INV, s.bias[0][col + u]));
+            bad |= !h_finite(o);
+            const float4 w0 = *reinterpret_cast<const float4*>(s.wr + (col + u) * 8);
+            const float2 w1 = *reinterpret_cast<const float2*>(s.wr + (col + u) * 8 + 4);
+            const float gsum = fmaf(w1.y, rb[5], fmaf(w1.x, rb[4], fmaf(w0.w, rb[3], fmaf(w0.z, rb[2],
+                               fmaf(w0.y, rb[1], w0.x * rb[0])))));
+            e2[u] = gsum * o;
+            acc[i + u] = o;
+          }
+          *reinterpret_cast<float2*>(tile + row * R_LDS + col) = make_float2(e2[0], e2[1]);
+        }
+      }
+      r_bar(cw);
+      r_segment_sums(tile, s.dst[cw], rows, wt, v_in);
+#pragma unroll
+      for (int j = 0; j < 16; ++j)
+#pragma unroll
+        for (int h = 0; h < 2; ++h) {
+          const int row = fr + 8 * h, i = 4 * j + 2 * h;
+          if (row < rows)
+            *reinterpret_cast<float2*>(e1_out + (size_t)(e0 + row) * 128 + 8 * j + fc) = make_float2(acc[i], acc[i + 1]);
+        }
+      if (MODE == RE_IA) r_acc_to_a(acc, a, H_SA);
+    } else if (MODE != RE_A) {
       if (wt < R_UNIT) cp_async4(&s.dst[cw][wt], dst + e0 + (wt < rows ? wt : 0), wt < rows);
       r_fetch_rows(tile, x_ji + (size_t)e0 * 128, rows, fr, fc);
       r_load_a<4>(a, m + (size_t)e0 * 64, 64, rows, wt);
@@ -696,7 +789,7 @@
       cp_async_commit();
       r_load_a<8>(a, e1_in + (size_t)e0 * 128, 128, rows, wt);
     }
-    if (MODE != RE_B) {
+    if (MODE != RE_B && MODE != RE_I) {
       tp(tr, 0);
       r_issue<2, 128>(s, a, acc, d, it);
       stagger();
@@ -779,11 +872,11 @@
   if (probe && cw == 0) { g_h16_trace[102] = clock64(); g_h16_trace[103] = (long long)global_ns(); }
 }
 
-template <int MODE>
+template <int MODE, bool TABLE = false>
 static int launch_update_e_h16(const float* m, const float* x_ji, const float* e1_in, const float* rbf0,
                                const int32_t* dst, int64_t n_edges, const REParams& P, float* e1_out, float* v_in,
                                cudaStream_t st) {
-  auto kfn = h16_fast_swish ? sphere_update_e_h16_kernel<true, MODE> : sphere_update_e_h16_kernel<false, MODE>;
+  auto kfn = h16_fast_swish ? sphere_update_e_h16_kernel<true, MODE, TABLE> : sphere_update_e_h16_kernel<false, MODE, TABLE>;
   cudaError_t e = cudaFuncSetAttribute(kfn, cudaFuncAttributeMaxDynamicSharedMemorySize, (int)sizeof(RSmem));
   if (e != cudaSuccess) {
     set_error("cudaFuncSetAttribute(%zu): %s", sizeof(RSmem), cudaGetErrorString(e));
@@ -799,141 +892,6 @@
   return DIG3D_OK;
 }
 
-struct HInitParams {
-  HGemm g[3];
-  const float *emb, *w_rbf0, *b_rbf0, *b_lin, *w_rbf1;
-  const float *tab_i, *tab_j;
-};
-
-template <bool FAST, bool TABLE>
-__global__ void __launch_bounds__(H_THREADS, 1)
-sphere_init_e_h16_kernel(const int64_t* __restrict__ z, const int32_t* __restrict__ src,
-                         const int32_t* __restrict__ dst, const float* __restrict__ rbf0, int n_edges, HInitParams P,
-                         float* __restrict__ e1, float* __restrict__ v_in) {
-  extern __shared__ __align__(1024) unsigned char h_raw[];
-  HSmem& s = *reinterpret_cast<HSmem*>(h_raw);
-  const int tid = threadIdx.x, warp = tid >> 5;
-  const int n_tiles = (n_edges + H_M - 1) / H_M, tile0 = blockIdx.x * 2, ntile = min(2, n_tiles - tile0);
-  float* w0 = &s.bias[2][0];
-  h_setup(s);
-  for (int i = tid; i < 128; i += H_THREADS) { s.bias[0][i] = __ldg(P.b_lin + i); s.bias[1][i] = __ldg(P.b_rbf0 + i); }
-  for (int i = tid; i < 128 * 6; i += H_THREADS) w0[i] = __ldg(P.w_rbf0 + i);
-  for (int i = tid; i < 128 * 8; i += H_THREADS) s.wr[i] = (i % 8 < 6) ? __ldg(P.w_rbf1 + (i / 8) * 6 + i % 8) : 0.f;
-  for (int i = tid; i < 2 * H_M; i += H_THREADS) {
-    const int t = i / H_M, r = i % H_M, e = (tile0 + t) * H_M + r;
-    const int d = (e < n_edges) ? dst[e] : -1, sj = (e < n_edges) ? src[e] : -1;
-    s.dst[t][r] = d;
-    s.aux[t][0][r] = d >= 0 ? (int)z[d] : 0;
-    s.aux[t][1][r] = sj >= 0 ? (int)z[sj] : 0;
-  }
-  tc_fence_before();
-  __syncthreads();
-  tc_fence_after();
-  HCtx c;
-  bool epi = false;
-  if (warp < H_CTRL_WARPS) {
-    h_regs_ctrl();
-    h_mma_n<false>(s, P.g, TABLE ? 1 : 3, ntile, s.tmem_base);
-  } else if (h_regs_epi(), (c = h_ctx(s, ntile)).t < ntile) {
-    epi = true;
-    const int e0 = (tile0 + c.t) * H_M, rows = min(H_M, n_edges - e0);
-    const bool valid = c.row < rows;
-    const size_t ge = (size_t)(e0 + c.row);
-    const int col0 = c.half * 64;
-    const uint32_t stash = c.tl + 256u + 128u * c.t + col0;
-    float rb[6];
-#pragma unroll
-    for (int n = 0; n < 6; ++n) rb[n] = valid ? __ldg(rbf0 + ge * 6 + n) : 0.f;
-    auto fill_embedding = [&](const int* zrow) {
-#pragma unroll
-      for (int k = 0; k < H_M * 16 / H_TILE_THREADS; ++k) {
-        const int f = c.et + k * H_TILE_THREADS, row = f >> 4, ku = f & 15;
-        float x[8];
-        if (row < rows) {
-          const float* er = P.emb + (size_t)zrow[row] * 128 + ku * 8;
-          const float4 p0 = __ldg(reinterpret_cast<const float4*>(er));
-          const float4 p1 = __ldg(reinterpret_cast<const float4*>(er + 4));
-          x[0] = p0.x * H_SA; x[1] = p0.y * H_SA; x[2] = p0.z * H_SA; x[3] = p0.w * H_SA;
-          x[4] = p1.x * H_SA; x[5] = p1.y * H_SA; x[6] = p1.z * H_SA; x[7] = p1.w * H_SA;
-        } else {
-#pragma unroll
-          for (int i = 0; i < 8; ++i) x[i] = 0.f;
-        }
-        h_store_ku(s, c, row, ku, x);
-      }
-    };
-    float acc[64];
-    if (!TABLE) {
-      fill_embedding(s.aux[c.t][0]);
-      h_epi_done(s, c.t);
-      h_drain<4, true>(s, c, col0, 2, acc);
-      fill_embedding(s.aux[c.t][1]);
-      h_epi_done(s, c.t);
-      h_drain<4, false>(s, c, col0, 2, acc);
-    }
-#pragma unroll
-    for (int p = 0; p < 4; ++p) {
-      float v[16];
-#pragma unroll
-      for (int i = 0; i < 16; ++i) {
-        const int col = col0 + 16 * p + i;
-        float a = 0.f;
-#pragma unroll
-        for (int n = 0; n < 6; ++n) a = fmaf(w0[col * 6 + n], rb[n], a);
-        v[i] = valid ? H_SA * hswish<FAST>(a + s.bias[1][col]) : 0.f;
-      }
-      h_store_a16(s, c, col0 + 16 * p, v);
-    }
-    h_epi_done(s, c.t);
-    if (TABLE) {
-      const float* ti = P.tab_i + (size_t)s.aux[c.t][0][c.row] * 128 + col0;
-      const float* tj = P.tab_j + (size_t)s.aux[c.t][1][c.row] * 128 + col0;
-#pragma unroll
-      for (int p = 0; p < 4; ++p) {
-        uint32_t r[16];
-#pragma unroll
-        for (int i = 0; i < 16; i += 4) {
-          const float4 a = __ldg(reinterpret_cast<const float4*>(ti + 16 * p + i));
-          const float4 b = __ldg(reinterpret_cast<const float4*>(tj + 16 * p + i));
-          r[i] = __float_as_uint(a.x + b.x); r[i + 1] = __float_as_uint(a.y + b.y);
-          r[i + 2] = __float_as_uint(a.z + b.z); r[i + 3] = __float_as_uint(a.w + b.w);
-        }
-        tmem_st16(stash + 16 * p, r);
-      }
-      tmem_st_wait();
-      h_drain<4, true>(s, c, col0, 2, acc);
-#pragma unroll
-      for (int p = 0; p < 4; ++p) {
-        uint32_t r[16];
-        tmem_ld16(stash + 16 * p, r);
-        tmem_ld_wait();
-#pragma unroll
-        for (int i = 0; i < 16; ++i) acc[16 * p + i] = fmaf(acc[16 * p + i], H_INV, __uint_as_float(r[i])) * (H_SA * H_SW);
-      }
-    } else {
-      h_drain<4, false>(s, c, col0, 2, acc);
-    }
-    float* e2t = reinterpret_cast<float*>(s.a[c.t][0]);
-#pragma unroll
-    for (int i = 0; i < 64; ++i) {
-      const int col = col0 + i;
-      const float o = hswish<FAST>(fmaf(acc[i], H_INV, s.bias[0][col]));
-      c.bad |= !h_finite(o);
-      const float4 w0 = *reinterpret_cast<const float4*>(s.wr + col * 8);
-      const float2 w1 = *reinterpret_cast<const float2*>(s.wr + col * 8 + 4);
-      const float gsum = fmaf(w1.y, rb[5], fmaf(w1.x, rb[4], fmaf(w0.w, rb[3], fmaf(w0.z, rb[2],
-                         fmaf(w0.y, rb[1], w0.x * rb[0])))));
-      e2t[c.row * H_LDS + col] = gsum * o;
-      acc[i] = o;
-    }
-    h_tile_bar(c.t);
-    h_segment_sums(s, c, rows, v_in);
-    h_tile_bar(c.t);
-    h_store_tile_coalesced<128>(s, c, col0, acc, e1 + (size_t)e0 * 128, rows);
-  }
-  h_finish(s, epi ? &c : nullptr);
-}
-
 struct HVBlock {
   const unsigned char* p[9];
   const float* b[9];
@@ -941,110 +899,210 @@
 };
 struct HVParams { HVBlock blk[8]; int n_lins, out_channels; };
 
+constexpr int V_STAGES = 6;
+constexpr int V_PLANE = 32 * R_UNIT * 16;
+struct VSmem {
+  unsigned char a[2][2][V_PLANE];
+  unsigned char w[V_STAGES][H_STAGE_BYTES];
+  uint64_t full[V_STAGES], empty[V_STAGES];
+};
+static_assert(sizeof(VSmem) <= 227 * 1024, "VSmem exceeds the shared memory of an SM");
+
+__device__ __forceinline__ void v_chunk(VSmem& s, uint32_t a_hi, uint32_t a_lo, int ch, float (&t)[64], int it) {
+#pragma unroll
+  for (int sl = 0; sl < 2; ++sl) {
+    const uint32_t w_hi = smem_u32(s.w[(it + 2 * ch + sl) % V_STAGES]), w_lo = w_hi + 4u * 128 * 16u;
+#pragma unroll
+    for (int ks = 0; ks < 2; ++ks) {
+      const uint32_t a_off = (uint32_t)((4 * ch + 2 * sl + ks) * 2 * R_UNIT * 16), b_off = (uint32_t)(ks * 2 * 128 * 16);
+      const uint64_t bh = smem_desc(w_hi + b_off, 128 * 16, 128), bl = smem_desc(w_lo + b_off, 128 * 16, 128);
+      mma_f16_ss(t, smem_desc(a_lo + a_off, R_UNIT * 16, 128), bh, (sl | ks) != 0);
+      mma_f16_ss(t, smem_desc(a_hi + a_off, R_UNIT * 16, 128), bl, 1);
+    }
+#pragma unroll
+    for (int ks = 0; ks < 2; ++ks) {
+      const uint32_t a_off = (uint32_t)((4 * ch + 2 * sl + ks) * 2 * R_UNIT * 16), b_off = (uint32_t)(ks * 2 * 128 * 16);
+      mma_f16_ss(t, smem_desc(a_hi + a_off, R_UNIT * 16, 128), smem_desc(w_hi + b_off, 128 * 16, 128), 1);
+    }
+  }
+}
+__device__ __forceinline__ void v_wait_slabs(VSmem& s, int it, int n) {
+  for (int i = 0; i < n; ++i) mbar_wait(&s.full[(it + i) % V_STAGES], ((it + i) / V_STAGES) & 1);
+}
+__device__ __forceinline__ void v_release(VSmem& s, int it, int n) {
+  __syncwarp();
+  if ((threadIdx.x & 31) == 0)
+    for (int i = 0; i < n; ++i) mbar_arrive(&s.empty[(it + i) % V_STAGES]);
+}
+__device__ __forceinline__ void v_half(VSmem& s, uint32_t a_hi, uint32_t a_lo, int nch, float (&acc)[64],
+                                      float (&d)[64], int& it) {
+  v_wait_slabs(s, it, 2);
+  wg_fence();
+  v_chunk(s, a_hi, a_lo, 0, acc, it);
+  wg_commit();
+  wg_wait0();
+  v_release(s, it, 2);
+#pragma unroll 1
+  for (int ch = 1; ch < nch; ++ch) {
+    v_wait_slabs(s, it + 2 * ch, 2);
+    wg_fence();
+    v_chunk(s, a_hi, a_lo, ch, d, it);
+    wg_commit();
+    wg_wait0();
+    v_release(s, it + 2 * ch, 2);
+#pragma unroll
+    for (int i = 0; i < 64; ++i) acc[i] = __fadd_rn(acc[i], d[i]);
+  }
+  it += 2 * nch;
+}
+__device__ __forceinline__ void v_store_a(unsigned char* hi, unsigned char* lo, const float (&v)[64], int col0, int fr,
+                                         int fc) {
+#pragma unroll
+  for (int j = 0; j < 16; ++j)
+#pragma unroll
+    for (int h = 0; h < 2; ++h) {
+      const int col = col0 + 8 * j + fc, i = 4 * j + 2 * h;
+      uint32_t xh, xl;
+      r_split(v[i], v[i + 1], xh, xl);
+      const int o = ((col >> 3) * R_UNIT + fr + 8 * h) * 16 + (col & 7) * 2;
+      *reinterpret_cast<uint32_t*>(hi + o) = xh;
+      *reinterpret_cast<uint32_t*>(lo + o) = xl;
+    }
+}
+
 template <bool FAST>
-__global__ void __launch_bounds__(H_THREADS, 1)
-sphere_update_v_h16_kernel(const float* __restrict__ v_in_all, int n_nodes, HVParams P, float* __restrict__ v_out_all) {
+__global__ void __launch_bounds__(R_THREADS, 1)
+sphere_update_v_h16_kernel(const float* __restrict__ v_in_all, int n_nodes, int n_blocks, HVParams P,
+                           float* __restrict__ v_out_all) {
   extern __shared__ __align__(1024) unsigned char h_raw[];
-  HSmem& s = *reinterpret_cast<HSmem*>(h_raw);
-  const int tid = threadIdx.x, warp = tid >> 5;
-  const HVBlock& B = P.blk[blockIdx.y];
-  const int r0 = blockIdx.x * H_M, rows = min(H_M, n_nodes - r0);
-  const int ng = P.n_lins + 1, C = P.out_channels;
-  __shared__ HGemm g[9];
-  h_setup(s, 2 * H_TILE_WARPS);
-  if (tid < ng) g[tid] = {B.p[tid], nullptr, tid == 0 ? 128 : 256, 128, (tid == 0 ? 128 : 256) * 128 * 4};
-  for (int i = tid; i < min(ng, 4) * 256; i += H_THREADS) (&s.bias[0][0])[i] = H_SA * __ldg(B.b[i / 256] + i % 256);
-  for (int i = tid; i < C * 256; i += H_THREADS) s.wr[i] = __ldg(B.w_out + i);
-  tc_fence_before();
+  VSmem& s = *reinterpret_cast<VSmem*>(h_raw);
+  const int tid = threadIdx.x, wg = tid / R_WG;
+  auto upb = [&]() { return (n_nodes + R_UNIT - 1) / R_UNIT; };
+  auto ppb = [&]() { return (upb() + 1) / 2; };
+  auto rounds = [&]() { return (n_blocks * ppb() - (int)blockIdx.x + (int)gridDim.x - 1) / (int)gridDim.x; };
+  if (tid == 0) {
+    for (int i = 0; i < V_STAGES; ++i) { mbar_init(&s.full[i], 1); mbar_init(&s.empty[i], 8); }
+    mbar_fence_init();
+  }
   __syncthreads();
-  tc_fence_after();
-  if (warp < H_CTRL_WARPS) {
-    h_regs_ctrl();
-    h_mma_n<true>(s, g, ng, 2, s.tmem_base);
-  } else {
-    h_regs_epi();
-    HCtx c = h_ctx(s, 2);
-    c.ahi = s.a[0][0];
-    c.alo = s.a[1][0];
-    const int et2 = tid - H_CTRL_THREADS;
-    const int col0 = c.half * 64;
-    const int gcol0 = 128 * c.t + col0;
-    const float* vin = v_in_all + ((size_t)blockIdx.y * n_nodes + r0) * 128;
-#pragma unroll
-    for (int k = 0; k < H_M * 16 / (2 * H_TILE_THREADS); ++k) {
-      const int f = et2 + k * 2 * H_TILE_THREADS, row = f >> 4, ku = f & 15;
-      float x[8];
-      if (row < rows) {
-        const float4 p0 = __ldg(reinterpret_cast<const float4*>(vin + (size_t)row * 128 + ku * 8));
-        const float4 p1 = __ldg(reinterpret_cast<const float4*>(vin + (size_t)row * 128 + ku * 8 + 4));
-        x[0] = p0.x * H_SA; x[1] = p0.y * H_SA; x[2] = p0.z * H_SA; x[3] = p0.w * H_SA;
-        x[4] = p1.x * H_SA; x[5] = p1.y * H_SA; x[6] = p1.z * H_SA; x[7] = p1.w * H_SA;
-      } else {
-#pragma unroll
-        for (int i = 0; i < 8; ++i) x[i] = 0.f;
-      }
-      h_store_ku(s, c, row, ku, x);
-    }
-    fence_async_smem();
-    tc_fence_before();
-    __syncwarp();
-    if ((tid & 31) == 0) mbar_arrive(&s.a_ready[0]);
-    float acc[64];
+  const int ng = P.n_lins + 1;
+
+  if (wg == 0) {
+    r_regs_producer();
+    if (tid == 0) {
+      int it = 0;
+      const int nr = rounds(), np = ppb();
+      const uint32_t bytes = 2u * 4u * 128u * 16u;
+      for (int k = 0; k < nr; ++k) {
+        const HVBlock& B = P.blk[(blockIdx.x + k * gridDim.x) / np];
+        for (int q = 0; q < ng; ++q) {
+          const int K = q ? 256 : 128;
+          for (int t = 0; t < 2; ++t)
+            for (int c = 0; c < K / H_SLAB_K; ++c, ++it) {
+              const int st = it % V_STAGES;
+              if (it >= V_STAGES) mbar_wait(&s.empty[st], ((it / V_STAGES) + 1) & 1);
+              mbar_arrive_expect_tx(&s.full[st], bytes);
+              bulk_g2s(s.w[st], B.p[q] + (size_t)t * K * 128 * 4 + (size_t)c * bytes, bytes, &s.full[st]);
+            }
+        }
+      }
+    }
+    return;
+  }
+
+  r_regs_consumer();
+  const int cw = threadIdx.x / R_WG - 1, wt = threadIdx.x & (R_WG - 1);
+  const int fr = frag_row(wt), fc = frag_col(wt), C = P.out_channels;
+  const int nr = rounds(), np = ppb(), nu = upb();
+  unsigned char *ahi = s.a[cw][0], *alo = s.a[cw][1];
+  const uint32_t a_hi = smem_u32(ahi), a_lo = smem_u32(alo);
+  int slabs = 2 * 128 / H_SLAB_K + 2 * (ng - 1) * 256 / H_SLAB_K;
+  bool staggered = cw == 1, bad = false;
+  auto stagger = [&]() {
+    if (!staggered) { asm volatile("bar.arrive 3, %0;" ::"n"(2 * R_WG) : "memory"); staggered = true; }
+  };
+  if (cw == 1) asm volatile("bar.sync 3, %0;" ::"n"(2 * R_WG) : "memory");
+  int it = 0;
+#pragma unroll 1
+  for (int k = 0; k < nr; ++k) {
+    const int pair = blockIdx.x + k * gridDim.x, blk = pair / np, unit = 2 * (pair % np) + cw;
+    if (unit >= nu) {
+      for (int i = 0; i < slabs; ++i, ++it) {
+        mbar_wait(&s.full[it % V_STAGES], (it / V_STAGES) & 1);
+        v_release(s, it, 1);
+      }
+      continue;
+    }
+    const HVBlock& B = P.blk[blk];
+    const int r0 = unit * R_UNIT, rows = min(R_UNIT, n_nodes - r0);
+    const float* vin = v_in_all + ((size_t)blk * n_nodes + r0) * 128;
+    float h0[64], acc[64], d[64];
+    r_bar(cw);
+#pragma unroll
+    for (int j = 0; j < 16; ++j)
+#pragma unroll
+      for (int h = 0; h < 2; ++h) {
+        const int row = fr + 8 * h, i = 4 * j + 2 * h;
+        const float2 x = row < rows ? __ldg(reinterpret_cast<const float2*>(vin + (size_t)row * 128 + 8 * j + fc))
+                                    : make_float2(0.f, 0.f);
+        acc[i] = x.x * H_SA;
+        acc[i + 1] = x.y * H_SA;
+      }
+    v_store_a(ahi, alo, acc, 0, fr, fc);
 #pragma unroll 1
     for (int q = 0; q < ng; ++q) {
-      h_drain<4, true>(s, c, col0, q == 0 ? 2 : 4, acc);
-#pragma unroll
-      for (int i = 0; i < 64; i += 4) {
-        float4 b;
-        if (q < 4) b = *reinterpret_cast<const float4*>(&(&s.bias[0][0])[q * 256 + gcol0 + i]);
-        else {
-          b = __ldg(reinterpret_cast<const float4*>(B.b[q] + gcol0 + i));
-          b.x *= H_SA; b.y *= H_SA; b.z *= H_SA; b.w *= H_SA;
-        }
-        acc[i] = fmaf(acc[i], H_SA * H_INV, b.x); acc[i + 1] = fmaf(acc[i + 1], H_SA * H_INV, b.y);
-        acc[i + 2] = fmaf(acc[i + 2], H_SA * H_INV, b.z); acc[i + 3] = fmaf(acc[i + 3], H_SA * H_INV, b.w);
-        if (q > 0) {
-          acc[i] = hswish8<FAST>(acc[i]); acc[i + 1] = hswish8<FAST>(acc[i + 1]);
-          acc[i + 2] = hswish8<FAST>(acc[i + 2]); acc[i + 3] = hswish8<FAST>(acc[i + 3]);
-        }
-      }
-      mbar_wait(&s.l_done, q & 1);
-      tc_fence_after();
+      fence_async_smem();
+      r_bar(cw);
+      const int nch = q ? 4 : 2;
+#pragma unroll
+      for (int t = 0; t < 2; ++t) {
+        float* v = t ? acc : h0;
+        v_half(s, a_hi, a_lo, nch, acc, d, it);
+        if (t == 0) stagger();
+#pragma unroll
+        for (int j = 0; j < 16; ++j)
+#pragma unroll
+          for (int u = 0; u < 2; ++u) {
+            const float b = H_SA * __ldg(B.b[q] + 128 * t + 8 * j + fc + u);
+#pragma unroll
+            for (int h = 0; h < 2; ++h) {
+              const int i = 4 * j + 2 * h + u;
+              const float x = fmaf(acc[i], H_SA * H_INV, b);
+              v[i] = q > 0 ? hswish8<FAST>(x) : x;
+            }
+          }
+      }
       if (q + 1 < ng) {
-#pragma unroll
-        for (int p = 0; p < 4; ++p) {
-          float v16[16];
-#pragma unroll
-          for (int i = 0; i < 16; ++i) v16[i] = acc[16 * p + i];
-          h_store_a16(s, c, gcol0 + 16 * p, v16);
-        }
-        fence_async_smem();
-        tc_fence_before();
-        __syncwarp();
-        if ((tid & 31) == 0) mbar_arrive(&s.a_ready[0]);
-      }
-    }
-    float* red = reinterpret_cast<float*>(s.a[0][0]);
-    const int slot = 2 * c.t + c.half;
+        r_bar(cw);
+        v_store_a(ahi, alo, h0, 0, fr, fc);
+        v_store_a(ahi, alo, acc, 128, fr, fc);
+      }
+    }
     for (int o = 0; o < C; ++o) {
-      float part = 0.f;
-#pragma unroll
-      for (int i = 0; i < 64; ++i) part = fmaf(acc[i], s.wr[o * 256 + gcol0 + i], part);
-      red[(c.row * 4 + slot) * C + o] = part * (1.0f / H_SA);
-      c.bad |= !h_finite(part);
-    }
-    asm volatile("bar.sync 3, %0;" ::"n"(2 * H_TILE_THREADS) : "memory");
-    if (slot == 0 && c.row < rows) {
-      float* out = v_out_all + ((size_t)blockIdx.y * n_nodes + r0 + c.row) * C;
-      for (int o = 0; o < C; ++o) {
-        const float* rr = red + (c.row * 4) * C + o;
-        out[o] = ((rr[0] + rr[C]) + rr[2 * C]) + rr[3 * C];
-      }
-    }
-    h_finish(s, &c);
-    return;
-  }
-  h_finish(s, nullptr);
+      float part[2] = {0.f, 0.f};
+#pragma unroll
+      for (int t = 0; t < 2; ++t)
+#pragma unroll
+        for (int j = 0; j < 16; ++j)
+#pragma unroll
+          for (int u = 0; u < 2; ++u) {
+            const float w = __ldg(B.w_out + o * 256 + 128 * t + 8 * j + fc + u);
+#pragma unroll
+            for (int h = 0; h < 2; ++h) part[h] = fmaf(t ? acc[4 * j + 2 * h + u] : h0[4 * j + 2 * h + u], w, part[h]);
+          }
+#pragma unroll
+      for (int h = 0; h < 2; ++h) {
+        part[h] += __shfl_xor_sync(0xffffffffu, part[h], 1);
+        part[h] += __shfl_xor_sync(0xffffffffu, part[h], 2);
+        const float y = part[h] * (1.0f / H_SA);
+        bad |= !h_finite(y);
+        const int row = fr + 8 * h;
+        if ((wt & 3) == 0 && row < rows) v_out_all[((size_t)blk * n_nodes + r0 + row) * C + o] = y;
+      }
+    }
+  }
+  stagger();
+  if (bad) atomicOr(&g_h16_overflow, 1u);
 }
 
 struct HLinParams { HGemm g[3]; };
@@ -1078,7 +1136,7 @@
   bool epi = false;
   if (warp < H_CTRL_WARPS) {
     h_regs_ctrl();
-    h_mma_n<false>(s, P.g, NPANEL, ntile, s.tmem_base);
+    h_mma_n(s, P.g, NPANEL, ntile, s.tmem_base);
   } else if (h_regs_epi(), (c = h_ctx(s, ntile)).t < ntile) {
     epi = true;
     const int r0 = (tile0 + c.t) * H_M, rows = min(H_M, n_rows - r0);
@@ -1408,24 +1466,25 @@
   return (int)v;
 }
 
+static void init_e_params(REParams& P, const int64_t* z, const int32_t* src, const dig3d_init_e_weights* w,
+                          const void* packed, const float* tab_i, const float* tab_j) {
+  P.g[0] = {(const unsigned char*)packed, nullptr, tab_i ? 128 : 384, 128};
+  P.w_rbf = w->w_rbf1;
+  P.z = z; P.src = src;
+  P.emb = w->emb; P.w_rbf0 = w->w_rbf0; P.b_rbf0 = w->b_rbf0; P.b_lin = w->b_lin;
+  P.tab_i = tab_i; P.tab_j = tab_j;
+}
+
 int dig3d_sphere_init_e_h16(const int64_t* z, const int32_t* src, const int32_t* dst, const float* rbf0,
                             int64_t n_edges, const dig3d_init_e_weights* w, const void* packed_lin, float* e1,
                             float* v_in, void* stream) {
   DIG3D_REQUIRE(z && src && dst && rbf0 && w && packed_lin && e1 && v_in, "sphere_init_e_h16: null pointer");
   DIG3D_REQUIRE(w->emb && w->w_rbf0 && w->b_rbf0 && w->b_lin && w->w_rbf1, "sphere_init_e_h16: null weight");
   if (n_edges == 0) return DIG3D_OK;
-  HInitParams P;
-  const size_t panel = (size_t)4 * 2 * 4 * 128 * 16;
-  for (int p = 0; p < 3; ++p) P.g[p] = {(const unsigned char*)packed_lin + p * panel, nullptr, 128, 128};
-  P.emb = w->emb; P.w_rbf0 = w->w_rbf0; P.b_rbf0 = w->b_rbf0; P.b_lin = w->b_lin; P.w_rbf1 = w->w_rbf1;
-  P.tab_i = P.tab_j = nullptr;
-  auto kfn = h16_fast_swish ? sphere_init_e_h16_kernel<true, false> : sphere_init_e_h16_kernel<false, false>;
-  int rc = h_smem_attr((const void*)kfn);
-  if (rc) return rc;
-  const int pairs = ceil_div(ceil_div(n_edges, H_M), 2);
-  kfn<<<pairs, H_THREADS, sizeof(HSmem), (cudaStream_t)stream>>>(z, src, dst, rbf0, (int)n_edges, P, e1, v_in);
-  DIG3D_LAUNCH_CHECK();
-  return DIG3D_OK;
+  REParams P = {};
+  init_e_params(P, z, src, w, packed_lin, nullptr, nullptr);
+  return launch_update_e_h16<RE_I, false>(nullptr, nullptr, nullptr, rbf0, dst, n_edges, P, e1, v_in,
+                                          (cudaStream_t)stream);
 }
 
 int dig3d_sphere_init_e_h16_tab(const int64_t* z, const int32_t* src, const int32_t* dst, const float* rbf0,
@@ -1436,18 +1495,34 @@
   DIG3D_REQUIRE(w->w_rbf0 && w->b_rbf0 && w->b_lin && w->w_rbf1, "sphere_init_e_h16_tab: null weight");
   DIG3D_REQUIRE((((uintptr_t)tab_i | (uintptr_t)tab_j) & 15) == 0, "sphere_init_e_h16_tab: tables must be 16-byte aligned");
   if (n_edges == 0) return DIG3D_OK;
-  HInitParams P;
-  P.g[0] = {(const unsigned char*)packed_rbf_panel, nullptr, 128, 128};
-  P.g[1] = P.g[2] = P.g[0];
-  P.emb = w->emb; P.w_rbf0 = w->w_rbf0; P.b_rbf0 = w->b_rbf0; P.b_lin = w->b_lin; P.w_rbf1 = w->w_rbf1;
-  P.tab_i = tab_i; P.tab_j = tab_j;
-  auto kfn = h16_fast_swish ? sphere_init_e_h16_kernel<true, true> : sphere_init_e_h16_kernel<false, true>;
-  int rc = h_smem_attr((const void*)kfn);
-  if (rc) return rc;
-  const int pairs = ceil_div(ceil_div(n_edges, H_M), 2);
-  kfn<<<pairs, H_THREADS, sizeof(HSmem), (cudaStream_t)stream>>>(z, src, dst, rbf0, (int)n_edges, P, e1, v_in);
-  DIG3D_LAUNCH_CHECK();
-  return DIG3D_OK;
+  REParams P = {};
+  init_e_params(P, z, src, w, packed_rbf_panel, tab_i, tab_j);
+  return launch_update_e_h16<RE_I, true>(nullptr, nullptr, nullptr, rbf0, dst, n_edges, P, e1, v_in,
+                                         (cudaStream_t)stream);
+}
+
+int dig3d_sphere_init_update_e_a_h16(const int64_t* z, const int32_t* src, const int32_t* dst, const float* rbf0,
+                                     int64_t n_edges, const dig3d_init_e_weights* w_init, const void* packed_init,
+                                     const float* tab_i, const float* tab_j, const dig3d_tc_update_e* w, float* e1,
+                                     float* v_in, float* x_ji, float* x_down, void* stream) {
+  DIG3D_REQUIRE(z && src && dst && rbf0 && w_init && packed_init && w && e1 && v_in && x_ji && x_down,
+                "sphere_init_update_e_a_h16: null pointer");
+  DIG3D_REQUIRE(w_init->w_rbf0 && w_init->b_rbf0 && w_init->b_lin && w_init->w_rbf1 && (tab_i || w_init->emb),
+                "sphere_init_update_e_a_h16: null weight");
+  DIG3D_REQUIRE(!tab_i == !tab_j, "sphere_init_update_e_a_h16: tab_i and tab_j must agree");
+  DIG3D_REQUIRE((((uintptr_t)tab_i | (uintptr_t)tab_j) & 15) == 0,
+                "sphere_init_update_e_a_h16: tables must be 16-byte aligned");
+  if (n_edges == 0) return DIG3D_OK;
+  REParams P = {};
+  init_e_params(P, z, src, w_init, packed_init, tab_i, tab_j);
+  P.g[1] = {(const unsigned char*)w->p_ji, w->b_ji, 128, 128};
+  P.g[2] = {(const unsigned char*)w->p_kj, w->b_kj, 128, 128};
+  P.g[3] = {(const unsigned char*)w->p_down, nullptr, 128, 64};
+  P.w_rbf1 = w->w_rbf1; P.w_rbf2 = w->w_rbf2;
+  P.x_ji = x_ji; P.x_down = x_down;
+  cudaStream_t st = (cudaStream_t)stream;
+  return tab_i ? launch_update_e_h16<RE_IA, true>(nullptr, nullptr, nullptr, rbf0, dst, n_edges, P, e1, v_in, st)
+               : launch_update_e_h16<RE_IA, false>(nullptr, nullptr, nullptr, rbf0, dst, n_edges, P, e1, v_in, st);
 }
 
 int dig3d_sphere_update_e_a_h16(const float* e1, const float* rbf0, int64_t n_edges, const dig3d_tc_update_e* w,
@@ -1594,10 +1669,17 @@
     P.blk[b].w_out = w[b].w_out;
   }
   auto kfn = h16_fast_swish ? sphere_update_v_h16_kernel<true> : sphere_update_v_h16_kernel<false>;
-  int rc = h_smem_attr((const void*)kfn);
-  if (rc) return rc;
-  dim3 grid(ceil_div(n_nodes, H_M), n_blocks);
-  kfn<<<grid, H_THREADS, sizeof(HSmem), (cudaStream_t)stream>>>(v_in_all, (int)n_nodes, P, v_out_all);
+  cudaError_t e = cudaFuncSetAttribute(kfn, cudaFuncAttributeMaxDynamicSharedMemorySize, (int)sizeof(VSmem));
+  if (e != cudaSuccess) {
+    set_error("cudaFuncSetAttribute(%zu): %s", sizeof(VSmem), cudaGetErrorString(e));
+    return DIG3D_ECUDA;
+  }
+  int dev = 0, n_sm = 132;
+  cudaGetDevice(&dev);
+  cudaDeviceGetAttribute(&n_sm, cudaDevAttrMultiProcessorCount, dev);
+  const int pairs = n_blocks * (int)ceil_div(ceil_div(n_nodes, R_UNIT), 2);
+  kfn<<<min(n_sm, pairs), R_THREADS, sizeof(VSmem), (cudaStream_t)stream>>>(v_in_all, (int)n_nodes, n_blocks, P,
+                                                                             v_out_all);
   DIG3D_LAUNCH_CHECK();
   return DIG3D_OK;
 }
diff --git a/dig_b200/csrc/wgmma.cuh b/dig_b200/csrc/wgmma.cuh
--- a/dig_b200/csrc/wgmma.cuh
+++ b/dig_b200/csrc/wgmma.cuh
@@ -136,6 +136,16 @@
       "wgmma.mma_async.sync.aligned.m64n128k16.f32.f16.f16 " TC90_D64 ", {%64,%65,%66,%67}, %68, p, 1, 1, 0;\n\t}"
       : TC90_D64_OPS(d)
       : "r"(a[0]), "r"(a[1]), "r"(a[2]), "r"(a[3]), "l"(b_desc), "r"(accumulate)
+      : "memory");
+}
+
+__device__ __forceinline__ void mma_f16_ss(float (&d)[64], uint64_t a_desc, uint64_t b_desc, uint32_t accumulate) {
+  asm volatile(
+      "{\n\t.reg .pred p;\n\t"
+      "setp.ne.b32 p, %66, 0;\n\t"
+      "wgmma.mma_async.sync.aligned.m64n128k16.f32.f16.f16 " TC90_D64 ", %64, %65, p, 1, 1, 0, 0;\n\t}"
+      : TC90_D64_OPS(d)
+      : "l"(a_desc), "l"(b_desc), "r"(accumulate)
       : "memory");
 }
 
@@ -193,14 +203,6 @@
   }
 }
 __device__ __forceinline__ void tmem_ld_wait() {}
-__device__ __forceinline__ void tmem_st16(uint32_t taddr, const uint32_t (&r)[16]) {
-  float4* p = reinterpret_cast<float4*>(tm_ptr(taddr, threadIdx.x & 31));
-#pragma unroll
-  for (int i = 0; i < 4; ++i)
-    __stcg(p + i, make_float4(__uint_as_float(r[4 * i]), __uint_as_float(r[4 * i + 1]), __uint_as_float(r[4 * i + 2]),
-                              __uint_as_float(r[4 * i + 3])));
-}
-__device__ __forceinline__ void tmem_st_wait() {}
 
 __device__ __forceinline__ void tm_store_frag(const float (&d)[32], int wt, uint32_t taddr) {
   float* base = tm_ptr(taddr, frag_row(wt)) + frag_col(wt);
diff --git a/dig_b200/threedgraph/method/dimenet_family.py b/dig_b200/threedgraph/method/dimenet_family.py
--- a/dig_b200/threedgraph/method/dimenet_family.py
+++ b/dig_b200/threedgraph/method/dimenet_family.py
@@ -358,19 +358,27 @@
             call("dig3d_triplet_basis_project_lists", a["bess"], a["angle"], a["torsion"] if tors else None, src, dst,
                  row_ptr, trip_ptr, graph_ptr, batch, E, T, int(self._basis_id), 4, 8, plan["w_s"].data_ptr(),
                  plan["w_t"].data_ptr() if tors else None, a["sbf_p"], a["t_p"] if tors else None, *ops._out_lists(g), st)
+        fuse = os.environ.get("DIG3D_FUSE_BA", "1") != "0"
+        zp = ops._p(z, torch.int64, "z")
         if plan["init_tables"] is not None:
             tab_i, tab_j, packed_rbf = plan["init_tables"]
-            call("dig3d_sphere_init_e_h16_tab", ops._p(z, torch.int64, "z"), src, dst, a["rbf0"], E, byref(plan["init_w"]),
-                 packed_rbf.data_ptr(), tab_i.data_ptr(), tab_j.data_ptr(), a["e1a"], v_in, st)
-        else:
-            call("dig3d_sphere_init_e_h16", ops._p(z, torch.int64, "z"), src, dst, a["rbf0"], E, byref(plan["init_w"]),
-                 plan["init_packed"].data_ptr(), a["e1a"], v_in, st)
-        fuse = os.environ.get("DIG3D_FUSE_BA", "1") != "0"
+            init_args = (packed_rbf.data_ptr(), tab_i.data_ptr(), tab_j.data_ptr())
+        else:
+            init_args = (plan["init_packed"].data_ptr(), None, None)
+        if fuse and L:
+            call("dig3d_sphere_init_update_e_a_h16", zp, src, dst, a["rbf0"], E, byref(plan["init_w"]), *init_args,
+                 byref(plan["layers"][0]), a["e1a"], v_in, a["x_ji"], a["x_down"], st)
+        elif plan["init_tables"] is not None:
+            call("dig3d_sphere_init_e_h16_tab", zp, src, dst, a["rbf0"], E, byref(plan["init_w"]), *init_args,
+                 a["e1a"], v_in, st)
+        else:
+            call("dig3d_sphere_init_e_h16", zp, src, dst, a["rbf0"], E, byref(plan["init_w"]), init_args[0],
+                 a["e1a"], v_in, st)
         e1, e1_next = a["e1a"], a["e1b"]
         x_ji, x_ji_next = a["x_ji"], a["x_ji2"]
         for l in range(L):
             w = plan["layers"][l]
-            if l == 0 or not fuse:
+            if not fuse:
                 call("dig3d_sphere_update_e_a_h16", e1, a["rbf0"], E, byref(w), x_ji, a["x_down"], st)
             sp = ctypes.c_void_p(a["sbf_p"] + 4 * 8 * T * l)
             tp = ctypes.c_void_p(a["t_p"] + 4 * 8 * T * l) if tors else None
diff --git a/include/dig3d.h b/include/dig3d.h
--- a/include/dig3d.h
+++ b/include/dig3d.h
@@ -196,6 +196,10 @@
                                  const int32_t* dst, int64_t n_edges, const dig3d_tc_update_e* w,
                                  const dig3d_tc_update_e* w_next, float* e1_out, float* v_in, float* x_ji_next,
                                  float* x_down_next, void* stream);
+int dig3d_sphere_init_update_e_a_h16(const int64_t* z, const int32_t* src, const int32_t* dst, const float* rbf0,
+                                     int64_t n_edges, const dig3d_init_e_weights* w_init, const void* packed_init,
+                                     const float* tab_i, const float* tab_j, const dig3d_tc_update_e* w, float* e1,
+                                     float* v_in, float* x_ji, float* x_down, void* stream);
 int dig3d_sphere_update_v_h16_supported(int32_t hidden, int32_t out_emb, int32_t out_channels, int32_t n_lins);
 int dig3d_sphere_update_v_h16(const float* v_in_all, int64_t n_nodes, int32_t n_blocks, int32_t out_channels,
                               int32_t n_lins, const void* const* packed, const dig3d_update_v_weights* w,
```

Measured after the change: 106,100 (median of 6 runs). 1.13x the previous value.
